# pachterlab/kallisto

Measured on AMD Instinct MI355X. Metric: M paired-end reads/sec quantified (human txome index), higher is better.
Workload: dtype u64+f64

## Files before the change

### include/kallisto_amd.h

```cpp
#ifndef KALLISTO_AMD_H
#define KALLISTO_AMD_H

#include <stddef.h>
#include <stdint.h>

#ifdef __cplusplus
extern "C" {
#endif

#define KAMD_MAX_FRAG_LEN 1000
#define KAMD_SLOTS_PER_BUCKET 3

typedef struct kamd_index kamd_index;
typedef struct kamd_ctx kamd_ctx;

typedef struct {
  int32_t k;
  uint64_t n_kmers, n_unitigs, n_blocks, n_uec, n_ecs, ec_nnz, n_targets, dlist_size;
  uint64_t n_buckets;
  uint64_t pad_buckets;
  const uint64_t* table;
  const uint32_t* slot_block;
  const uint32_t* slot_dist;
  const uint32_t* uec_ec;
  const uint64_t* ec_off;
  const uint32_t* ec_ids;
  const uint64_t* unitig_blk_off;
  const uint32_t* unitig_len;
  const uint32_t* blk_unitig;
  const uint32_t* blk_lb;
  const uint32_t* blk_ub;
  const uint32_t* blk_ec;
  const uint64_t* blk_pos_off;
  const uint32_t* blk_posw;
  const uint8_t* blk_sense;
  const int32_t* target_lens;
  const uint32_t* onlist_bits;
  uint64_t onlist_words;
  const uint64_t* dtable;
  uint64_t n_dbuckets, dpad_buckets;
  uint64_t dummy_slot;
  uint32_t dummy_uec;
  uint32_t dummy_strand;
  const uint32_t* utext;
  uint64_t utext_words;
  uint64_t text_bases;
  const uint64_t* unitig_gpos;
  uint32_t table_layout, slots_per_bucket, tag_q, tag_dsh, tag_w;
  uint64_t n_shades;
  const uint32_t* shade_colour;
  const uint64_t* core_off;
  const uint32_t* core_ids;
  uint64_t core_nnz;
  const uint64_t* shade_off;
  const uint32_t* shade_ids;
  uint64_t shade_nnz;
} kamd_index_view;

typedef struct {
  int32_t paired;
  double fld;
  double sd;
  int32_t single_overhang;
  int32_t strand;
  int32_t no_jump;
  int32_t do_union;
} kamd_quant_opts;

const char* kamd_last_error(void);
#define KAMD_ABI_VERSION 8
uint32_t kamd_abi_version(void);

int kamd_index_load(const char* path, int threads, kamd_index** out);
#define KAMD_TABLE_WIDE 0
#define KAMD_TABLE_COMPACT 1
#define KAMD_TABLE_AUTO 2
int kamd_index_load_layout(const char* path, int threads, int layout, double load, kamd_index** out);
int kamd_index_load_deferred(const char* path, int threads, int layout, double load, kamd_index** out);
int kamd_index_save(const kamd_index*, const char* path);
int kamd_flat_index_matches(const char* flat_path, const char* index_path);
void kamd_index_free(kamd_index*);
int kamd_index_get_view(const kamd_index*, kamd_index_view* out);
const char* kamd_index_target_name(const kamd_index*, uint64_t i);
int kamd_index_check_opts(const kamd_index*, const kamd_quant_opts*);

typedef struct {
  int32_t text_verify;
  int32_t items_per_wave;
  int32_t refill_min;
  int32_t lds_pad;
  int32_t em_form;
  int32_t em_entries_per_lane;
  int32_t em_windowed;
  int32_t em_graph;
  int32_t em_row_lanes;
  int32_t em_fin_blocks;
  int32_t em_local_block;
  int32_t em_group_div;
  int32_t em_split_len;
  int32_t dedup_form;
  int32_t align_chunks;
  int32_t em_small_nnz;
  int32_t em_reg_slices;
  int32_t em_hybrid;
  int32_t overflow_second_pass;
  int32_t em_giant_nnz;
  int32_t em_blocked;
} kamd_tuning;
int kamd_ctx_tune(kamd_ctx*, const kamd_tuning*);
int kamd_ctx_get_tuning(const kamd_ctx*, kamd_tuning* out);
int kamd_ctx_create(int device, void* hip_stream, kamd_ctx** out);
void kamd_ctx_destroy(kamd_ctx*);
int kamd_index_upload(kamd_ctx*, const kamd_index*);
int kamd_ec_reset(kamd_ctx*);
typedef struct {
  uint64_t n_buckets, pad_buckets;
  uint32_t table_layout, slots_per_bucket, tag_q, tag_dsh, tag_w;
  uint64_t n_dbuckets, dpad_buckets;
  uint64_t dummy_slot;
  uint32_t dummy_uec, dummy_strand;
  int32_t built_on_device;
  int32_t build_rounds;
  float build_ms;
  float build_count_ms, build_place_ms, build_order_ms, build_fill_ms, build_dlist_ms;
} kamd_table_info;
int kamd_ctx_table_info(kamd_ctx*, kamd_table_info* out);
int kamd_ctx_table_download(kamd_ctx*, uint64_t* table, uint32_t* slot_block, uint32_t* slot_dist, uint64_t* dtable);

uint64_t kamd_packed_record_words(int32_t max_len);
int kamd_pack_reads_host(const char* seqs, const uint64_t* off, const int32_t* len, uint64_t n_reads, int32_t max_len,
                         uint32_t* out_words, uint16_t* out_len);
int kamd_pack_reads_host_strided(const char* seqs, const uint64_t* off, const int32_t* len, uint64_t n_reads, int32_t max_len,
                                 uint32_t* out_words, uint16_t* out_len, uint64_t rec_stride, uint64_t rec_first);
int kamd_pack_reads_device(kamd_ctx*, const char* d_seqs, const uint64_t* d_off, const int32_t* d_len, uint64_t n_reads,
                           int32_t max_len, uint32_t* d_out_words, uint16_t* d_out_len);

typedef struct {
  const uint32_t* d_words;
  const uint16_t* d_len;
  uint64_t n_items;
  int32_t max_len;
  int32_t status;
  uint64_t first_bad_record;
} kamd_fastq_unit;
int kamd_fastq_unit_parse(kamd_ctx*, const char* const* d_text, const uint64_t* n_bytes, int32_t n_files, uint64_t n_records,
                          kamd_fastq_unit* out);
int kamd_fastq_batch_pack(kamd_ctx*, kamd_fastq_unit* out);
int kamd_fastq_unit_pack(kamd_ctx*, const char* const* d_text, const uint64_t* n_bytes, int32_t n_files, uint64_t n_records,
                         kamd_fastq_unit* out);

int kamd_pseudoalign(kamd_ctx*, const kamd_quant_opts*, const uint32_t* d_words, const uint16_t* d_len, uint64_t n_items,
                     int32_t max_len);
int kamd_fld_from_batch(kamd_ctx*, const kamd_quant_opts*, const uint32_t* d_words, const uint16_t* d_len, uint64_t n_items,
                        int32_t max_len, uint32_t* flens, uint64_t* n_used);
int kamd_fld_prefetch(kamd_ctx*, const kamd_quant_opts*, const uint32_t* d_words, const uint16_t* d_len, uint64_t n_items,
                      int32_t max_len);

typedef struct {
  uint64_t n_processed;
  uint64_t n_single;
  uint64_t n_multi;
  uint64_t n_probes;
  uint64_t n_bucket_reads;
  uint64_t n_distinct_tuples;
  uint64_t n_stream_words;
  uint64_t n_raw_words;
  uint64_t n_text_hits;
  uint64_t n_wave_iters;
  uint64_t n_lane_iters;
} kamd_align_stats;
int kamd_align_stats_get(kamd_ctx*, kamd_align_stats* out);

typedef struct {
  float last_align_kernel_ms;
  float last_em_ms;
  uint64_t last_em_iters;
  float last_classify_ms;
  int32_t kernel_a_version;
  uint64_t last_em_nnz;
  uint64_t last_em_nnz_multi;
  uint64_t last_em_nseg;
  uint64_t last_em_necs;
  int32_t last_em_k;
  uint32_t last_em_grid;
  uint32_t last_em_lds;
  int32_t last_em_plan_cached;
  float last_finalize_ms;
  uint64_t last_fin_records;
  uint64_t last_fin_stream_words;
  uint64_t last_fin_cand_words;
  float absorb_ms;
  uint64_t n_distinct_tuples;
  uint64_t tuple_store_words;
  uint64_t tuple_table_slots;
  uint64_t last_em_max_comp_nnz;
  uint64_t last_em_giant_nnz;
  uint64_t last_em_giant_rows;
  uint64_t last_em_giant_tr;
  uint32_t last_em_giant_chunks;
  int32_t last_em_graph_fallback;
  float last_em_plan_ms;
  uint64_t n_overflow_items;
  float overflow_ms;
  float last_merge_ms;
  float em_collective_ms;
  uint32_t em_collectives;
  uint64_t n_overflow_second_pass;
  uint64_t last_em_giant_pieces;
} kamd_profile;
int kamd_profile_get(kamd_ctx*, kamd_profile* out);

int kamd_debug_random_lines(kamd_ctx*, uint32_t n_blocks, uint32_t block_threads, uint32_t iters, double* gbytes_per_s,
                            double* mlines_per_s);
int kamd_debug_random_lines_span(kamd_ctx*, uint32_t n_blocks, uint32_t block_threads, uint32_t iters, uint32_t span_mb,
                                 uint32_t access_bytes, double* gbytes_per_s, double* mlines_per_s);

int kamd_ec_dense_counts(kamd_ctx*, uint32_t** d_counts, uint64_t* n);
int kamd_ec_tuples_export(kamd_ctx*, uint64_t* n_words, uint64_t* n_tuples);
int kamd_ec_tuples_copy(kamd_ctx*, uint32_t* d_out_words, uint64_t* d_out_rec_off);
int kamd_ec_tuples_replace(kamd_ctx*, const uint32_t* d_words, uint64_t n_words, const uint64_t* d_rec_off, uint64_t n_recs);

int kamd_ec_explicit_export(kamd_ctx*, uint64_t* n_words, uint64_t* n_recs);
int kamd_ec_explicit_copy(kamd_ctx*, uint32_t* d_out_words, uint64_t* d_out_rec_off);
int kamd_ec_explicit_replace(kamd_ctx*, const uint32_t* d_words, uint64_t n_words, const uint64_t* d_rec_off, uint64_t n_recs);

typedef struct kamd_comm kamd_comm;
#define KAMD_COMM_ID_BYTES 128
typedef struct {
  int (*allreduce_sum)(void* user, void* d_buf, uint64_t count, int32_t type);
  int (*allgather)(void* user, const void* d_send, void* d_recv, uint64_t bytes_per_rank);
  int (*broadcast)(void* user, void* d_buf, uint64_t bytes, int32_t root);
} kamd_comm_callbacks;
int kamd_comm_unique_id(void* id128);
int kamd_comm_create_rccl(kamd_ctx*, int32_t rank, int32_t world, const void* id128, kamd_comm** out);
int kamd_comm_create_callbacks(kamd_ctx*, int32_t rank, int32_t world, const kamd_comm_callbacks*, void* user, kamd_comm** out);
void kamd_comm_destroy(kamd_comm*);
int kamd_comm_info(const kamd_comm*, int32_t* rank, int32_t* world, int32_t* ranks_seen, int32_t* backend);
int kamd_ec_allreduce(kamd_ctx*, kamd_comm*);
int kamd_comm_broadcast_host(kamd_ctx*, kamd_comm*, void* buf, uint64_t bytes, int32_t root);
int kamd_comm_sum_u64_host(kamd_ctx*, kamd_comm*, uint64_t* values, uint64_t count);
int kamd_em_run_comm(kamd_ctx*, kamd_comm*, const double* eff_lens, uint64_t n_targets, uint32_t n_iter, uint32_t min_rounds,
                     double* alpha, double* alpha_before_zeroes, int32_t* rounds);

typedef struct {
  uint64_t n_ecs, nnz, n_pseudoaligned;
  const uint64_t* d_ec_off;
  const uint32_t* d_ec_ids;
  const uint32_t* d_counts;
} kamd_ec_result;
int kamd_ec_track_order(kamd_ctx*, int on);
int kamd_ec_finalize(kamd_ctx*, kamd_ec_result* out);
int kamd_ec_finalize_result(kamd_ctx*, kamd_ec_result* out);
int kamd_ec_download(kamd_ctx*, uint64_t* ec_off, uint32_t* ec_ids, uint32_t* counts);
int kamd_ec_upload(kamd_ctx*, const uint64_t* ec_off, const uint32_t* ec_ids, const uint32_t* counts, uint64_t n_ecs);
int kamd_ec_set_counts(kamd_ctx*, const uint32_t* counts);

int kamd_em_run(kamd_ctx*, const uint64_t* d_ec_off, const uint32_t* d_ec_ids, const uint32_t* d_counts,
                const uint32_t* d_weight_counts, uint64_t n_ecs, const double* eff_lens, uint64_t n_targets, uint32_t n_iter,
                uint32_t min_rounds, double* alpha, double* alpha_before_zeroes, int32_t* rounds);

typedef int (*kamd_em_sum_cb)(void* user, int32_t* d_counts, int32_t n);
// ... 58 lines not shown
```

### kallisto_amd/api.py

```python
from __future__ import annotations

import ctypes as C
import os
import sys
from dataclasses import dataclass, field

import numpy as np

HERE = os.path.dirname(os.path.abspath(__file__))
MAX_FRAG_LEN = 1000


class KallistoAmdError(RuntimeError):
    pass


def library_path() -> str:
    return os.path.join(HERE, "libkallisto_amd.so")


class _View(C.Structure):
    _fields_ = ([("k", C.c_int32)] +
                [(n, C.c_uint64) for n in ("n_kmers", "n_unitigs", "n_blocks", "n_uec", "n_ecs", "ec_nnz", "n_targets",
                                           "dlist_size", "n_buckets", "pad_buckets")] +
                [(n, C.c_void_p) for n in ("table", "slot_block", "slot_dist", "uec_ec", "ec_off", "ec_ids",
                                           "unitig_blk_off", "unitig_len", "blk_unitig", "blk_lb", "blk_ub", "blk_ec",
                                           "blk_pos_off", "blk_posw", "blk_sense", "target_lens", "onlist_bits")] +
                [("onlist_words", C.c_uint64), ("dtable", C.c_void_p), ("n_dbuckets", C.c_uint64), ("dpad_buckets", C.c_uint64),
                 ("dummy_slot", C.c_uint64), ("dummy_uec", C.c_uint32), ("dummy_strand", C.c_uint32),
                 ("utext", C.c_void_p), ("utext_words", C.c_uint64), ("text_bases", C.c_uint64), ("unitig_gpos", C.c_void_p)] +
                [(n, C.c_uint32) for n in ("table_layout", "slots_per_bucket", "tag_q", "tag_dsh", "tag_w")] +
                [("n_shades", C.c_uint64), ("shade_colour", C.c_size_t),
                 ("core_off", C.c_size_t), ("core_ids", C.c_size_t), ("core_nnz", C.c_uint64),
                 ("shade_off", C.c_size_t), ("shade_ids", C.c_size_t), ("shade_nnz", C.c_uint64)])


class QuantOpts(C.Structure):
    _fields_ = [("paired", C.c_int32), ("fld", C.c_double), ("sd", C.c_double), ("single_overhang", C.c_int32),
                ("strand", C.c_int32), ("no_jump", C.c_int32), ("do_union", C.c_int32)]


class _Stats(C.Structure):
    _fields_ = [(n, C.c_uint64) for n in ("n_processed", "n_single", "n_multi", "n_probes", "n_bucket_reads",
                                          "n_distinct_tuples", "n_stream_words", "n_raw_words", "n_text_hits", "n_wave_iters",
                                          "n_lane_iters")]


class Tuning(C.Structure):
    _fields_ = [(n, C.c_int32) for n in ("text_verify", "items_per_wave", "refill_min", "lds_pad", "em_form", "em_entries_per_lane", "em_windowed", "em_graph", "em_row_lanes",
                                         "em_fin_blocks", "em_local_block", "em_group_div", "em_split_len", "dedup_form", "align_chunks", "em_small_nnz", "em_reg_slices",
                                         "em_hybrid", "overflow_second_pass", "em_giant_nnz", "em_blocked")]


EM_FORMS = {"streamed": 1, "csr": 2, "local": 3}
ABI_VERSION = 8


class _Profile(C.Structure):
    _fields_ = [("last_align_kernel_ms", C.c_float), ("last_em_ms", C.c_float), ("last_em_iters", C.c_uint64),
                ("last_classify_ms", C.c_float), ("kernel_a_version", C.c_int32), ("last_em_nnz", C.c_uint64),
                ("last_em_nnz_multi", C.c_uint64), ("last_em_nseg", C.c_uint64), ("last_em_necs", C.c_uint64),
                ("last_em_k", C.c_int32), ("last_em_grid", C.c_uint32), ("last_em_lds", C.c_uint32),
                ("last_em_plan_cached", C.c_int32), ("last_finalize_ms", C.c_float), ("last_fin_records", C.c_uint64),
                ("last_fin_stream_words", C.c_uint64), ("last_fin_cand_words", C.c_uint64), ("absorb_ms", C.c_float),
                ("n_distinct_tuples", C.c_uint64), ("tuple_store_words", C.c_uint64), ("tuple_table_slots", C.c_uint64),
                ("last_em_max_comp_nnz", C.c_uint64), ("last_em_giant_nnz", C.c_uint64), ("last_em_giant_rows", C.c_uint64),
                ("last_em_giant_tr", C.c_uint64), ("last_em_giant_chunks", C.c_uint32), ("last_em_graph_fallback", C.c_int32),
                ("last_em_plan_ms", C.c_float), ("n_overflow_items", C.c_uint64), ("overflow_ms", C.c_float),
                ("last_merge_ms", C.c_float), ("em_collective_ms", C.c_float), ("em_collectives", C.c_uint32), ("n_overflow_second_pass", C.c_uint64), ("last_em_giant_pieces", C.c_uint64)]


class _AaStats(C.Structure):
    _fields_ = [("n_processed", C.c_uint64), ("n_rejected_offlist", C.c_uint64), ("n_all_empty", C.c_uint64), ("n_frame_clashes", C.c_uint64),
                ("n_winner", C.c_uint64 * 6), ("last_translate_ms", C.c_float), ("last_match_ms", C.c_float)]


class BgzfMember(C.Structure):
    _fields_ = [("src_off", C.c_uint64), ("src_len", C.c_uint32), ("isize", C.c_uint32), ("crc32", C.c_uint32), ("reserved", C.c_uint32),
                ("dst_off", C.c_uint64)]


class _InflateResult(C.Structure):
    _fields_ = [("status", C.c_int32), ("reason", C.c_int32), ("first_bad_member", C.c_uint64), ("n_bytes", C.c_uint64), ("n_newlines", C.c_uint64)]


class _TableInfo(C.Structure):
    _fields_ = [("n_buckets", C.c_uint64), ("pad_buckets", C.c_uint64), ("table_layout", C.c_uint32), ("slots_per_bucket", C.c_uint32),
                ("tag_q", C.c_uint32), ("tag_dsh", C.c_uint32), ("tag_w", C.c_uint32), ("n_dbuckets", C.c_uint64), ("dpad_buckets", C.c_uint64),
                ("dummy_slot", C.c_uint64), ("dummy_uec", C.c_uint32), ("dummy_strand", C.c_uint32), ("built_on_device", C.c_int32),
                ("build_rounds", C.c_int32), ("build_ms", C.c_float), ("build_count_ms", C.c_float), ("build_place_ms", C.c_float),
                ("build_order_ms", C.c_float), ("build_fill_ms", C.c_float), ("build_dlist_ms", C.c_float)]


class _FastqUnit(C.Structure):
    _fields_ = [("d_words", C.c_void_p), ("d_len", C.c_void_p), ("n_items", C.c_uint64), ("max_len", C.c_int32), ("status", C.c_int32),
                ("first_bad_record", C.c_uint64)]


class _Batch(C.Structure):
    _fields_ = [("d_words", C.c_void_p), ("d_len", C.c_void_p), ("n_items", C.c_uint64), ("max_len", C.c_int32)]


class _QuantOut(C.Structure):
    _fields_ = [("n_processed", C.c_uint64), ("em_rounds", C.c_int32), ("flens", C.c_void_p), ("eff_lens", C.c_void_p), ("est_counts", C.c_void_p),
                ("alpha_before_zeroes", C.c_void_p), ("tpm", C.c_void_p)]


class _EcResult(C.Structure):
    _fields_ = [("n_ecs", C.c_uint64), ("nnz", C.c_uint64), ("n_pseudoaligned", C.c_uint64), ("d_ec_off", C.c_void_p),
                ("d_ec_ids", C.c_void_p), ("d_counts", C.c_void_p)]


_LIB = None

_SYMBOLS = {
    "kamd_last_error": (C.c_char_p, []),
    "kamd_abi_version": (C.c_uint32, []),
    "kamd_index_load": (C.c_int, [C.c_char_p, C.c_int, C.POINTER(C.c_void_p)]),
    "kamd_index_load_layout": (C.c_int, [C.c_char_p, C.c_int, C.c_int, C.c_double, C.POINTER(C.c_void_p)]),
    "kamd_index_load_deferred": (C.c_int, [C.c_char_p, C.c_int, C.c_int, C.c_double, C.POINTER(C.c_void_p)]),
    "kamd_index_free": (None, [C.c_void_p]),
    "kamd_index_save": (C.c_int, [C.c_void_p, C.c_char_p]),
# ... 378 lines not shown
                                                          text.data_ptr(), int(text.numel() if text_cap is None else text_cap), 1 if debug_check_crc else 0,
                                                          C.byref(res), C.byref(ms)), "kamd_debug_bgzf_inflate")
            return {"status": int(res.status), "reason": int(res.reason), "first_bad_member": int(res.first_bad_member), "n_bytes": int(res.n_bytes),
                    "n_newlines": int(res.n_newlines), "kernel_ms": float(ms.value)}
        _check(load_library().kamd_bgzf_inflate(self._h, comp.data_ptr(), int(comp.numel() if comp_bytes is None else comp_bytes), arr, len(members),
                                                text.data_ptr(), int(text.numel() if text_cap is None else text_cap), C.byref(res)), "kamd_bgzf_inflate")
        return {"status": int(res.status), "reason": int(res.reason), "first_bad_member": int(res.first_bad_member), "n_bytes": int(res.n_bytes),
                "n_newlines": int(res.n_newlines)}

    def text_cut(self, texts, n_bytes, max_records: int):
        ptrs = (C.c_void_p * 2)(*[t.data_ptr() for t in texts], *([None] * (2 - len(texts))))
        nb = (C.c_uint64 * 2)(*[int(n) for n in n_bytes], *([0] * (2 - len(texts))))
        nrec, end = C.c_uint64(0), (C.c_uint64 * 2)(0, 0)
        _check(load_library().kamd_text_cut(self._h, ptrs, nb, len(texts), int(max_records), C.byref(nrec), end), "kamd_text_cut")
        return int(nrec.value), [int(end[i]) for i in range(len(texts))]

    def fld_prefetch(self, opts: QuantOpts, words, lens, n_items: int, max_len: int):
        _check(load_library().kamd_fld_prefetch(self._h, C.byref(opts), words.data_ptr(), lens.data_ptr(), n_items, max_len),
               "kamd_fld_prefetch")

    def fld_from_batch(self, opts: QuantOpts, words, lens, n_items: int, max_len: int, flens=None, used: int = 0):
        if flens is None:
            flens = np.zeros(MAX_FRAG_LEN, np.uint32)
        used = C.c_uint64(used)
        _check(load_library().kamd_fld_from_batch(self._h, C.byref(opts), words.data_ptr(), lens.data_ptr(), n_items, max_len,
                                                  flens.ctypes.data, C.byref(used)), "kamd_fld_from_batch")
        return flens, int(used.value)

    def stats(self) -> dict:
        s = _Stats()
        _check(load_library().kamd_align_stats_get(self._h, C.byref(s)), "kamd_align_stats_get")
        return {n: int(getattr(s, n)) for n, _ in _Stats._fields_}

    def random_lines(self, n_blocks: int, block_threads: int = 256, iters: int = 256, span_mb: int = 0, access_bytes: int = 64):
        g, m = C.c_double(0), C.c_double(0)
        _check(load_library().kamd_debug_random_lines_span(self._h, n_blocks, block_threads, iters, span_mb, access_bytes, C.byref(g), C.byref(m)),
               "kamd_debug_random_lines_span")
        return g.value, m.value

    def profile(self) -> dict:
        p = _Profile()
        _check(load_library().kamd_profile_get(self._h, C.byref(p)), "kamd_profile_get")
        return {"align_kernel_ms": float(p.last_align_kernel_ms), "em_ms": float(p.last_em_ms), "em_iters": int(p.last_em_iters),
                "classify_ms": float(p.last_classify_ms), "kernel_a_version": int(p.kernel_a_version),
                "em_nnz": int(p.last_em_nnz), "em_nnz_multi": int(p.last_em_nnz_multi), "em_nseg": int(p.last_em_nseg),
                "em_necs": int(p.last_em_necs), "em_k": int(p.last_em_k), "em_grid": int(p.last_em_grid), "em_lds": int(p.last_em_lds),
                "em_plan_cached": int(p.last_em_plan_cached), "finalize_ms": float(p.last_finalize_ms),
                "fin_records": int(p.last_fin_records), "fin_stream_words": int(p.last_fin_stream_words),
                "fin_cand_words": int(p.last_fin_cand_words), "absorb_ms": float(p.absorb_ms), "n_distinct_tuples": int(p.n_distinct_tuples),
                "tuple_store_words": int(p.tuple_store_words), "tuple_table_slots": int(p.tuple_table_slots),
                "em_max_comp_nnz": int(p.last_em_max_comp_nnz), "em_giant_nnz": int(p.last_em_giant_nnz), "em_giant_rows": int(p.last_em_giant_rows),
                "em_giant_tr": int(p.last_em_giant_tr), "em_giant_chunks": int(p.last_em_giant_chunks), "em_graph_fallback": int(p.last_em_graph_fallback), "em_giant_pieces": int(p.last_em_giant_pieces),
                "em_plan_ms": float(p.last_em_plan_ms), "n_overflow_items": int(p.n_overflow_items), "overflow_ms": float(p.overflow_ms),
                "merge_ms": float(p.last_merge_ms), "em_collective_ms": float(p.em_collective_ms), "em_collectives": int(p.em_collectives), "n_overflow_second_pass": int(p.n_overflow_second_pass)}

    def dense_counts(self):
        torch = self.torch
        p, n = C.c_void_p(), C.c_uint64(0)
        _check(load_library().kamd_ec_dense_counts(self._h, C.byref(p), C.byref(n)), "kamd_ec_dense_counts")
        return _alias_tensor(torch, p.value, int(n.value), torch.int32, self.device)

    def tuples_export(self):
        torch = self.torch
        nw, nt = C.c_uint64(0), C.c_uint64(0)
        _check(load_library().kamd_ec_tuples_export(self._h, C.byref(nw), C.byref(nt)), "kamd_ec_tuples_export")
        words = torch.zeros(max(int(nw.value), 1), dtype=torch.int32, device=f"cuda:{self.device}")
        offs = torch.zeros(max(int(nt.value), 1), dtype=torch.int64, device=f"cuda:{self.device}")
        _check(load_library().kamd_ec_tuples_copy(self._h, words.data_ptr(), offs.data_ptr()), "kamd_ec_tuples_copy")
        return words[:int(nw.value)], offs[:int(nt.value)]

    def tuples_replace(self, words, offs):
        _check(load_library().kamd_ec_tuples_replace(self._h, words.data_ptr() if words.numel() else None, words.numel(),
                                                     offs.data_ptr() if offs.numel() else None, offs.numel()),
               "kamd_ec_tuples_replace")

    def explicit_export(self):
        torch = self.torch
        nw, nr = C.c_uint64(0), C.c_uint64(0)
        _check(load_library().kamd_ec_explicit_export(self._h, C.byref(nw), C.byref(nr)), "kamd_ec_explicit_export")
        words = torch.zeros(max(int(nw.value), 1), dtype=torch.int32, device=f"cuda:{self.device}")
        offs = torch.zeros(max(int(nr.value), 1), dtype=torch.int64, device=f"cuda:{self.device}")
        _check(load_library().kamd_ec_explicit_copy(self._h, words.data_ptr(), offs.data_ptr()), "kamd_ec_explicit_copy")
        return words[:int(nw.value)], offs[:int(nr.value)]

    def explicit_replace(self, words, offs):
        _check(load_library().kamd_ec_explicit_replace(self._h, words.data_ptr() if words.numel() else None, words.numel(),
                                                       offs.data_ptr() if offs.numel() else None, offs.numel()),
               "kamd_ec_explicit_replace")

    def ec_allreduce(self, comm: "Comm"):
        _check(load_library().kamd_ec_allreduce(self._h, comm._h), "kamd_ec_allreduce")

    def em_run_comm(self, comm: "Comm", eff_lens: np.ndarray, n_iter: int = 10000, min_rounds: int = 50):
        eff = np.ascontiguousarray(eff_lens, np.float64)
        T = len(eff)
        alpha = np.zeros(T, np.float64)
        abz = np.zeros(T, np.float64)
        rounds = C.c_int32(0)
        _check(load_library().kamd_em_run_comm(self._h, comm._h, eff.ctypes.data, T, n_iter, min_rounds, alpha.ctypes.data,
                                               abz.ctypes.data, C.byref(rounds)), "kamd_em_run_comm")
        return alpha, abz, int(rounds.value)

    def finalize(self, download: bool = True):
        res = _EcResult()
        _check(load_library().kamd_ec_finalize(self._h, C.byref(res)), "kamd_ec_finalize")
        self.ec_result = res
        if not download:
# ... 404 lines not shown
```

### kallisto_amd/csrc/kamd_ctx.hip

```cpp
#include "kamd_dev.h"

namespace {
void tuning_defaults(kamd_tuning* t) {
  memset(t, 0, sizeof *t);
  t->text_verify = 1; t->items_per_wave = 1024; t->refill_min = 8; t->lds_pad = -1;
  t->em_form = 3; t->em_local_block = 1024; t->em_group_div = -1; t->em_split_len = 16; t->em_small_nnz = -1; t->em_entries_per_lane = -1; t->em_windowed = 2; t->em_graph = 1; t->em_row_lanes = 4;
  t->em_fin_blocks = 1024; t->dedup_form = 2; t->align_chunks = -1; t->em_reg_slices = 1;
  t->em_hybrid = 1; t->overflow_second_pass = 1; t->em_giant_nnz = -1; t->em_blocked = 1;
}
void tuning_merge(kamd_tuning* t, const kamd_tuning& n) {
  if (n.text_verify == 1 || n.text_verify == 2) t->text_verify = n.text_verify;
  if (n.dedup_form == 1 || n.dedup_form == 2) t->dedup_form = n.dedup_form;
  if (n.items_per_wave >= 64) t->items_per_wave = n.items_per_wave;
  if (n.refill_min >= 1 && n.refill_min <= 64) t->refill_min = n.refill_min;
  if (n.lds_pad != 0) t->lds_pad = n.lds_pad < 0 ? -1 : n.lds_pad;
  if (n.em_form >= 1 && n.em_form <= 3) t->em_form = n.em_form;
  if (n.em_local_block == 128 || n.em_local_block == 256 || n.em_local_block == 512 || n.em_local_block == 1024) t->em_local_block = n.em_local_block;
  if (n.em_split_len >= 1 && n.em_split_len <= 64) t->em_split_len = n.em_split_len;
  if (n.em_group_div >= 1 && n.em_group_div <= 1024) t->em_group_div = n.em_group_div;
  else if (n.em_group_div < 0) t->em_group_div = -1;
  if (n.em_small_nnz != 0) t->em_small_nnz = n.em_small_nnz < 0 ? -1 : std::min(n.em_small_nnz, 4096);
  if (n.em_entries_per_lane != 0) t->em_entries_per_lane = n.em_entries_per_lane < 0 ? -1 : n.em_entries_per_lane;
  if (n.em_windowed == 1 || n.em_windowed == 2) t->em_windowed = n.em_windowed;
  if (n.em_graph == 1 || n.em_graph == 2) t->em_graph = n.em_graph;
  if (n.em_row_lanes == 2 || n.em_row_lanes == 4 || n.em_row_lanes == 8) t->em_row_lanes = n.em_row_lanes;
  if (n.em_fin_blocks >= 64) t->em_fin_blocks = n.em_fin_blocks;
  if (n.align_chunks != 0) t->align_chunks = n.align_chunks < 0 ? -1 : std::min(n.align_chunks, 64);
  if (n.em_reg_slices == 1 || n.em_reg_slices == 2) t->em_reg_slices = n.em_reg_slices;
  if (n.em_hybrid == 1 || n.em_hybrid == 2) t->em_hybrid = n.em_hybrid;
  if (n.overflow_second_pass >= 1 && n.overflow_second_pass <= 3) t->overflow_second_pass = n.overflow_second_pass;
  if (n.em_blocked == 1 || n.em_blocked == 2) t->em_blocked = n.em_blocked;
  if (n.em_giant_nnz != 0) t->em_giant_nnz = n.em_giant_nnz < 0 ? -1 : std::max(n.em_giant_nnz, 8);
}
void tuning_from_env(kamd_tuning* t) {
  const char* e = getenv("KAMD_TUNE");
  if (!e || !*e) return;
  kamd_tuning n; memset(&n, 0, sizeof n);
  struct Field { const char* name; int32_t kamd_tuning::*p; bool onoff; };
  static const Field fields[] = {
    {"text_verify", &kamd_tuning::text_verify, true}, {"items_per_wave", &kamd_tuning::items_per_wave, false}, {"refill_min", &kamd_tuning::refill_min, false},
    {"lds_pad", &kamd_tuning::lds_pad, false}, {"em_form", &kamd_tuning::em_form, false}, {"em_entries_per_lane", &kamd_tuning::em_entries_per_lane, false},
    {"em_windowed", &kamd_tuning::em_windowed, true}, {"em_graph", &kamd_tuning::em_graph, true}, {"em_row_lanes", &kamd_tuning::em_row_lanes, false},
    {"em_fin_blocks", &kamd_tuning::em_fin_blocks, false}, {"em_local_block", &kamd_tuning::em_local_block, false}, {"em_group_div", &kamd_tuning::em_group_div, false},
    {"em_split_len", &kamd_tuning::em_split_len, false}, {"dedup_form", &kamd_tuning::dedup_form, false}, {"align_chunks", &kamd_tuning::align_chunks, false},
    {"em_small_nnz", &kamd_tuning::em_small_nnz, false}, {"em_reg_slices", &kamd_tuning::em_reg_slices, true}, {"em_hybrid", &kamd_tuning::em_hybrid, true},
    {"overflow_second_pass", &kamd_tuning::overflow_second_pass, false}, {"em_giant_nnz", &kamd_tuning::em_giant_nnz, false}, {"em_blocked", &kamd_tuning::em_blocked, true}};
  std::string all(e);
  for (size_t pos = 0; pos < all.size();) {
    size_t end = all.find(',', pos);
    if (end == std::string::npos) end = all.size();
    const std::string kv = all.substr(pos, end - pos);
    pos = end + 1;
    const size_t eq = kv.find('=');
    if (eq == std::string::npos) continue;
    const std::string key = kv.substr(0, eq), val = kv.substr(eq + 1);
    bool known = false;
    for (const Field& f : fields) {
      if (key != f.name) continue;
      known = true;
      int32_t v = atoi(val.c_str());
      if (key == "em_form") v = val == "streamed" ? 1 : val == "csr" ? 2 : val == "local" ? 3 : v;
      if (key == "overflow_second_pass" && v == 0) v = 2;
      n.*(f.p) = f.onoff ? (v != 0 ? 1 : 2) : v;
    }
    if (!known) fprintf(stderr, "[kallisto_amd] KAMD_TUNE: unknown field '%s' ignored\n", key.c_str());
  }
  tuning_merge(t, n);
}
}
namespace kamdi {
void apply_quant_opts(kamd_ctx* c, const kamd_quant_opts* o) {
  c->ix.no_jump = o->no_jump ? 1 : 0;
  c->ix.union_mode = o->do_union ? 1 : 0;
  c->ix.comprehensive = (o->strand != 0 && (o->no_jump || o->do_union || c->ix.n_shades)) ? 1 : 0;
}
void apply_tuning(kamd_ctx* c) {
  c->items_per_wave = c->tune.items_per_wave; c->refill_min = c->tune.refill_min;
}
int sync_state(kamd_ctx* c) {
  if (!c->state_pin) HIPC(hipHostMalloc((void**)&c->state_pin, sizeof(DevState), hipHostMallocDefault));
  HIPC(hipMemcpyAsync(c->state_pin, c->state.p, sizeof(DevState), hipMemcpyDeviceToHost, c->stream));
  HIPC(hipStreamSynchronize(c->stream));
  memcpy(&c->host_state, c->state_pin, sizeof(DevState));
  return 0;
}
int push_state(kamd_ctx* c) {
  HIPC(hipMemcpyAsync(c->state.p, &c->host_state, sizeof(DevState), hipMemcpyHostToDevice, c->stream));
  return 0;
}
}

extern "C" uint32_t kamd_abi_version(void) { return KAMD_ABI_VERSION; }
extern "C" int kamd_ctx_create(int device, void* hip_stream, kamd_ctx** out) {
  if (!out) return kamd::fail(-1, "kamd_ctx_create: null output pointer");
  *out = nullptr;
  int ndev = 0;
  if (hipGetDeviceCount(&ndev) != hipSuccess || ndev == 0)
    return kamd::fail(-102, "kamd_ctx_create: no HIP device available (this library has no CPU path)");
  if (device < 0 || device >= ndev) return kamd::fail(-1, "kamd_ctx_create: bad device ordinal");
// ... 219 lines not shown
    const u64 b = __umul64hi(x, n_buckets);
    u64 v;
    if (WORDS == 8) {
      const ulonglong2* bp = (const ulonglong2*)(table + b * 8);
      const ulonglong2 s0 = bp[0], s1 = bp[1], s2 = bp[2], s3 = bp[3];
      v = s0.x ^ s0.y ^ s1.x ^ s1.y ^ s2.x ^ s2.y ^ s3.x ^ s3.y;
    } else v = table[b * 8 + (x & 7)];
    acc ^= v;
    x = kamd::mix64(x ^ v);
  }
  if (acc == 0x1234567ULL) sink[0] = acc;
}
}
extern "C" int kamd_debug_random_lines_span(kamd_ctx* c, uint32_t n_blocks, uint32_t block_threads, uint32_t iters, uint32_t span_mb,
                                            uint32_t access_bytes, double* gbytes_per_s, double* mlines_per_s) {
  if (!c || !c->has_index) return kamd::fail(-1, "kamd_debug_random_lines: no context / index");
  HIPC(hipSetDevice(c->device));
  if (int rc = c->sizes.ensure(64, 0, c->stream)) return rc;
  u64 nb = c->ix.n_buckets;
  if (span_mb) nb = std::min<u64>(nb, (u64)span_mb * 1024 * 1024 / 64);
  auto launch = [&](int it) {
    if (access_bytes == 8) hipLaunchKernelGGL(k_random_lines<1>, dim3(n_blocks), dim3(block_threads), 0, c->stream, c->ix.table, nb, it, c->sizes.as<u64>());
    else hipLaunchKernelGGL(k_random_lines<8>, dim3(n_blocks), dim3(block_threads), 0, c->stream, c->ix.table, nb, it, c->sizes.as<u64>());
  };
  launch(8);
  HIPC(hipEventRecord(c->ev0, c->stream));
  launch((int)iters);
  HIPC(hipEventRecord(c->ev1, c->stream));
  HIPC(hipEventSynchronize(c->ev1));
  float ms = 0.f;
  HIPC(hipEventElapsedTime(&ms, c->ev0, c->ev1));
  const double lines = (double)n_blocks * block_threads * iters;
  if (mlines_per_s) *mlines_per_s = lines / (ms * 1e-3) / 1e6;
  if (gbytes_per_s) *gbytes_per_s = lines * 64.0 / (ms * 1e-3) / 1e9;
  return 0;
}
extern "C" int kamd_debug_random_lines(kamd_ctx* c, uint32_t n_blocks, uint32_t block_threads, uint32_t iters, double* gbytes_per_s,
                                       double* mlines_per_s) {
  return kamd_debug_random_lines_span(c, n_blocks, block_threads, iters, 0, 64, gbytes_per_s, mlines_per_s);
}

extern "C" int kamd_profile_get(kamd_ctx* c, kamd_profile* p) {
  if (!c || !p) return kamd::fail(-1, "kamd_profile_get: null argument");
  p->last_align_kernel_ms = c->last_align_ms; p->last_em_ms = c->last_em_ms; p->last_em_iters = c->last_em_iters;
  p->last_classify_ms = c->last_classify_ms; p->kernel_a_version = 3;
  p->last_em_nnz = c->last_em_nnz; p->last_em_nnz_multi = c->last_em_nnz_multi; p->last_em_nseg = c->last_em_nseg; p->last_em_necs = c->last_em_necs;
  p->last_em_k = c->last_em_k; p->last_em_grid = c->last_em_grid; p->last_em_lds = c->last_em_lds; p->last_em_plan_cached = c->last_em_plan_cached;
  p->last_finalize_ms = c->last_finalize_ms; p->last_fin_records = c->last_fin_records; p->last_fin_stream_words = c->last_fin_stream_words;
  p->last_fin_cand_words = c->last_fin_cand_words;
  p->absorb_ms = c->last_absorb_ms; p->n_distinct_tuples = c->n_distinct_tuples; p->tuple_store_words = c->host_state.ts_words; p->tuple_table_slots = c->tcap;
  p->last_em_max_comp_nnz = c->last_em_max_comp_nnz; p->last_em_giant_nnz = c->last_em_giant_nnz; p->last_em_giant_rows = c->last_em_giant_rows;
  p->last_em_giant_tr = c->last_em_giant_tr; p->last_em_giant_chunks = c->last_em_giant_chunks; p->last_em_graph_fallback = c->last_em_graph_fallback; p->last_em_giant_pieces = c->last_em_giant_pieces;
  p->last_em_plan_ms = c->last_em_plan_ms;
  p->n_overflow_items = c->overflow_total; p->overflow_ms = c->overflow_ms;
  p->n_overflow_second_pass = c->overflow_second_total;
  p->last_merge_ms = c->last_merge_ms; p->em_collective_ms = c->em_coll_ms; p->em_collectives = c->em_coll_n;
  return 0;
}

namespace {
typedef struct ncclComm* ncclComm_t;
typedef struct { char internal[KAMD_COMM_ID_BYTES]; } ncclUniqueId;
typedef int ncclResult_t;
enum { kNcclSum = 0, kNcclUint8 = 1, kNcclInt32 = 2, kNcclUint32 = 3, kNcclUint64 = 5, kNcclFloat64 = 8 };
struct RcclApi {
  void* lib = nullptr;
  ncclResult_t (*GetUniqueId)(ncclUniqueId*) = nullptr;
  ncclResult_t (*CommInitRank)(ncclComm_t*, int, ncclUniqueId, int) = nullptr;
  ncclResult_t (*CommDestroy)(ncclComm_t) = nullptr;
  ncclResult_t (*CommCount)(const ncclComm_t, int*) = nullptr;
  ncclResult_t (*AllReduce)(const void*, void*, size_t, int, int, ncclComm_t, hipStream_t) = nullptr;
  ncclResult_t (*AllGather)(const void*, void*, size_t, int, ncclComm_t, hipStream_t) = nullptr;
  ncclResult_t (*Broadcast)(const void*, void*, size_t, int, int, ncclComm_t, hipStream_t) = nullptr;
  const char* (*GetErrorString)(ncclResult_t) = nullptr;
};
RcclApi g_rccl;
int rccl_load() {
  if (g_rccl.lib) return 0;
  void* h = nullptr;
  for (const char* n : {"librccl.so", "librccl.so.1"}) { h = dlopen(n, RTLD_NOW | RTLD_NOLOAD); if (h) break; }
  if (!h) if (const char* e = getenv("KAMD_RCCL_LIB")) h = dlopen(e, RTLD_NOW | RTLD_GLOBAL);
  if (!h) for (const char* n : {"librccl.so.1", "librccl.so", "/opt/rocm/lib/librccl.so.1", "/opt/rocm/lib/librccl.so"}) { h = dlopen(n, RTLD_NOW | RTLD_GLOBAL); if (h) break; }
  if (!h) return kamd::fail(-106, std::string("kamd_comm: librccl.so could not be loaded (") + (dlerror() ? dlerror() : "not found") + "); set KAMD_RCCL_LIB");
  RcclApi a; a.lib = h;
  a.GetUniqueId = (decltype(a.GetUniqueId))dlsym(h, "ncclGetUniqueId");
  a.CommInitRank = (decltype(a.CommInitRank))dlsym(h, "ncclCommInitRank");
  a.CommDestroy = (decltype(a.CommDestroy))dlsym(h, "ncclCommDestroy");
  a.CommCount = (decltype(a.CommCount))dlsym(h, "ncclCommCount");
  a.AllReduce = (decltype(a.AllReduce))dlsym(h, "ncclAllReduce");
  a.AllGather = (decltype(a.AllGather))dlsym(h, "ncclAllGather");
  a.Broadcast = (decltype(a.Broadcast))dlsym(h, "ncclBroadcast");
  a.GetErrorString = (decltype(a.GetErrorString))dlsym(h, "ncclGetErrorString");
  if (!a.GetUniqueId || !a.CommInitRank || !a.CommDestroy || !a.AllReduce || !a.AllGather || !a.Broadcast)
    return kamd::fail(-106, "kamd_comm: librccl.so lacks an expected entry point");
  g_rccl = a;
  return 0;
}
int rccl_fail(ncclResult_t r, const char* what) {
  return kamd::fail(-107, std::string(what) + ": " + (g_rccl.GetErrorString ? g_rccl.GetErrorString(r) : "RCCL error") + " (" + std::to_string(r) + ")");
}
}

struct kamd_comm {
  kamd_ctx* ctx = nullptr;
  int device = 0;
  int rank = 0, world = 1;
// ... 307 lines not shown
```

### kallisto_amd/csrc/kamd_dev.h

```cpp
#pragma once

#include <hip/hip_runtime.h>

#include <dlfcn.h>

#include <algorithm>
#include <cstring>
#include <string>
#include <chrono>
#include <thread>
#include <vector>

#include "../../include/kallisto_amd.h"
#include "kamd_core.h"
#include "kamd_fq_core.h"
#include "kamd_host.h"
#include "kamd_em_local.h"
#include "kamd_em_sell.h"

#define HIPC(x)                                                                                   \
  do {                                                                                            \
    hipError_t e_ = (x);                                                                          \
    if (e_ != hipSuccess) return kamd::fail(-100, std::string(#x) + ": " + hipGetErrorString(e_)); \
  } while (0)
// ... 199 lines not shown
  u32 n_set_bitmaps = 0;
  kamd_table_info tinfo{};
  DBuf dense, stream_buf, rec_off, overflow_items, overflow_scratch, state, rec_slot, retry, ttable, list;
  DBuf cand, cand_off, cand_slot, ctable, clist, sizes, block_sums, tup_bound, tup_off, tup_big;
  DBuf raw2, overflow_left, stats_b;
  u64 overflow_second_total = 0;
  DBuf ov_state; DevState* ov_pin = nullptr; hipStream_t ov_stream = nullptr; hipEvent_t ov_ev_in = nullptr, ov_ev_done = nullptr, ov_ev_t0 = nullptr, ov_ev_t1 = nullptr;
  bool ov_side_pending = false;
  u64 last_fin_big = 0;
  DBuf explicit_items, explicit_items_big, exp_stream, exp_off, exp_scratch, bs_cp, bs_samp, raw, dense_first, exp_key, cand_key, ec_first;
  DBuf ec_off, ec_ids, ec_counts;
  DBuf em_alpha, em_next, em_eff, em_state, em_cn, em_colcnt, em_coloff, em_colrow, em_segoff, em_segt, em_partial, em_a0, em_a1, em_single, em_actflag, em_actpos, em_active;
  DBuf pm_a, pm_b, pm_rank;
  DBuf eml_tmp, ems_tmp, ems_plan, ems_maps;
  SellCache* sell_cache = nullptr;
  u64 ec_generation = 0;
  int last_em_plan_cached = 0;
  DBuf fq_tiles, fq_nlpos[2], fq_recs, fq_res, fq_words, fq_len;
  void* fq_host = nullptr;
  u64 fq_batch_reads = 0; int32_t fq_batch_max_len = 0, fq_batch_files = 0;
  DBuf fld_tl, fld_card, fld_scratch, fld_items, fld_cand;
  void* fld_host = nullptr; u64 fld_host_cap = 0;
  hipStream_t fld_stream = nullptr; hipEvent_t fld_ev = nullptr, fld_ev_in = nullptr;
  struct { const uint32_t* w = nullptr; const uint16_t* l = nullptr; u64 n = 0; int32_t max_len = 0, strand = 0, so = 0; bool valid = false; } fld_pending;
  struct { const uint32_t* w = nullptr; const uint16_t* l = nullptr; u64 n = 0; int32_t max_len = 0, strand = 0, so = 0, comp = 0; bool valid = false; } fld_deferred;
  DBuf pt_label, pt_flag, pt_len, pt_rowpos, pt_nnzpos, pt_off, pt_ids, pt_counts, pt_wcounts, pt_hist, pt_ck_alpha, pt_ck_a;
  DevState host_state{};
  DevState* state_pin = nullptr;
  u64 tcap = 0, ccap = 0;
  DBuf tstore;
  bool ttable_clean = false;
  u64 recs_total = 0;
  u64 multi_before = 0;
  u64 n_distinct_tuples = 0;
  float last_absorb_ms = 0.f; hipEvent_t ev_ab0 = nullptr, ev_ab1 = nullptr;
  kamd_ec_result result{};
  bool finalized = false;
  u64 exp_words_done = 0;
  hipEvent_t ev0 = nullptr, ev1 = nullptr;
  float last_align_ms = 0.f, last_em_ms = 0.f, last_classify_ms = 0.f;
  hipEvent_t ev2 = nullptr, ev3 = nullptr, ev_fin0 = nullptr, ev_fin1 = nullptr;
  DBuf stats_a;
  hipStream_t al_stream = nullptr; hipEvent_t al_ev_in = nullptr, al_ev_out = nullptr; std::vector<hipEvent_t> al_ev_chunk;
  float last_finalize_ms = 0.f; u64 last_fin_records = 0, last_fin_stream_words = 0, last_fin_cand_words = 0;
  hipStream_t em_stream = nullptr;
  hipStream_t em_side_stream = nullptr; hipEvent_t em_ev_fork = nullptr, em_ev_join = nullptr;
  void* em_pin = nullptr; size_t em_pin_bytes = 0;
  DBuf em_clk;
  DBuf hy_sub, hy_a, hy_b, hy_x, hy_maps;
  DBuf hy_gb[6];
  hipStream_t hy_giant_stream = nullptr;
  hipEvent_t hy_ev_sell = nullptr, hy_ev_giant = nullptr;
  uint64_t last_em_max_comp_nnz = 0, last_em_giant_nnz = 0, last_em_giant_rows = 0, last_em_giant_tr = 0;
  uint32_t last_em_giant_chunks = 0; uint64_t last_em_giant_pieces = 0; int last_em_graph_fallback = 0; float last_em_plan_ms = 0.f;
  float last_merge_ms = 0.f, em_coll_ms = 0.f; uint32_t em_coll_n = 0; hipEvent_t ev_mg0 = nullptr, ev_mg1 = nullptr;
  const uint32_t* labels_override = nullptr;
  bool em_prefer_hybrid = false;
  uint64_t overflow_total = 0; float overflow_ms = 0.f; hipEvent_t ev_ov0 = nullptr, ev_ov1 = nullptr;
  int items_per_wave = 1024, refill_min = 8;
  kamd_tuning tune{};
  bool track_order = false;
  bool had_overflow_items = false;
  int n_cus = 0, last_em_k = 0; unsigned last_em_grid = 0, last_em_lds = 0;
  uint64_t last_em_iters = 0, last_em_nnz = 0, last_em_nnz_multi = 0, last_em_nseg = 0, last_em_necs = 0;
  DBuf aa_frames, aa_flen, aa_scratch, aa_offlist, aa_ctr;
  bool aa_ready = false;
  kamd_aa_stats aa_stats{};
  hipEvent_t aa_ev[3] = {nullptr, nullptr, nullptr};
  DBuf inf_members, inf_res, txt_counts, txt_res;
  std::vector<struct kamd_comm*> comms;
};

namespace kamdi {
int sync_state(kamd_ctx* c);
int push_state(kamd_ctx* c);
void apply_quant_opts(kamd_ctx* c, const kamd_quant_opts* o);
void apply_tuning(kamd_ctx* c);
void comm_detach_all(kamd_ctx* c);
int index_build_device(kamd_ctx* c, const kamd_index* hix, const kamd_index_view& v, DevIndex* d, kamd_table_info* info);
int exclusive_scan(kamd_ctx* c, const u32* sizes, u64 n, u64* out, u64* d_total);
int tuples_clear(kamd_ctx* c);
int absorb_tuples(kamd_ctx* c, const u32* batch, const u64* rec_off, u64 n, u64 batch_words, u64 key_base, u64 n_tuple_bound,
                  const u64* first_idx = nullptr, u32 fixed_stride = 0, u64 item0 = 0);
template <class T>
int upload(kamd_ctx* c, const T* host, size_t n, const T** dev) {
  void* p = nullptr;
  size_t bytes = std::max<size_t>(n, 1) * sizeof(T);
  HIPC(hipMalloc(&p, bytes));
  c->index_allocs.push_back(p);
  if (n) HIPC(hipMemcpyAsync(p, host, n * sizeof(T), hipMemcpyHostToDevice, c->stream));
  *dev = reinterpret_cast<const T*>(p);
  return 0;
}
}
```

### kallisto_amd/csrc/kamd_em.hip

```cpp
#include "kamd_dev.h"

namespace {

struct EmState {
  int iter;
  int chcount;
  int final_round;
  int done;
  int rounds;
  int force_final;
  int pad[2];
};
struct EmNow { int it, fin, done, rounds; };
__host__ __device__ inline EmNow em_next_round(const EmState& prev, int n_iter, int min_rounds, bool spec) {
  EmNow n; n.it = prev.iter; n.fin = prev.final_round; n.done = prev.done; n.rounds = prev.rounds;
  if (n.done) return n;
  if (prev.final_round) { n.done = 1; n.rounds = prev.iter; return n; }
  const bool stopEM = !spec && prev.chcount == 0 && prev.iter > min_rounds;
  n.it = prev.iter + 1;
  n.fin = (stopEM || prev.force_final) ? 1 : 0;
  if (n.it >= n_iter) { n.done = 1; n.rounds = n_iter; }
  return n;
}
__device__ __forceinline__ double em_clamped(const double* alpha, const double* a, u32 t, int clamp) {
// ... 1078 lines not shown
    ems_reg_gather<NB>(w, lds0, v);
#pragma unroll
    for (int i = 0; i < 4 * NB; i++) S += v[i];
    if constexpr (NQ > 2) return ems_reg_sum<NQ - 2, false>(w + 2, lds0, S);
    else return S;
  } else {
    constexpr int NB = NQ < 4 ? NQ : 4;
    double v[4 * NB];
    ems_reg_gather<NB>(w, lds0, v);
#pragma unroll
    for (int st = 1; st < 4 * NB; st *= 2)
#pragma unroll
      for (int i = 0; i + st < 4 * NB; i += 2 * st) v[i] += v[i + st];
    if constexpr (NQ > 4) return ems_reg_sum<NQ - 4, true>(w + 4, lds0, S + v[0]);
    else return S + v[0];
  }
}
template <int W, bool TREE, int NQ = 1>
__device__ __forceinline__ double ems_reg_slice_sum(const u64* w, u32 nq, const unsigned char* lds0) {
  if constexpr (NQ >= W) return ems_reg_sum<W, TREE>(w, lds0);
  else { if (nq <= (u32)NQ) return ems_reg_sum<NQ, TREE>(w, lds0); return ems_reg_slice_sum<W, TREE, NQ + 1>(w, nq, lds0); }
}
__device__ __forceinline__ u32 pm_scan_seg_steps(int reach, int lane) {
  const int r = lane & 15;
  u32 m = 0;
  if (__ballot(reach >= 1 && r >= 1)) m |= 1u;
  if (__ballot(reach >= 2 && r >= 2)) m |= 2u;
  if (__ballot(reach >= 4 && r >= 4)) m |= 4u;
  if (__ballot(reach >= 8 && r >= 8)) m |= 8u;
  if (__ballot((lane & 16) && reach > r)) m |= 16u;
  if (__ballot(lane >= 32 && reach > lane - 32)) m |= 32u;
  return m;
}
__device__ __forceinline__ double pm_scan_seg_masked(double y, int reach, int lane, u32 steps) {
  const int r = lane & 15;
  if (steps & 1u) { const double t = pm_dpp<0x111, 0xF>(y); if (reach >= 1 && r >= 1) y += t; }
  if (steps & 2u) { const double t = pm_dpp<0x112, 0xF>(y); if (reach >= 2 && r >= 2) y += t; }
  if (steps & 4u) { const double t = pm_dpp<0x114, 0xF>(y); if (reach >= 4 && r >= 4) y += t; }
  if (steps & 8u) { const double t = pm_dpp<0x118, 0xF>(y); if (reach >= 8 && r >= 8) y += t; }
  if (steps & 16u) { const double t = pm_dpp<0x142, 0xA>(y); if ((lane & 16) && reach > r) y += t; }
  if (steps & 32u) { const double t = pm_dpp<0x143, 0xC>(y); if (lane >= 32 && reach > lane - 32) y += t; }
  return y;
}
__device__ __forceinline__ double ems_slice_sum_narrow(const u64* e, u32 width, const double* src) {
  double S = 0.0;
  for (u32 j = 0; j < width; j += 4) {
    const u64 w = e[(size_t)(j >> 2) * 64];
    const u32 lo = (u32)w, hi = (u32)(w >> 32);
    const double v0 = src[lo & 0xFFFFu], v1 = src[lo >> 16], v2 = src[hi & 0xFFFFu], v3 = src[hi >> 16];
    S += v0; S += v1; S += v2; S += v3;
  }
  return S;
}
template <int W, int NS>
__device__ __forceinline__ void ems_group_rounds_reg(const EmSellDev& P, u32 g, unsigned char* smem, u32 tid, u32 nthr, const double* alpha, const double* a,
                                                     double* alpha_out, double* a_out, int n_rounds, int clamp, int* s_hist, long long* clk = nullptr) {
  namespace L = kamd_em_sell;
  constexpr bool TREE = W >= 8 || (W == 4 && NS == 2);
  const int lane = lane_id();
  const u32 wv = (u32)__builtin_amdgcn_readfirstlane((int)(tid >> 6)), NW = nthr >> 6;
  const u32 r0 = P.row_base[g], nR = P.row_base[g + 1] - r0, t0 = P.tr_base[g], nT = P.tr_base[g + 1] - t0;
  const u32 rs0 = P.rslice_base[g], nrs = P.rslice_base[g + 1] - rs0, cs0 = P.cslice_base[g], ncs = P.cslice_base[g + 1] - cs0;
  const u64 re0 = P.rell_base[g], ce0 = P.cell_base[g];
  const u32 nru = (u32)(P.rell_base[g + 1] - re0), ncu = (u32)(P.cell_base[g + 1] - ce0);
  double* s_a0 = reinterpret_cast<double*>(smem);
  double* s_g = s_a0 + (nT + 1);
  double* s_al0 = s_g + (nR + 1);
  double* s_single = s_al0 + (nT + 1); double* s_eff = s_single + nT;
  u64* s_cw = reinterpret_cast<u64*>(s_eff + nT);
  u32* s_rdesc = reinterpret_cast<u32*>(s_cw + nR); u32* s_cdesc = s_rdesc + 2 * nrs;
  uint16_t* s_rell = reinterpret_cast<uint16_t*>(s_cdesc + 2 * ncs); uint16_t* s_cell = s_rell + ((nru + 1) & ~1u);
  const u32 a_off = 0u, g_off = (nT + 1) * 8u;
  const bool near = g_off + (nR + 1) * 8u <= 0x10000u;
  for (u32 i = tid; i < nT; i += nthr) {
    double al = alpha[t0 + i], av = a[t0 + i];
    if (clamp && al < 1e-7 / 10.0) { al = 0.0; av = 0.0; }
    s_al0[i] = al; s_a0[i] = av; s_single[i] = P.single[t0 + i]; s_eff[i] = P.eff[t0 + i];
  }
  for (u32 i = tid; i < nR; i += nthr) s_cw[i] = P.cw[r0 + i];
  for (u32 i = tid; i < 2 * nrs; i += nthr) s_rdesc[i] = P.rdesc[2 * (u64)rs0 + i];
  for (u32 i = tid; i < 2 * ncs; i += nthr) s_cdesc[i] = P.cdesc[2 * (u64)cs0 + i];
  for (u32 i = tid; i < nru; i += nthr) { const uint16_t v = P.rell[re0 + i]; s_rell[i] = v == (uint16_t)L::SELL_PAD ? (uint16_t)nT : v; }
  for (u32 i = tid; i < ncu; i += nthr) { const uint16_t v = P.cell[ce0 + i]; s_cell[i] = v == (uint16_t)L::SELL_PAD ? (uint16_t)nR : v; }
  if (tid == 0) { s_al0[nT] = s_a0[nT] = 0.0; s_g[nR] = 0.0; }
  __syncthreads();
  struct Own { u64 w[W]; u32 nq, seg, steps; int reach; bool has, meta, fin; };
  auto take = [&](const u32* desc, const uint16_t* ell, u32 s, u32 n_slices, u32 n_segs, u32 zero, u32 base_off) {
    Own o;
    o.has = near && s < n_slices; o.nq = 1; o.seg = 0; o.reach = 0; o.meta = false; o.fin = false; o.steps = 0;
    if (o.has && (((desc[2 * s + 1] & 0xFFFFu) + 3u) >> 2) > (u32)W) o.has = false;
    const u64 padw = (u64)(base_off + zero * 8u) * 0x0001000100010001ULL;
#pragma unroll
    for (int q = 0; q < W; q++) o.w[q] = padw;
    if (o.has) {
      const u32 d0 = desc[2 * s], d1 = desc[2 * s + 1];
      o.meta = (d0 & L::DESC_META) != 0;
      const u32 off = d0 & ~L::DESC_META, width = d1 & 0xFFFFu;
      o.nq = (u32)__builtin_amdgcn_readfirstlane((int)((width + 3u) >> 2));
      const u64* e = reinterpret_cast<const u64*>(ell + off + (o.meta ? 2 * L::SELL_META_WORDS : 0u)) + lane;
#pragma unroll
      for (int q = 0; q < W; q++) if ((u32)q < o.nq) {
        const u64 ix4 = e[(size_t)q * 64];
        o.w[q] = ((ix4 & 0x1FFF1FFF1FFF1FFFULL) << 3) + (u64)base_off * 0x0001000100010001ULL;
      }
      o.seg = (d1 >> 16) + (u32)lane; o.fin = o.seg < n_segs;
      if (o.meta) {
        const u32 w = reinterpret_cast<const u32*>(ell + off)[lane];
        o.reach = (int)((w >> 16) & 0x7Fu); o.seg = w & 0xFFFFu; o.fin = (w & L::META_ACTIVE) && (w & L::META_LAST);
        o.steps = pm_scan_seg_steps(o.reach, lane);
      }
      if (!o.fin) o.seg = 0;
    }
    return o;
  };
  Own ro[NS], co[NS];
  u32 r_cnt[NS], r_wc[NS];
  double c_single[NS], c_eff[NS], c_at[NS], c_cur[NS];
  u32 r_next = wv, c_next = wv;
#pragma unroll
  for (int k = 0; k < NS; k++) {
    ro[k] = take(s_rdesc, s_rell, wv + (u32)k * NW, nrs, nR, nT, a_off);
    co[k] = take(s_cdesc, s_cell, wv + (u32)k * NW, ncs, nT, nR, g_off);
    if (ro[k].has && r_next == wv + (u32)k * NW) r_next += NW; else ro[k].has = false;
    if (co[k].has && c_next == wv + (u32)k * NW) c_next += NW; else co[k].has = false;
    r_cnt[k] = 0; r_wc[k] = 0; c_single[k] = 0.0; c_eff[k] = 1.0; c_at[k] = 0.0; c_cur[k] = 0.0;
    if (ro[k].has && ro[k].fin) { const u64 cwv = s_cw[ro[k].seg]; r_cnt[k] = (u32)cwv; r_wc[k] = (u32)(cwv >> 32); }
    if (co[k].has && co[k].fin) { c_single[k] = s_single[co[k].seg]; c_eff[k] = s_eff[co[k].seg]; c_at[k] = s_a0[co[k].seg]; c_cur[k] = s_al0[co[k].seg]; }
  }
  double* const al = s_al0; double* const av = s_a0;
  const unsigned char* const lds0 = smem;
  for (int r = 0; r < n_rounds; r++) {
    const bool tick = clk && r == EMS_CLK_ROUND && lane == 0;
    long long w0 = 0;
    if (tick) { clk[0] = clock64(); w0 = wall_clock64(); }
#pragma unroll
    for (int k = 0; k < NS; k++) {
      if (ro[k].has) {
        const bool tk = tick && k == 0;
        if (tk) clk[12] = clock64();
        double S = ems_reg_slice_sum<W, TREE>(ro[k].w, ro[k].nq, lds0);
        if (tk) { clk[13] = clock64(); clk[14] = (long long)((ro[k].nq * 4u) | (ro[k].meta ? 0x10000u : 0u)); }
        if (ro[k].meta) S = pm_scan_seg_masked(S, ro[k].reach, lane, ro[k].steps);
        if (ro[k].fin) s_g[ro[k].seg] = (r_cnt[k] == 0 || (double)r_wc[k] * S < 4.9406564584124654e-324) ? 0.0 : (double)r_cnt[k] / S;
        if (tk) clk[15] = clock64();
      }
    }
    for (u32 s = r_next; s < nrs; s += NW) {
      const u32 d0 = s_rdesc[2 * s], d1 = s_rdesc[2 * s + 1];
      const bool meta = (d0 & L::DESC_META) != 0;
      const u32 off = d0 & ~L::DESC_META, width = d1 & 0xFFFFu;
      double S = ems_slice_sum_narrow(reinterpret_cast<const u64*>(s_rell + off + (meta ? 2 * L::SELL_META_WORDS : 0u)) + lane, width, av);
      u32 seg = (d1 >> 16) + (u32)lane; bool fin = seg < nR;
      if (meta) {
        const u32 w = reinterpret_cast<const u32*>(s_rell + off)[lane];
        S = pm_scan_seg(S, (int)((w >> 16) & 0x7Fu), lane);
        seg = w & 0xFFFFu; fin = (w & L::META_ACTIVE) && (w & L::META_LAST);
      }
      if (fin) {
        const u64 cwv = s_cw[seg];
        const u32 cnt = (u32)cwv, wc = (u32)(cwv >> 32);
        s_g[seg] = (cnt == 0 || (double)wc * S < 4.9406564584124654e-324) ? 0.0 : (double)cnt / S;
      }
    }
    if (tick) clk[1] = clock64();
    __syncthreads();
    if (tick) clk[2] = clock64();
    int ch = 0;
    auto finish_col = [&](u32 seg, double at, double cur, double single, double eff, double acc, double& nx_out, double& a_out_v) {
      const double nx = single + at * acc;
      const double dd = fabs(nx - cur);
      bool moved = dd > 1.0000001e-2 * nx;
      if (dd > 0.9999999e-2 * nx && !moved) moved = dd / nx > 1e-2;
      nx_out = nx; a_out_v = nx / eff;
      al[seg] = nx; av[seg] = a_out_v;
      return nx > 1e-2 && moved;
    };
#pragma unroll
    for (int k = 0; k < NS; k++) {
      if (co[k].has) {
        const bool tk = tick && k == 0;
        if (tk) clk[8] = clock64();
        double acc = ems_reg_slice_sum<W, TREE>(co[k].w, co[k].nq, lds0);
        if (tk) { clk[9] = clock64(); clk[10] = (long long)((co[k].nq * 4u) | (co[k].meta ? 0x10000u : 0u)); }
        if (co[k].meta) acc = pm_scan_seg_masked(acc, co[k].reach, lane, co[k].steps);
        bool chg = false;
        if (co[k].fin) chg = finish_col(co[k].seg, c_at[k], c_cur[k], c_single[k], c_eff[k], acc, c_cur[k], c_at[k]);
        ch += __popcll(__ballot(chg));
        if (tk) clk[11] = clock64();
      }
    }
    for (u32 s = c_next; s < ncs; s += NW) {
      const u32 d0 = s_cdesc[2 * s], d1 = s_cdesc[2 * s + 1];
      const bool meta = (d0 & L::DESC_META) != 0;
      const u32 off = d0 & ~L::DESC_META, width = d1 & 0xFFFFu;
      double acc = ems_slice_sum_narrow(reinterpret_cast<const u64*>(s_cell + off + (meta ? 2 * L::SELL_META_WORDS : 0u)) + lane, width, s_g);
      u32 seg = (d1 >> 16) + (u32)lane; bool fin = seg < nT;
      if (meta) {
        const u32 w = reinterpret_cast<const u32*>(s_cell + off)[lane];
        acc = pm_scan_seg(acc, (int)((w >> 16) & 0x7Fu), lane);
        seg = w & 0xFFFFu; fin = (w & L::META_ACTIVE) && (w & L::META_LAST);
      }
      bool chg = false;
      if (fin) { double nx, an; chg = finish_col(seg, av[seg], al[seg], s_single[seg], s_eff[seg], acc, nx, an); }
      ch += __popcll(__ballot(chg));
    }
    if (ch && lane == 0) atomicAdd(&s_hist[r], ch);
    if (tick) clk[3] = clock64();
    __syncthreads();
    if (tick) { clk[4] = clock64(); clk[5] = (long long)(nrs | (ncs << 16)); clk[6] = (long long)(nru | ((u64)ncu << 32)); clk[7] = wall_clock64() - w0; }
  }
  for (u32 i = tid; i < nT; i += nthr) { alpha_out[t0 + i] = al[i]; a_out[t0 + i] = av[i]; }
}
struct EmsPrev { const int* hist; int n; int base; int min_rounds; int* host_hist; int* host_seq; int seq; };
__device__ __forceinline__ bool ems_prev_stopped(const EmsPrev& v, int* s_flag) {
  if (!v.hist) return false;
  if (threadIdx.x < 64) {
    const int i = (int)threadIdx.x;
    const int h = i < v.n ? v.hist[i] : 1;
    const bool stop = i < v.n && h == 0 && v.base + i > v.min_rounds;
    const u64 m = __ballot(stop);
    if (blockIdx.x == 0 && v.host_hist) {
      if (i < v.n) v.host_hist[i] = h;
      __threadfence_system();
      if (i == 0) __hip_atomic_store(v.host_seq, v.seq, __ATOMIC_RELEASE, __HIP_MEMORY_SCOPE_SYSTEM);
    }
    if (i == 0) *s_flag = m != 0;
  }
  __syncthreads();
  return *s_flag != 0;
}
template <bool CLK, int EXP = 0, int W = 0, int NS = 1>
__global__ __launch_bounds__(EMS_MAX_BLOCK) __attribute__((amdgpu_waves_per_eu((W >= 8 || (W == 4 && NS == 2)) ? 4 : 8))) void k_em_sell(EmSellDev P, u32 g_first, const double* alpha, const double* a, double* alpha_out, double* a_out,
                                                           int n_rounds, int clamp, int* hist, EmsPrev prev, long long* clk) {
  extern __shared__ __attribute__((aligned(16))) unsigned char ems_smem[];
  __shared__ int s_hist[EML_MAX_ROUNDS];
  __shared__ int s_stop;
  if (ems_prev_stopped(prev, &s_stop)) return;
  if (threadIdx.x < EML_MAX_ROUNDS) s_hist[threadIdx.x] = 0;
  __syncthreads();
  long long* my_clk = CLK ? clk + ((size_t)blockIdx.x * (EMS_MAX_BLOCK / 64) + (threadIdx.x >> 6)) * EMS_CLK_WORDS : nullptr;
  if constexpr (W > 0) ems_group_rounds_reg<W, NS>(P, g_first + blockIdx.x, ems_smem, threadIdx.x, blockDim.x, alpha, a, alpha_out, a_out, n_rounds, clamp, s_hist, my_clk);
  else ems_group_rounds<false, EXP>(P, g_first + blockIdx.x, ems_smem, threadIdx.x, blockDim.x, alpha, a, alpha_out, a_out, n_rounds, clamp, s_hist, my_clk);
  __syncthreads();
  if (hist && (int)threadIdx.x < n_rounds && s_hist[threadIdx.x]) atomicAdd(&hist[threadIdx.x], s_hist[threadIdx.x]);
}
constexpr int EMS_WAVE_TEAMS = 4;
__global__ __launch_bounds__(64 * EMS_WAVE_TEAMS) void k_em_sell_wave(EmSellDev P, u32 n_small, u32 team_bytes, const double* alpha, const double* a,
                                                                        double* alpha_out, double* a_out, int n_rounds, int clamp, int* hist, EmsPrev prev) {
  extern __shared__ __attribute__((aligned(16))) unsigned char ems_smem[];
  __shared__ int s_hist[EML_MAX_ROUNDS];
  __shared__ int s_stop;
  if (ems_prev_stopped(prev, &s_stop)) return;
  if (threadIdx.x < EML_MAX_ROUNDS) s_hist[threadIdx.x] = 0;
  __syncthreads();
  const u32 team = (u32)__builtin_amdgcn_readfirstlane((int)(threadIdx.x >> 6));
  const u32 g = blockIdx.x * EMS_WAVE_TEAMS + team;
  if (g < n_small) ems_group_rounds<true>(P, g, ems_smem + (size_t)team * team_bytes, (u32)lane_id(), 64u, alpha, a, alpha_out, a_out, n_rounds, clamp, s_hist);
  __syncthreads();
  if (hist && (int)threadIdx.x < n_rounds && s_hist[threadIdx.x]) atomicAdd(&hist[threadIdx.x], s_hist[threadIdx.x]);
}
struct SellBuild {
  const u32* row_base; const u32* tr_base; const u32* row_ptr; const u32* col_ptr; const uint16_t* row_tr; const uint16_t* col_row; const u64* nz_base;
  const u64* cw; const double* single; const double* eff; const u32* tr_id; u32 n_groups; u32 R; u32 M; u32 cap;
  u32* rlen; u32* clen; u32* rnew; u32* cnew; u32* rlane; u32* clane; u32* rvl; u32* cvl; u32* gsz;
  const u32* rslice_base; const u32* cslice_base; const u64* rell_base; const u64* cell_base;
  u32* rdesc; u32* cdesc; uint16_t* rell; uint16_t* cell; u64* cw_new; double* single_new; double* eff_new; u32* tr_id_new;
};
__device__ __forceinline__ u32 sell_group_of(const u32* base, u32 n_groups, u32 i) {
  u32 lo = 0, hi = n_groups;
  while (hi - lo > 1) { const u32 mid = (lo + hi) / 2; if (base[mid] <= i) lo = mid; else hi = mid; }
  return lo;
}
__global__ void k_sell_lens(SellBuild B) {
  const u32 i = blockIdx.x * blockDim.x + threadIdx.x;
  if (i < B.R) { const u32 g = sell_group_of(B.row_base, B.n_groups, i); B.rlen[i] = B.row_ptr[(u64)i + g + 1] - B.row_ptr[(u64)i + g]; }
  if (i < B.M) { const u32 g = sell_group_of(B.tr_base, B.n_groups, i); B.clen[i] = B.col_ptr[(u64)i + g + 1] - B.col_ptr[(u64)i + g]; }
}
constexpr int SELL_BUILD_WAVES = 4;
struct SellWaveScratch { u32 hist[kamd_em_sell::SELL_LANES + 1], start[kamd_em_sell::SELL_LANES + 1], cur[kamd_em_sell::SELL_LANES + 1]; };
template <class Sink>
__device__ kamd_em_sell::LayoutSize sell_layout_wave(const u32* __restrict__ len, u32 n, u32 cap, Sink& sink, SellWaveScratch& S) {
  namespace L = kamd_em_sell;
  const int lane = lane_id();
  for (u32 b = lane; b <= L::SELL_LANES; b += 64) { S.hist[b] = 0; S.cur[b] = 0; }
  __builtin_amdgcn_wave_barrier();
  u32 n_split = 0, pos = 0;
  u32 off = 0;
  u32 width = 0;
  u32 mw = 0;
  u32 closed = 0;
  for (u32 c0 = 0; c0 < n; c0 += 64) {
    const u32 i = c0 + lane;
    const u32 l = i < n ? len[i] : 0;
    if (i < n && l <= cap) atomicAdd(&S.hist[l], 1u);
    u64 m = __ballot(i < n && l > cap);
    while (m) {
      const int b = __ffsll((unsigned long long)m) - 1;
      m &= m - 1;
      const u32 lb = (u32)__shfl((int)l, b, 64);
      const u32 nv = L::seg_lanes(lb, cap), vl = L::seg_vlen(lb, cap);
      if ((pos % L::SELL_LANES) + nv > L::SELL_LANES) {
        sink.meta(off, lane, mw);
        if (lane == 0) sink.slice(closed, off | L::DESC_META, width);
        off += 2 * L::SELL_META_WORDS + L::quad_width(width) * L::SELL_LANES; ++closed; width = 0; mw = 0;
        pos = (pos / L::SELL_LANES + 1) * L::SELL_LANES;
      }
      if (Sink::wants_segments && lane == b) sink.seg(c0 + b, n_split, pos, nv, vl);
      const u32 rel = pos % L::SELL_LANES;
      if ((u32)lane >= rel && (u32)lane < rel + nv) {
        const u32 v = (u32)lane - rel;
        mw = n_split | (v << 16) | (v + 1 == nv ? L::META_LAST : 0u) | L::META_ACTIVE;
      }
      width = vl > width ? vl : width;
      pos += nv; ++n_split;
      if (pos % L::SELL_LANES == 0) {
        sink.meta(off, lane, mw);
        if (lane == 0) sink.slice(closed, off | L::DESC_META, width);
        off += 2 * L::SELL_META_WORDS + L::quad_width(width) * L::SELL_LANES; ++closed; width = 0; mw = 0;
      }
    }
  }
  __builtin_amdgcn_wave_barrier();
  const u32 split_lanes = pos;
  if (lane == 0) { u32 c = split_lanes; for (u32 b = L::SELL_LANES; b >= 1; b--) { S.start[b] = c; c += S.hist[b]; } S.start[0] = c; }
  __builtin_amdgcn_wave_barrier();
  const u32 total_lanes = S.start[0];
  if (Sink::wants_segments) {
    for (u32 c0 = 0; c0 < n; c0 += 64) {
      const u32 i = c0 + lane;
      const u32 l = i < n ? len[i] : 0u;
      const bool act = i < n && l <= cap;
      u64 same = __ballot(act);
#pragma unroll
      for (int b = 0; b < 7; b++) { const u64 bal = __ballot((l >> b) & 1u); same &= ((l >> b) & 1u) ? bal : ~bal; }
      const u32 below = (u32)__popcll(same & ((1ULL << lane) - 1ULL)), cls = (u32)__popcll(same);
      u32 base = 0;
      if (act) base = S.cur[l];
      __builtin_amdgcn_wave_barrier();
      if (act) {
        const u32 p = S.start[l] + base + below;
        sink.seg(i, n_split + (p - split_lanes), p, 1u, l);
        if (below + 1 == cls) S.cur[l] = base + cls;
      }
      __builtin_amdgcn_wave_barrier();
    }
  }
  auto len_at = [&](u32 p) -> u32 {
    u32 b = L::SELL_LANES;
    while (b > 1 && !(p >= S.start[b] && p < S.start[b] + S.hist[b])) --b;
    return b;
  };
  const u32 n_slices = (total_lanes + L::SELL_LANES - 1) / L::SELL_LANES;
  if (split_lanes % L::SELL_LANES) {
    const u32 lo = closed * L::SELL_LANES, p = lo + (u32)lane;
    if (split_lanes < total_lanes) { const u32 b = len_at(split_lanes); width = b > width ? b : width; }
    if (p >= split_lanes && p < total_lanes) mw = (n_split + (p - split_lanes)) | L::META_LAST | L::META_ACTIVE;
    sink.meta(off, lane, mw);
    if (lane == 0) sink.slice(closed, off | L::DESC_META, width);
    off += 2 * L::SELL_META_WORDS + L::quad_width(width) * L::SELL_LANES; ++closed;
  }
  for (u32 s0 = closed; s0 < n_slices; s0 += 64) {
    const u32 si = s0 + (u32)lane;
    u32 w = 0;
    if (si < n_slices) w = len_at(si * L::SELL_LANES);
    const u32 mine = L::quad_width(w) * L::SELL_LANES;
    const u32 incl = wave_incl_scan(mine);
    if (si < n_slices) sink.slice(si, off + (incl - mine), w | ((n_split + (si * L::SELL_LANES - split_lanes)) << 16));
    off += (u32)__shfl((int)incl, 63, 64);
  }
  return L::LayoutSize{n_slices, off};
}
__global__ __launch_bounds__(64 * SELL_BUILD_WAVES) void k_sell_sizes(SellBuild B) {
  __shared__ SellWaveScratch scr[SELL_BUILD_WAVES];
  const u32 w = (blockIdx.x * blockDim.x + threadIdx.x) / 64, g = w >> 1;
  if (g >= B.n_groups) return;
  kamd_em_sell::NullSink ns;
  const kamd_em_sell::LayoutSize z = (w & 1) ? sell_layout_wave(B.clen + B.tr_base[g], B.tr_base[g + 1] - B.tr_base[g], B.cap, ns, scr[threadIdx.x / 64])
                                             : sell_layout_wave(B.rlen + B.row_base[g], B.row_base[g + 1] - B.row_base[g], B.cap, ns, scr[threadIdx.x / 64]);
  if (lane_id() == 0) { B.gsz[4 * g + 2 * (w & 1)] = z.n_slices; B.gsz[4 * g + 2 * (w & 1) + 1] = z.n_u16; }
}
struct SellDevSink {
  static const bool wants_segments = true;
  u32* new_id; u32* lane; u32* vlen; u32* desc; uint16_t* ell; u32 seg0; u32 desc0; u64 ell0;
  __device__ void seg(u32 old, u32 id, u32 ln, u32, u32 vl) const { new_id[seg0 + old] = id; lane[seg0 + old] = ln; vlen[seg0 + old] = vl; }
  __device__ void slice(u32 i, u32 d0, u32 d1) const { desc[2 * (u64)(desc0 + i)] = d0; desc[2 * (u64)(desc0 + i) + 1] = d1; }
  __device__ void meta(u32 off, u32 l, u32 w) const { ell[ell0 + off + 2 * l] = (uint16_t)w; ell[ell0 + off + 2 * l + 1] = (uint16_t)(w >> 16); }
};
__global__ __launch_bounds__(64 * SELL_BUILD_WAVES) void k_sell_layout(SellBuild B) {
  __shared__ SellWaveScratch scr[SELL_BUILD_WAVES];
  const u32 w = (blockIdx.x * blockDim.x + threadIdx.x) / 64, g = w >> 1;
  if (g >= B.n_groups) return;
  if (w & 1) {
    SellDevSink sc{B.cnew, B.clane, B.cvl, B.cdesc, B.cell, B.tr_base[g], B.cslice_base[g], B.cell_base[g]};
    sell_layout_wave(B.clen + B.tr_base[g], B.tr_base[g + 1] - B.tr_base[g], B.cap, sc, scr[threadIdx.x / 64]);
  } else {
    SellDevSink sr{B.rnew, B.rlane, B.rvl, B.rdesc, B.rell, B.row_base[g], B.rslice_base[g], B.rell_base[g]};
    sell_layout_wave(B.rlen + B.row_base[g], B.row_base[g + 1] - B.row_base[g], B.cap, sr, scr[threadIdx.x / 64]);
  }
}
__global__ void k_sell_entries(SellBuild B) {
  const u32 i = blockIdx.x * blockDim.x + threadIdx.x;
  if (i < B.R) {
    const u32 g = sell_group_of(B.row_base, B.n_groups, i), r0 = B.row_base[g], t0 = B.tr_base[g];
    B.cw_new[r0 + B.rnew[i]] = B.cw[i];
    const u32* rd = B.rdesc + 2 * (u64)B.rslice_base[g];
    const uint16_t* src = B.row_tr + B.nz_base[g];
    const u32 b = B.row_ptr[(u64)i + g], e = B.row_ptr[(u64)i + g + 1];
    const u32 ln = B.rlane[i], vl = B.rvl[i];
    for (u32 j = b, q = 0; j < e; j++, q++)
      B.rell[B.rell_base[g] + kamd_em_sell::entry_pos(rd, ln, vl, q)] = (uint16_t)B.cnew[t0 + src[j]];
  }
  if (i < B.M) {
    const u32 g = sell_group_of(B.tr_base, B.n_groups, i), r0 = B.row_base[g], t0 = B.tr_base[g];
    const u32 m = t0 + B.cnew[i];
    B.single_new[m] = B.single[i]; B.eff_new[m] = B.eff[i]; B.tr_id_new[m] = B.tr_id[i];
    const u32* cd = B.cdesc + 2 * (u64)B.cslice_base[g];
    const uint16_t* src = B.col_row + B.nz_base[g];
    const u32 b = B.col_ptr[(u64)i + g], e = B.col_ptr[(u64)i + g + 1];
    const u32 ln = B.clane[i], vl = B.cvl[i];
    for (u32 j = b, q = 0; j < e; j++, q++)
      B.cell[B.cell_base[g] + kamd_em_sell::entry_pos(cd, ln, vl, q)] = (uint16_t)B.rnew[r0 + src[j]];
  }
}
__global__ void k_eml_init(double* alpha, double* a, const double* __restrict__ eff_m, u64 M, double a0) {
  const u64 m = (u64)blockIdx.x * blockDim.x + threadIdx.x;
  if (m < M) { alpha[m] = a0; a[m] = a0 / eff_m[m]; }
}
__device__ __forceinline__ void eml_step_tr_f_wave(u64 t, const kamd_em_local::BuildArgs& A) {
  const bool act = t < A.T && A.in_multi[t];
  const u32 g = act ? kamd_em_local::eml_group_of(A, A.label[t]) : 0xFFFFFFFFu;
  u64 m = __ballot(act);
  const u64 lt = (1ULL << lane_id()) - 1ULL;
  while (m) {
    const int leader = __ffsll((long long)m) - 1;
    const u32 lg = (u32)__shfl((int)g, leader, 64);
    const u64 same = __ballot(act && g == lg);
    u32 base = 0;
    if (lane_id() == leader) base = atomicAdd(&A.tr_fill[lg], (u32)__popcll(same));
    base = (u32)__shfl((int)base, leader, 64);
    if (act && g == lg) A.tmp_tr_id[(u64)A.tr_base[lg] + base + (u32)__popcll(same & lt)] = (u32)t;
    m &= ~same;
  }
}
__device__ __forceinline__ void eml_step_tr_b_wave(u64 t, const kamd_em_local::BuildArgs& A) {
  const bool act = t < A.T && A.in_multi[t];
  const u32 r = act ? A.label[t] : 0xFFFFFFFFu;
  u64 m = __ballot(act);
  while (m) {
    const int leader = __ffsll((long long)m) - 1;
    const u32 lr = (u32)__shfl((int)r, leader, 64);
// ... 977 lines not shown
  if (P.n_fix[0]) hipLaunchKernelGGL(k_gi_rows_fix, dim3(grid_for(P.n_chunks, PM_BLOCK)), dim3(PM_BLOCK), 0, s, P.args, G.desc);
  if (P.windowed) hipLaunchKernelGGL((k_gi_cols<K, PRE_C, true>), dim3(grid), dim3(PM_BLOCK), 0, s, P.args, al_src, a_src, al_dst, a_dst, round, clamp, G.desc);
  else hipLaunchKernelGGL((k_gi_cols<K, PRE_C, false>), dim3(grid), dim3(PM_BLOCK), 0, s, P.args, al_src, a_src, al_dst, a_dst, round, clamp, G.desc);
  if (P.n_fix[1]) hipLaunchKernelGGL(k_gi_cols_fix, dim3(grid_for(P.n_chunks, PM_BLOCK)), dim3(PM_BLOCK), 0, s, P.args, al_src, a_src, al_dst, a_dst, round, clamp, G.desc);
}
void gi_enqueue_rounds(const GiantPart& G, hipStream_t s, int n, int clamp, int pin, int pout) {
  const u32 M = G.plan.args.M;
  for (int i = 0; i < n; i++) {
    const double* al_src = i == 0 ? G.G_al[pin] : G.S_al[(i - 1) & 1];
    const double* a_src = i == 0 ? G.G_a[pin] : G.S_a[(i - 1) & 1];
    double* al_dst = i == n - 1 ? G.G_al[pout] : G.S_al[i & 1];
    double* a_dst = i == n - 1 ? G.G_a[pout] : G.S_a[i & 1];
    if (clamp) {
      hipLaunchKernelGGL(k_gi_clamp, dim3(grid_for((u64)M + 1, BLOCK)), dim3(BLOCK), 0, s, al_src, a_src, G.ac, M, G.desc);
      a_src = G.ac;
    }
    if (G.gb.valid) { gb_round(G, s, i, clamp, al_src, a_src, al_dst, a_dst); continue; }
    switch (G.plan.k) {
      case 8: gi_round<8>(G, s, i, clamp, al_src, a_src, al_dst, a_dst); break;
      case 12: gi_round<12>(G, s, i, clamp, al_src, a_src, al_dst, a_dst); break;
      case 16: gi_round<16>(G, s, i, clamp, al_src, a_src, al_dst, a_dst); break;
      case 20: gi_round<20>(G, s, i, clamp, al_src, a_src, al_dst, a_dst); break;
      case 24: gi_round<24>(G, s, i, clamp, al_src, a_src, al_dst, a_dst); break;
      case 28: gi_round<28>(G, s, i, clamp, al_src, a_src, al_dst, a_dst); break;
      default: gi_round<32>(G, s, i, clamp, al_src, a_src, al_dst, a_dst); break;
    }
  }
}
int gi_launch_chunk(GiantPart& G, int n, int clamp, int pin, int pout, int* d_h, const EmsPrev& prev) {
  hipLaunchKernelGGL(k_gi_set_desc, dim3(1), dim3(64), 0, G.stream, G.desc, prev, d_h);
  if (G.use_graph && n == EML_MAX_ROUNDS && !clamp && pin != pout) {
    if (!G.gexec[pin]) {
      const bool inject = getenv("KAMD_DEBUG_GRAPH_FAIL") != nullptr;
      hipError_t e = hipStreamBeginCapture(G.stream, hipStreamCaptureModeThreadLocal);
      if (e == hipSuccess) {
        gi_enqueue_rounds(G, G.stream, n, 0, pin, pout);
        e = hipStreamEndCapture(G.stream, &G.graph[pin]);
      }
      if (e == hipSuccess && inject && G.gexec[pin ^ 1]) e = hipErrorOutOfMemory;
      if (e == hipSuccess) e = hipGraphInstantiate(&G.gexec[pin], G.graph[pin], nullptr, nullptr, 0);
      if (e != hipSuccess) {
        (void)hipGetLastError();
        G.drop_graphs();
        G.use_graph = false;
      }
    }
    if (G.use_graph) { HIPC(hipGraphLaunch(G.gexec[pin], G.stream)); }
    else gi_enqueue_rounds(G, G.stream, n, clamp, pin, pout);
  } else gi_enqueue_rounds(G, G.stream, n, clamp, pin, pout);
  HIPC(hipGetLastError());
  return 0;
}
}
namespace kamdi {
struct SellCache {
  bool valid = false;
  const u64* d_ec_off = nullptr; const u32* d_ec_ids = nullptr; u64 n_ecs = 0, nnz = 0, T = 0, generation = 0;
  int split_len = 0, group_div = 0, small_nnz = 0;
  bool host_maps = false;
  kamd_em_sell::Plan P;
  EmSellDev dev{};
  u32* row_final = nullptr; u32* mslot = nullptr; double* single_all = nullptr; double* d_eff = nullptr;
  bool hybrid = false;
  GiantPart G;
  struct HyKeep {
    const u32* flag_s = nullptr; const u32* flag_g = nullptr; const u64* rpos_s = nullptr; const u64* rpos_g = nullptr;
    const u64* off_s = nullptr; const u64* off_g = nullptr; const u32* ids_s = nullptr; const u32* ids_g = nullptr;
    u32* cnt_s = nullptr; u32* cnt_g = nullptr; u32* wc_s = nullptr; u32* wc_g = nullptr;
    u64 n_s = 0, n_g = 0; bool no_groups = false;
  } hy;
  int giant_nnz_t = 0, blocked_t = 0, hybrid_t = 0;
  ~SellCache() { G.drop_graphs(); }
};
}
namespace {

__global__ void k_em_publish(EmsPrev prev);
struct EmSellGpu {
  kamd_ctx* c; const kamd_em_sell::Plan& P; EmSellDev dev{}; u64 M = 0; size_t lds = 0, team_bytes = 0; int block = 256;
  hipStream_t side = nullptr; hipEvent_t ev_fork = nullptr, ev_join = nullptr;
  int reg_words = 0;
  double* d_alpha = nullptr; double* d_a = nullptr; double* d_ck_alpha = nullptr; double* d_ck_a = nullptr; int* d_hist = nullptr; double* d_out = nullptr;
  std::vector<double> h_alpha; int err = 0;
  const EmPartition* part = nullptr;
  GiantPart* gi = nullptr;
  hipEvent_t ev_sell = nullptr;
  int gi_par(const double* al) const { return al == d_alpha ? 0 : 1; }
  EmSellGpu(kamd_ctx* ctx, const kamd_em_sell::Plan& p) : c(ctx), P(p) {}
  int setup(int hist_ints, const double* d_eff_new, u64 T_out);
  void checkpoint() {
    if (err) return;
    if (hipMemcpyAsync(d_ck_alpha, d_alpha, M * 8, hipMemcpyDeviceToDevice, c->stream) != hipSuccess ||
        hipMemcpyAsync(d_ck_a, d_a, M * 8, hipMemcpyDeviceToDevice, c->stream) != hipSuccess) err = -104;
    if (gi && !err) {
      const size_t gb = ((size_t)gi->plan.args.M + 1) * 8;
      if (hipMemcpyAsync(gi->G_al[1], gi->G_al[0], gb, hipMemcpyDeviceToDevice, c->stream) != hipSuccess ||
          hipMemcpyAsync(gi->G_a[1], gi->G_a[0], gb, hipMemcpyDeviceToDevice, c->stream) != hipSuccess) err = -104;
    }
  }
  void restore() {
    if (err) return;
    if (hipMemcpyAsync(d_alpha, d_ck_alpha, M * 8, hipMemcpyDeviceToDevice, c->stream) != hipSuccess ||
        hipMemcpyAsync(d_a, d_ck_a, M * 8, hipMemcpyDeviceToDevice, c->stream) != hipSuccess) err = -104;
    if (gi && !err) {
      const size_t gb = ((size_t)gi->plan.args.M + 1) * 8;
      if (hipMemcpyAsync(gi->G_al[0], gi->G_al[1], gb, hipMemcpyDeviceToDevice, c->stream) != hipSuccess ||
          hipMemcpyAsync(gi->G_a[0], gi->G_a[1], gb, hipMemcpyDeviceToDevice, c->stream) != hipSuccess) err = -104;
    }
  }
  std::vector<double> h_gi_cur, h_gi_prev; int host_reads = 0;
  int launch(int n, int clamp, const double* al_in, const double* a_in, double* al_out, double* a_out, int* d_h, const EmsPrev& prev, long long* clk = nullptr) {
    if (n <= 0 || n > EML_MAX_ROUNDS) return -104;
    const u32 n_big = P.n_groups - P.n_small;
    const bool fork = P.n_small && n_big;
    hipStream_t ss = c->stream;
    if ((fork || gi) && hipEventRecord(ev_fork, c->stream) != hipSuccess) return -104;
    if (fork && hipStreamWaitEvent(side, ev_fork, 0) != hipSuccess) return -104;
    if (gi) {
      if (!n_big && !P.n_small && prev.hist && prev.host_hist) hipLaunchKernelGGL(k_em_publish, dim3(1), dim3(64), 0, c->stream, prev);
      if (hipStreamWaitEvent(gi->stream, ev_fork, 0) != hipSuccess) return -104;
      if (ss != c->stream && hipStreamWaitEvent(ss, ev_fork, 0) != hipSuccess) return -104;
      if (int rc = gi_launch_chunk(*gi, n, clamp, gi_par(al_in), gi_par(al_out), d_h, prev)) return rc;
      if (hipEventRecord(gi->ev, gi->stream) != hipSuccess) return -104;
    }
    if (n_big) {
#define KAMD_EMS_LAUNCH(C, E) hipLaunchKernelGGL((k_em_sell<C, E>), dim3(n_big), dim3(block), lds, ss, dev, P.n_small, al_in, a_in, al_out, a_out, n, clamp, d_h, prev, clk)
#define KAMD_EMS_LAUNCH_REG(C, W, NS) hipLaunchKernelGGL((k_em_sell<C, 0, W, NS>), dim3(n_big), dim3(block), lds, ss, dev, P.n_small, al_in, a_in, al_out, a_out, n, clamp, d_h, prev, clk)
      if (reg_words == 2) { if (clk) KAMD_EMS_LAUNCH_REG(true, 2, 1); else KAMD_EMS_LAUNCH_REG(false, 2, 1); }
      else if (reg_words == 4) { if (clk) KAMD_EMS_LAUNCH_REG(true, 4, 2); else KAMD_EMS_LAUNCH_REG(false, 4, 2); }
      else if (reg_words == 8) { if (clk) KAMD_EMS_LAUNCH_REG(true, 8, 1); else KAMD_EMS_LAUNCH_REG(false, 8, 1); }
      else if (clk) KAMD_EMS_LAUNCH(true, 0);
      else KAMD_EMS_LAUNCH(false, 0);
#undef KAMD_EMS_LAUNCH
#undef KAMD_EMS_LAUNCH_REG
    }
    EmsPrev prev_w = prev;
    if (n_big) prev_w.host_hist = nullptr;
    if (P.n_small) hipLaunchKernelGGL(k_em_sell_wave, dim3((P.n_small + EMS_WAVE_TEAMS - 1) / EMS_WAVE_TEAMS), dim3(64 * EMS_WAVE_TEAMS), (size_t)EMS_WAVE_TEAMS * team_bytes,
                                      fork ? side : c->stream, dev, P.n_small, (u32)team_bytes, al_in, a_in, al_out, a_out, n, clamp, d_h, prev_w);
    if (hipGetLastError() != hipSuccess) return -104;
    if (fork && (hipEventRecord(ev_join, side) != hipSuccess || hipStreamWaitEvent(c->stream, ev_join, 0) != hipSuccess)) return -104;
    if (gi) {
      if (ss != c->stream && (hipEventRecord(ev_sell, ss) != hipSuccess || hipStreamWaitEvent(c->stream, ev_sell, 0) != hipSuccess)) return -104;
      if (hipStreamWaitEvent(c->stream, gi->ev, 0) != hipSuccess) return -104;
    }
    return 0;
  }
  void run(int n, int clamp, int* hist) {
    if (err || n <= 0) return;
    if (n > EML_MAX_ROUNDS) { err = -104; return; }
    if (hist && hipMemsetAsync(d_hist, 0, (size_t)n * sizeof(int), c->stream) != hipSuccess) { err = -104; return; }
    if (int rc = launch(n, clamp, d_alpha, d_a, d_alpha, d_a, hist ? d_hist : nullptr, EmsPrev{})) { err = rc; return; }
    if (hist && part) {
      if (hipStreamSynchronize(c->stream) != hipSuccess) { err = -104; return; }
      if (part->cb(part->user, (int32_t*)d_hist, n)) { err = -103; return; }
    }
    if (hist && (hipMemcpyAsync(hist, d_hist, (size_t)n * sizeof(int), hipMemcpyDeviceToHost, c->stream) != hipSuccess ||
                 hipStreamSynchronize(c->stream) != hipSuccess)) err = -104;
  }
  const std::vector<double>& host_alpha() {
    h_alpha.resize(M);
    if (gi && !err) {
      h_gi_prev.swap(h_gi_cur);
      h_gi_cur.resize(gi->plan.args.M);
      if (hipMemcpyAsync(h_gi_cur.data(), gi->G_al[0], (size_t)gi->plan.args.M * 8, hipMemcpyDeviceToHost, c->stream) != hipSuccess) err = -104;
    }
    ++host_reads;
    if (!err && ((M && hipMemcpyAsync(h_alpha.data(), d_alpha, M * 8, hipMemcpyDeviceToHost, c->stream) != hipSuccess) ||
                 hipStreamSynchronize(c->stream) != hipSuccess)) err = -104;
    return h_alpha;
  }
};
int EmSellGpu::setup(int hist_ints, const double* d_eff_new, u64 T_out) {
  Carver sv;
  const u64 Mp = M ? M : 1;
  const size_t o_al = sv.take(2 * Mp * 8 + 8), o_a = sv.take(2 * Mp * 8 + 8), o_h = sv.take((size_t)hist_ints * 4 + 8), o_out = sv.take(2 * T_out * 8 + 8);
  if (int rc = c->pm_b.ensure(sv.off, 0, c->stream)) return rc;
  char* sb = (char*)c->pm_b.p;
  d_alpha = (double*)(sb + o_al); d_a = (double*)(sb + o_a); d_ck_alpha = d_alpha + Mp; d_ck_a = d_a + Mp; d_hist = (int*)(sb + o_h); d_out = (double*)(sb + o_out);
  if (M) hipLaunchKernelGGL(k_eml_init, dim3(grid_for(M, BLOCK)), dim3(BLOCK), 0, c->stream, d_alpha, d_a, d_eff_new, M, 1.0 / (double)P.T);
  HIPC(hipGetLastError());
  lds = (size_t)P.max_group_bytes;
  reg_words = 0;
  {
    const int cap = std::min(64, std::max(1, c->tune.em_split_len));
    if (c->tune.em_reg_slices == 1) reg_words = cap <= 8 ? 2 : cap <= 16 ? 4 : cap <= 32 ? 8 : 0;
  }
  if (P.n_groups > P.n_small) {
    HIPC(hipFuncSetAttribute((const void*)k_em_sell<false, 0>, hipFuncAttributeMaxDynamicSharedMemorySize, (int)lds));
    HIPC(hipFuncSetAttribute((const void*)k_em_sell<true, 0>, hipFuncAttributeMaxDynamicSharedMemorySize, (int)lds));
    HIPC(hipFuncSetAttribute((const void*)k_em_sell<false, 0, 2>, hipFuncAttributeMaxDynamicSharedMemorySize, (int)lds));
    HIPC(hipFuncSetAttribute((const void*)k_em_sell<true, 0, 2>, hipFuncAttributeMaxDynamicSharedMemorySize, (int)lds));
    HIPC(hipFuncSetAttribute((const void*)k_em_sell<false, 0, 4, 2>, hipFuncAttributeMaxDynamicSharedMemorySize, (int)lds));
    HIPC(hipFuncSetAttribute((const void*)k_em_sell<true, 0, 4, 2>, hipFuncAttributeMaxDynamicSharedMemorySize, (int)lds));
    HIPC(hipFuncSetAttribute((const void*)k_em_sell<false, 0, 8>, hipFuncAttributeMaxDynamicSharedMemorySize, (int)lds));
    HIPC(hipFuncSetAttribute((const void*)k_em_sell<true, 0, 8>, hipFuncAttributeMaxDynamicSharedMemorySize, (int)lds));
  }
  if (gi && !c->em_ev_fork) {
    HIPC(hipEventCreateWithFlags(&c->em_ev_fork, hipEventDisableTiming));
    HIPC(hipEventCreateWithFlags(&c->em_ev_join, hipEventDisableTiming));
  }
  if (gi) ev_fork = c->em_ev_fork;
  if (P.n_small) {
    team_bytes = ((size_t)P.max_small_bytes + 15) & ~(size_t)15;
    HIPC(hipFuncSetAttribute((const void*)k_em_sell_wave, hipFuncAttributeMaxDynamicSharedMemorySize, (int)(EMS_WAVE_TEAMS * team_bytes)));
    if (!c->em_side_stream) {
      HIPC(hipStreamCreateWithFlags(&c->em_side_stream, hipStreamNonBlocking));
      if (!c->em_ev_fork) {
        HIPC(hipEventCreateWithFlags(&c->em_ev_fork, hipEventDisableTiming));
        HIPC(hipEventCreateWithFlags(&c->em_ev_join, hipEventDisableTiming));
      }
    }
    side = c->em_side_stream; ev_fork = c->em_ev_fork; ev_join = c->em_ev_join;
  }
  return 0;
}
__global__ void k_em_scatter(const u32* __restrict__ mslot, const double* __restrict__ single_all, const double* __restrict__ fin,
                             const double* __restrict__ before, u64 T, int have_final, double* out_alpha, double* out_abz) {
  const u64 t = (u64)blockIdx.x * blockDim.x + threadIdx.x;
  if (t >= T) return;
  const u32 ms = mslot[t];
  const double sa = single_all[t];
  out_alpha[t] = ms != 0xFFFFFFFFu ? fin[ms] : sa;
  out_abz[t] = have_final ? (ms != 0xFFFFFFFFu ? before[ms] : sa) : 0.0;
}
__global__ void k_em_publish(EmsPrev prev) {
  __shared__ int s_stop;
  (void)ems_prev_stopped(prev, &s_stop);
}
int em_sell_drive_async(kamd_ctx* c, EmSellGpu& B, const SellCache& K, u64 T, int n_iter, int min_rounds, double* alpha_out, double* abz_out, int* rounds_out) {
  const int CH = EML_MAX_ROUNDS;
  if (n_iter <= 0) {
    hipLaunchKernelGGL(k_em_scatter, dim3(grid_for(T, BLOCK)), dim3(BLOCK), 0, c->stream, K.mslot, K.single_all, B.d_alpha, B.d_alpha, T, 0, B.d_out, B.d_out + T);
    if (B.gi) hipLaunchKernelGGL(k_gi_scatter, dim3(grid_for(T, BLOCK)), dim3(BLOCK), 0, c->stream, T, B.gi->plan.mflag, B.gi->plan.mpos, B.gi->G_al[0], B.gi->G_al[0], 0,
                                 B.d_out, B.d_out + T);
    HIPC(hipGetLastError());
    std::vector<double> tmp(2 * T);
    HIPC(hipMemcpyAsync(tmp.data(), B.d_out, 2 * T * 8, hipMemcpyDeviceToHost, c->stream));
    HIPC(hipStreamSynchronize(c->stream));
    memcpy(alpha_out, tmp.data(), T * 8);
    if (abz_out) memcpy(abz_out, tmp.data() + T, T * 8);
    *rounds_out = 0;
    return 0;
  }
  const int n_chunks = std::max(1, (n_iter + CH - 1) / CH);
  const size_t hist_ints = (size_t)(n_chunks + 1) * CH;
  const size_t need = hist_ints * 4 + 256 + 2 * T * 8 + 256;
  if (c->em_pin_bytes < need) {
    if (c->em_pin) { HIPC(hipStreamSynchronize(c->stream)); HIPC(hipHostFree(c->em_pin)); c->em_pin = nullptr; c->em_pin_bytes = 0; }
// ... 56 lines not shown
    const int base = decided * CH, n = std::min(CH, n_iter - base);
    const int* hh = h_hist + (size_t)decided * CH;
    for (int i = 0; i < n; i++) if (hh[i] == 0 && base + i > min_rounds) { stop = base + i; break; }
    if (stop >= 0) break;
    if (++decided == n_chunks) break;
  }
  const double* fin; const double* before;
  int rounds;
  const bool have_final = stop >= 0;
  if (have_final) {
    const int s = decided, base = s * CH;
    if (int rc = B.launch(stop - base + 1, 0, al[s & 1], av[s & 1], al[(s + 1) & 1], av[(s + 1) & 1], nullptr, EmsPrev{})) return kamd::fail(rc, "kamd_em_run: replay failed to launch");
    if (int rc = B.launch(1, 1, al[(s + 1) & 1], av[(s + 1) & 1], al[s & 1], av[s & 1], nullptr, EmsPrev{})) return kamd::fail(rc, "kamd_em_run: final round failed to launch");
    before = al[(s + 1) & 1]; fin = al[s & 1];
    rounds = stop + 1;
  } else {
    fin = al[n_chunks & 1]; before = fin;
    rounds = n_iter;
  }
  hipLaunchKernelGGL(k_em_scatter, dim3(grid_for(T, BLOCK)), dim3(BLOCK), 0, c->stream, K.mslot, K.single_all, fin, before, T, have_final ? 1 : 0, B.d_out, B.d_out + T);
  if (B.gi) hipLaunchKernelGGL(k_gi_scatter, dim3(grid_for(T, BLOCK)), dim3(BLOCK), 0, c->stream, T, B.gi->plan.mflag, B.gi->plan.mpos, B.gi->G_al[B.gi_par(fin)],
                               B.gi->G_al[B.gi_par(before)], have_final ? 1 : 0, B.d_out, B.d_out + T);
  HIPC(hipGetLastError());
  HIPC(hipMemcpyAsync(h_out, B.d_out, 2 * T * 8, hipMemcpyDeviceToHost, c->stream));
  HIPC(hipStreamSynchronize(c->stream));
  memcpy(alpha_out, h_out, T * 8);
  if (abz_out) memcpy(abz_out, h_out + T, T * 8);
  if (d_clk) {
    std::vector<long long> hc(clk_words);
    HIPC(hipMemcpy(hc.data(), d_clk, clk_words * 8, hipMemcpyDeviceToHost));
    if (FILE* f = fopen(clk_path, "wb")) {
      const long long hdr[4] = {(long long)(B.P.n_groups - B.P.n_small), EMS_MAX_BLOCK / 64, EMS_CLK_WORDS, B.block};
      fwrite(hdr, 8, 4, f); fwrite(hc.data(), 8, clk_words, f); fclose(f);
    }
  }
  *rounds_out = rounds;
  return 0;
}
int em_sell_setup_device(kamd_ctx* c, const u64* d_ec_off, const u32* d_ec_ids, const u32* d_counts, const u32* d_wcounts, u64 n_ecs, u64 nnz,
                         const double* eff_lens, u64 T, u64 lds_budget, u64 target, kamd_em_sell::Plan* P, EmSellDev* dev, SellCache* cache,
                         u32 small_limit = 0, u64 target_small = 0, u64 small_budget = 0, bool host_maps = true, CompStats* comp_out = nullptr) {
  namespace S = kamd_em_sell;
  kamd_em_local::Plan C;
  EmLocalDev cd{};
  kamd_em_local::BuildArgs A{};
  if (int rc = em_local_setup_device(c, d_ec_off, d_ec_ids, d_counts, d_wcounts, n_ecs, nnz, eff_lens, T, ~0ULL, target, &C, &cd, &A, small_limit, target_small, host_maps, comp_out)) return rc;
  const u32 ng = C.n_groups;
  const u64 R = C.row_base[ng], M = C.tr_base[ng];
  if (R >= 0xFFFFFFF0ULL || M >= 0xFFFFFFF0ULL) return 1;
  for (u32 g = 0; g < ng; g++)
    if (C.row_base[g + 1] - C.row_base[g] >= S::SELL_PAD || C.tr_base[g + 1] - C.tr_base[g] >= S::SELL_PAD) return 1;
  Carver tv;
  const size_t o_rlen = tv.take(R * 4 + 8), o_clen = tv.take(M * 4 + 8), o_rnew = tv.take(R * 4 + 8), o_cnew = tv.take(M * 4 + 8);
  const size_t o_rlane = tv.take(R * 4 + 8), o_clane = tv.take(M * 4 + 8), o_rvl = tv.take(R * 4 + 8), o_cvl = tv.take(M * 4 + 8), o_gsz = tv.take((size_t)ng * 16 + 16);
  if (int rc = c->ems_tmp.ensure(tv.off, 0, c->stream)) return rc;
  char* tb = (char*)c->ems_tmp.p;
  SellBuild B{};
  B.row_base = cd.row_base; B.tr_base = cd.tr_base; B.row_ptr = cd.row_ptr; B.col_ptr = cd.col_ptr; B.row_tr = cd.row_tr; B.col_row = cd.col_row;
  B.nz_base = cd.nz_base; B.cw = cd.cw; B.single = cd.single; B.eff = cd.eff; B.tr_id = cd.tr_id; B.n_groups = ng; B.R = (u32)R; B.M = (u32)M;
  B.cap = (u32)std::min(64, std::max(1, c->tune.em_split_len));
  B.rlen = (u32*)(tb + o_rlen); B.clen = (u32*)(tb + o_clen); B.rnew = (u32*)(tb + o_rnew); B.cnew = (u32*)(tb + o_cnew);
  B.rlane = (u32*)(tb + o_rlane); B.clane = (u32*)(tb + o_clane); B.rvl = (u32*)(tb + o_rvl); B.cvl = (u32*)(tb + o_cvl); B.gsz = (u32*)(tb + o_gsz);
  const u64 nseg = std::max(R, M);
  hipLaunchKernelGGL(k_sell_lens, dim3(grid_for(nseg, BLOCK)), dim3(BLOCK), 0, c->stream, B);
  hipLaunchKernelGGL(k_sell_sizes, dim3(grid_for(2 * (u64)ng, SELL_BUILD_WAVES)), dim3(64 * SELL_BUILD_WAVES), 0, c->stream, B);
  std::vector<u32> gsz((size_t)ng * 4);
  HIPC(hipMemcpyAsync(gsz.data(), B.gsz, (size_t)ng * 16, hipMemcpyDeviceToHost, c->stream));
  HIPC(hipStreamSynchronize(c->stream));
  P->n_groups = ng; P->n_small = C.n_small; P->T = T; P->row_base = C.row_base; P->tr_base = C.tr_base; P->single_all = C.single_all;
  P->rslice_base.assign(ng + 1, 0); P->cslice_base.assign(ng + 1, 0); P->rell_base.assign(ng + 1, 0); P->cell_base.assign(ng + 1, 0);
  P->max_group_bytes = 0; P->max_small_bytes = 0;
  for (u32 g = 0; g < ng; g++) {
    const u64 gb = S::group_bytes(C.row_base[g + 1] - C.row_base[g], C.tr_base[g + 1] - C.tr_base[g], gsz[4 * g], gsz[4 * g + 2], gsz[4 * g + 1], gsz[4 * g + 3]);
    if (g < P->n_small) {
      if (gb > small_budget) return 2;
      P->max_small_bytes = std::max<uint64_t>(P->max_small_bytes, gb);
    } else {
      if (gb > lds_budget) return 1;
      P->max_group_bytes = std::max<uint64_t>(P->max_group_bytes, gb);
    }
    P->rslice_base[g + 1] = P->rslice_base[g] + gsz[4 * g]; P->rell_base[g + 1] = P->rell_base[g] + gsz[4 * g + 1];
    P->cslice_base[g + 1] = P->cslice_base[g] + gsz[4 * g + 2]; P->cell_base[g + 1] = P->cell_base[g] + gsz[4 * g + 3];
  }
  const u64 nrs = P->rslice_base[ng], ncs = P->cslice_base[ng], nru = P->rell_base[ng], ncu = P->cell_base[ng];
  Carver pv;
  const size_t p_rsb = pv.take((ng + 1) * 4), p_csb = pv.take((ng + 1) * 4), p_reb = pv.take((ng + 1) * 8), p_ceb = pv.take((ng + 1) * 8);
  const size_t p_rd = pv.take(nrs * 8 + 8), p_cdesc = pv.take(ncs * 8 + 8), p_re = pv.take(nru * 2 + 8), p_ce = pv.take(ncu * 2 + 8);
  const size_t p_cw = pv.take(R * 8 + 8), p_sg = pv.take(M * 8 + 8), p_ef = pv.take(M * 8 + 8), p_id = pv.take(M * 4 + 8);
  if (int rc = c->ems_plan.ensure(pv.off, 0, c->stream)) return rc;
  char* pb = (char*)c->ems_plan.p;
  HIPC(hipMemcpyAsync(pb + p_rsb, P->rslice_base.data(), (ng + 1) * 4, hipMemcpyHostToDevice, c->stream));
  HIPC(hipMemcpyAsync(pb + p_csb, P->cslice_base.data(), (ng + 1) * 4, hipMemcpyHostToDevice, c->stream));
  HIPC(hipMemcpyAsync(pb + p_reb, P->rell_base.data(), (ng + 1) * 8, hipMemcpyHostToDevice, c->stream));
  HIPC(hipMemcpyAsync(pb + p_ceb, P->cell_base.data(), (ng + 1) * 8, hipMemcpyHostToDevice, c->stream));
  HIPC(hipMemsetAsync(pb + p_re, 0xFF, nru * 2, c->stream));
  HIPC(hipMemsetAsync(pb + p_ce, 0xFF, ncu * 2, c->stream));
  B.rslice_base = (const u32*)(pb + p_rsb); B.cslice_base = (const u32*)(pb + p_csb); B.rell_base = (const u64*)(pb + p_reb); B.cell_base = (const u64*)(pb + p_ceb);
  B.rdesc = (u32*)(pb + p_rd); B.cdesc = (u32*)(pb + p_cdesc); B.rell = (uint16_t*)(pb + p_re); B.cell = (uint16_t*)(pb + p_ce);
  B.cw_new = (u64*)(pb + p_cw); B.single_new = (double*)(pb + p_sg); B.eff_new = (double*)(pb + p_ef); B.tr_id_new = (u32*)(pb + p_id);
  hipLaunchKernelGGL(k_sell_layout, dim3(grid_for(2 * (u64)ng, SELL_BUILD_WAVES)), dim3(64 * SELL_BUILD_WAVES), 0, c->stream, B);
  hipLaunchKernelGGL(k_sell_entries, dim3(grid_for(nseg, BLOCK)), dim3(BLOCK), 0, c->stream, B);
  HIPC(hipGetLastError());
  if (host_maps) {
    P->tr_id.resize(M);
    if (M) HIPC(hipMemcpyAsync(P->tr_id.data(), B.tr_id_new, M * 4, hipMemcpyDeviceToHost, c->stream));
  }
  Carver bv;
  const size_t b_rb = bv.take((ng + 1) * 4), b_tb = bv.take((ng + 1) * 4), b_rf = bv.take(n_ecs * 4 + 8), b_ms = bv.take(T * 4 + 8), b_sa = bv.take(T * 8 + 8),
               b_ef = bv.take(T * 8 + 8);
  if (int rc = c->ems_maps.ensure(bv.off, 0, c->stream)) return rc;
  char* mb = (char*)c->ems_maps.p;
  HIPC(hipMemcpyAsync(mb + b_rb, cd.row_base, (ng + 1) * 4, hipMemcpyDeviceToDevice, c->stream));
  HIPC(hipMemcpyAsync(mb + b_tb, cd.tr_base, (ng + 1) * 4, hipMemcpyDeviceToDevice, c->stream));
  hipLaunchKernelGGL(k_sell_maps, dim3(grid_for(std::max<u64>(n_ecs, T), BLOCK)), dim3(BLOCK), 0, c->stream, A, B, (u32*)(mb + b_rf), (u32*)(mb + b_ms));
  HIPC(hipMemcpyAsync(mb + b_sa, A.single_all, T * 8, hipMemcpyDeviceToDevice, c->stream));
  HIPC(hipGetLastError());
  HIPC(hipStreamSynchronize(c->stream));
  *dev = EmSellDev{(const u32*)(mb + b_rb), (const u32*)(mb + b_tb), B.rslice_base, B.cslice_base, B.rell_base, B.cell_base, B.rdesc, B.cdesc, B.rell, B.cell,
                   B.cw_new, B.single_new, B.eff_new};
  if (cache) { cache->row_final = (u32*)(mb + b_rf); cache->mslot = (u32*)(mb + b_ms); cache->single_all = (double*)(mb + b_sa); cache->d_eff = (double*)(mb + b_ef); }
  return 0;
}
}
namespace kamdi { void sell_cache_free(SellCache* k) { delete k; } }
namespace {
__global__ void k_hy_comp_nnz(const u64* __restrict__ ec_off, const u32* __restrict__ ec_ids, u64 n_ecs, const u32* __restrict__ label, u32* c_nnz) {
  const u64 e = (u64)blockIdx.x * blockDim.x + threadIdx.x;
  u32 root = 0xFFFFFFFFu, len = 0;
  if (e < n_ecs) {
    const u64 a = ec_off[e], b = ec_off[e + 1];
    if (b - a >= 2) { root = label[ec_ids[a]]; len = (u32)(b - a); }
  }
  const bool act = len != 0;
  const u64 am = __ballot(act);
  if (!am) return;
// ... 172 lines not shown
    K.hy.cnt_s = cnt_s; K.hy.cnt_g = cnt_g; K.hy.wc_s = wc_s; K.hy.wc_g = wc_g; K.hy.n_s = n_s; K.hy.n_g = n_g; K.hy.no_groups = K.row_final == nullptr;
    c->last_em_giant_nnz = c->last_em_nnz_multi; c->last_em_giant_rows = A.R; c->last_em_giant_tr = A.M; c->last_em_giant_chunks = G.plan.n_chunks;
    return 0;
  }
  return 1;
}
__global__ void k_hy_counts(const u32* __restrict__ counts, const u32* __restrict__ wcounts, u64 n_ecs, const u32* __restrict__ row_flag, const u64* __restrict__ row_pos,
                            u32* out_counts, u32* out_wcounts) {
  const u64 e = (u64)blockIdx.x * blockDim.x + threadIdx.x;
  if (e >= n_ecs || !row_flag[e]) return;
  out_counts[row_pos[e]] = counts[e]; out_wcounts[row_pos[e]] = wcounts[e];
}
__global__ void k_gi_refresh(const u64* __restrict__ off, const u32* __restrict__ ids, const u32* __restrict__ counts, const u32* __restrict__ wcounts, u64 n,
                             const u64* __restrict__ rpos, u64* cw, double* single_t) {
  const u64 e = (u64)blockIdx.x * blockDim.x + threadIdx.x;
  if (e >= n) return;
  const u64 a = off[e], len = off[e + 1] - a;
  if (len == 1) single_t[ids[a]] = (double)counts[e];
  else if (len >= 2) cw[rpos[e]] = (u64)counts[e] | ((u64)wcounts[e] << 32);
}
int em_hybrid_refresh(kamd_ctx* c, SellCache& K, const u32* d_counts, const u32* d_wcounts, u64 n_ecs, const double* eff_lens, u64 T) {
  const SellCache::HyKeep& H = K.hy;
  GiantPart& G = K.G;
  const PmArgs& A = G.plan.args;
  hipLaunchKernelGGL(k_hy_counts, dim3(grid_for(n_ecs, BLOCK)), dim3(BLOCK), 0, c->stream, d_counts, d_wcounts, n_ecs, H.flag_s, H.rpos_s, H.cnt_s, H.wc_s);
  hipLaunchKernelGGL(k_hy_counts, dim3(grid_for(n_ecs, BLOCK)), dim3(BLOCK), 0, c->stream, d_counts, d_wcounts, n_ecs, H.flag_g, H.rpos_g, H.cnt_g, H.wc_g);
  HIPC(hipMemsetAsync(K.single_all, 0, T * 8, c->stream));
  if (H.no_groups) { if (H.n_s) hipLaunchKernelGGL(k_hy_single, dim3(grid_for(H.n_s, BLOCK)), dim3(BLOCK), 0, c->stream, H.off_s, H.ids_s, (const u32*)H.cnt_s, H.n_s, K.single_all); }
  else {
    HIPC(hipMemcpyAsync(K.d_eff, eff_lens, T * 8, hipMemcpyHostToDevice, c->stream));
    hipLaunchKernelGGL(k_sell_refresh, dim3(grid_for(std::max<u64>(H.n_s, T), BLOCK)), dim3(BLOCK), 0, c->stream, H.off_s, H.ids_s, (const u32*)H.cnt_s, (const u32*)H.wc_s,
                       H.n_s, K.d_eff, T, K.row_final, K.mslot, const_cast<u64*>(K.dev.cw), const_cast<double*>(K.dev.single), const_cast<double*>(K.dev.eff), K.single_all);
  }
  for (DBuf* b : {&c->em_eff, &c->em_single}) if (int rc = b->ensure(T * sizeof(double), 0, c->stream)) return rc;
  HIPC(hipMemcpyAsync(c->em_eff.p, eff_lens, T * sizeof(double), hipMemcpyHostToDevice, c->stream));
  HIPC(hipMemsetAsync(c->em_single.p, 0, T * sizeof(double), c->stream));
  hipLaunchKernelGGL(k_gi_refresh, dim3(grid_for(H.n_g, BLOCK)), dim3(BLOCK), 0, c->stream, H.off_g, H.ids_g, (const u32*)H.cnt_g, (const u32*)H.wc_g, H.n_g, G.plan.rpos,
                     const_cast<u64*>(A.cw), c->em_single.as<double>());
  hipLaunchKernelGGL(k_pm_minit, dim3(grid_for(T, BLOCK)), dim3(BLOCK), 0, c->stream, T, G.plan.mflag, G.plan.mpos, (const u64*)nullptr, (const double*)c->em_single.as<double>(),
                     (const double*)c->em_eff.as<double>(), (u64)A.M, (u64*)nullptr, const_cast<double*>(A.single), const_cast<double*>(A.eff), A.alpha0, A.alpha1, A.a0, A.a1, A.ac0, A.ac1);
  HIPC(hipGetLastError());
  return 0;
}
int em_sell_run_device(kamd_ctx* c, const u64* d_ec_off, const u32* d_ec_ids, const u32* d_counts, const u32* d_wcounts, u64 n_ecs, u64 nnz,
                       const double* eff_lens, u64 T, int n_iter, int min_rounds, double* alpha, double* abz, int32_t* rounds,
                       const EmPartition* part = nullptr) {
  const bool multi = part && part->world > 1 && part->cb;
  if (c->n_cus == 0) { int v = 0; HIPC(hipDeviceGetAttribute(&v, hipDeviceAttributeMultiprocessorCount, c->device)); c->n_cus = v > 0 ? v : 256; }
  if (!c->sell_cache) c->sell_cache = new SellCache;
  SellCache& K = *c->sell_cache;
  HIPC(hipEventRecord(c->ev0, c->stream));
  const bool own = c->finalized && d_ec_off == (const u64*)c->result.d_ec_off && d_ec_ids == c->result.d_ec_ids;
  const bool hit = own && K.valid && K.d_ec_off == d_ec_off && K.d_ec_ids == d_ec_ids && K.n_ecs == n_ecs && K.nnz == nnz && K.T == T &&
                   K.generation == c->ec_generation && K.split_len == c->tune.em_split_len && K.group_div == c->tune.em_group_div &&
                   K.small_nnz == c->tune.em_small_nnz && (K.host_maps || !multi) &&
                   (!K.hybrid || (!multi && K.giant_nnz_t == c->tune.em_giant_nnz && K.blocked_t == c->tune.em_blocked && K.hybrid_t == c->tune.em_hybrid));
  if (hit && K.hybrid) {
    c->last_em_plan_ms = 0.f;
    if (int rc = em_hybrid_refresh(c, K, d_counts, d_wcounts, n_ecs, eff_lens, T)) return rc;
  } else if (hit) {
    c->last_em_plan_ms = 0.f;
    HIPC(hipMemcpyAsync(K.d_eff, eff_lens, T * 8, hipMemcpyHostToDevice, c->stream));
    HIPC(hipMemsetAsync(K.single_all, 0, T * 8, c->stream));
    hipLaunchKernelGGL(k_sell_refresh, dim3(grid_for(std::max<u64>(n_ecs, T), BLOCK)), dim3(BLOCK), 0, c->stream, d_ec_off, d_ec_ids, d_counts, d_wcounts,
                       n_ecs, K.d_eff, T, K.row_final, K.mslot, const_cast<u64*>(K.dev.cw), const_cast<double*>(K.dev.single), const_cast<double*>(K.dev.eff),
                       K.single_all);
    HIPC(hipGetLastError());
    if (multi) {
      K.P.single_all.resize(T);
      HIPC(hipMemcpyAsync(K.P.single_all.data(), K.single_all, T * 8, hipMemcpyDeviceToHost, c->stream));
      HIPC(hipStreamSynchronize(c->stream));
    }
  } else {
    const auto plan_t0 = std::chrono::steady_clock::now();
    K.valid = false; K.hybrid = false;
    c->last_em_giant_nnz = 0; c->last_em_giant_rows = 0; c->last_em_giant_tr = 0; c->last_em_giant_chunks = 0; c->last_em_giant_pieces = 0;
    const u64 lds_budget = 160 * 1024 - 2048;
    int prc = 1;
    if (multi && n_ecs == 0) {
      K.P = kamd_em_sell::Plan{};
      K.P.T = T; K.P.row_base.assign(1, 0); K.P.tr_base.assign(1, 0); K.P.single_all.assign(T, 0.0);
      K.dev = EmSellDev{};
      prc = 0;
    } else {
      const bool may_hybrid = c->tune.em_hybrid != 2 && n_ecs > 0;
      if (may_hybrid && c->em_prefer_hybrid) {
        prc = em_hybrid_setup(c, d_ec_off, d_ec_ids, d_counts, d_wcounts, n_ecs, nnz, eff_lens, T, lds_budget, K, true, multi);
        if (prc < 0) return prc;
        if (prc == 1) { K.hybrid = false; c->em_prefer_hybrid = false; }
      }
      if (prc == 1) {
        CompStats cst{};
        prc = em_sell_plan_search(c, d_ec_off, d_ec_ids, d_counts, d_wcounts, n_ecs, nnz, eff_lens, T, lds_budget, c->n_cus, multi, K, &cst);
        c->last_em_max_comp_nnz = cst.max_nnz;
        if (prc == 1 && may_hybrid && cst.max_nnz > 0) {
          prc = em_hybrid_setup(c, d_ec_off, d_ec_ids, d_counts, d_wcounts, n_ecs, nnz, eff_lens, T, lds_budget, K, false, multi);
          if (prc == 1) K.hybrid = false;
          else if (prc == 0) c->em_prefer_hybrid = true;
        }
      }
    }
    if (prc < 0) return prc;
    bool not_applicable = prc == 1 || (!multi && K.P.n_groups == 0 && !K.hybrid);
    if (multi) {
      int flag = not_applicable ? 1 : 0;
      if (int rc = c->pt_hist.ensure(64, 0, c->stream)) return rc;
      HIPC(hipMemcpyAsync(c->pt_hist.p, &flag, sizeof(int), hipMemcpyHostToDevice, c->stream));
      HIPC(hipStreamSynchronize(c->stream));
      if (int rc = part->cb(part->user, (int32_t*)c->pt_hist.p, 1)) return kamd::fail(-103, "kamd_em_run_partitioned: the sum callback failed (" + std::to_string(rc) + ")");
      HIPC(hipMemcpyAsync(&flag, c->pt_hist.p, sizeof(int), hipMemcpyDeviceToHost, c->stream));
      HIPC(hipStreamSynchronize(c->stream));
      not_applicable = flag != 0;
    }
    if (not_applicable) return 1;
    c->last_em_plan_ms = std::chrono::duration<float, std::milli>(std::chrono::steady_clock::now() - plan_t0).count();
    if (own) {
      K.giant_nnz_t = c->tune.em_giant_nnz; K.blocked_t = c->tune.em_blocked; K.hybrid_t = c->tune.em_hybrid;
      K.valid = true; K.d_ec_off = d_ec_off; K.d_ec_ids = d_ec_ids; K.n_ecs = n_ecs; K.nnz = nnz; K.T = T; K.generation = c->ec_generation;
      K.split_len = c->tune.em_split_len; K.group_div = c->tune.em_group_div; K.small_nnz = c->tune.em_small_nnz; K.host_maps = multi;
    }
  }
  const kamd_em_sell::Plan& P = K.P;
  const int chunk = EML_MAX_ROUNDS;
  EmSellGpu B(c, P);
  B.dev = K.dev; B.M = P.tr_base[P.n_groups]; B.block = c->tune.em_local_block; B.part = multi ? part : nullptr;
  if (K.hybrid) { B.gi = &K.G; B.ev_sell = c->hy_ev_sell; }
  const int n_chunks = std::max(1, (n_iter + chunk - 1) / chunk);
  if (int rc = B.setup(multi ? chunk : n_chunks * chunk, K.dev.eff, multi ? 0 : T)) return rc;
  int r = 0;
  if (multi) {
    r = kamd_em_local::run(B, P, n_iter, min_rounds, chunk, alpha, abz);
    if (K.hybrid && !B.err) {
      const PmPlan& GP = K.G.plan;
      std::vector<u32> mflag(T); std::vector<u64> mpos(T);
      HIPC(hipMemcpyAsync(mflag.data(), GP.mflag, T * 4, hipMemcpyDeviceToHost, c->stream));
      HIPC(hipMemcpyAsync(mpos.data(), GP.mpos, T * 8, hipMemcpyDeviceToHost, c->stream));
      HIPC(hipStreamSynchronize(c->stream));
      const bool have_final = B.host_reads >= 2;
      for (u64 t = 0; t < T; t++) if (mflag[t]) {
        alpha[t] = B.h_gi_cur[mpos[t]];
        if (abz) abz[t] = have_final ? B.h_gi_prev[mpos[t]] : 0.0;
      }
    }
  }
  else if (int rc = em_sell_drive_async(c, B, K, T, n_iter, min_rounds, alpha, abz, &r)) return rc;
  if (B.err) return kamd::fail(B.err, "kamd_em_run: the component-local EM failed on the device");
  HIPC(hipEventRecord(c->ev1, c->stream));
  HIPC(hipEventSynchronize(c->ev1));
  HIPC(hipEventElapsedTime(&c->last_em_ms, c->ev0, c->ev1));
  c->last_em_iters = (uint64_t)r + (r < n_iter ? 1 : 0);
  c->last_em_nnz = nnz; c->last_em_k = -2; c->last_em_grid = P.n_groups; c->last_em_necs = n_ecs;
  c->last_em_lds = (uint32_t)P.max_group_bytes;
  c->last_em_plan_cached = hit ? 1 : 0;
  c->last_em_graph_fallback = (K.hybrid && c->tune.em_graph != 2 && !K.G.use_graph) ? 1 : 0;
  if (rounds) *rounds = r;
  return 0;
}
int em_run_impl(kamd_ctx* c, const uint64_t* d_ec_off, const uint32_t* d_ec_ids, const uint32_t* d_counts,
                const uint32_t* d_weight_counts, uint64_t n_ecs, const double* eff_lens, uint64_t n_targets, uint32_t n_iter,
                uint32_t min_rounds, double* alpha, double* alpha_before_zeroes, int32_t* rounds, const EmPartition& part) {
  if (!c || !eff_lens || !alpha) return kamd::fail(-1, "kamd_em_run: null argument");
  HIPC(hipSetDevice(c->device));
  if (!d_ec_off) {
    if (!c->finalized) return kamd::fail(-1, "kamd_em_run: no EC result (call kamd_ec_finalize or pass a CSR)");
    d_ec_off = c->result.d_ec_off; d_ec_ids = c->result.d_ec_ids; n_ecs = c->result.n_ecs;
    if (!d_counts) d_counts = c->result.d_counts;
    if (!d_weight_counts) d_weight_counts = c->result.d_counts;
  }
  const u32* d_wcounts = d_weight_counts ? d_weight_counts : d_counts;
  const u64 T = n_targets;
  if (T == 0) return kamd::fail(-1, "kamd_em_run: no targets");
  const bool spec = part.world > 1;
  if (spec && n_ecs) {
    u64 nnz_all = 0;
    HIPC(hipMemcpyAsync(&nnz_all, (const u64*)d_ec_off + n_ecs, sizeof(u64), hipMemcpyDeviceToHost, c->stream));
    HIPC(hipStreamSynchronize(c->stream));
    if (int rc = c->pt_label.ensure((T + 1) * sizeof(u32), 0, c->stream)) return rc;
    if (int rc = c->pt_hist.ensure(64, 0, c->stream)) return rc;
    if (int rc = cc_labels(c, (const u64*)d_ec_off, d_ec_ids, (u64)n_ecs, T)) return rc;
    for (DBuf* b : {&c->pt_flag, &c->pt_len}) if (int rc = b->ensure((n_ecs + 1) * sizeof(u32), 0, c->stream)) return rc;
    for (DBuf* b : {&c->pt_rowpos, &c->pt_nnzpos}) if (int rc = b->ensure((n_ecs + 2) * sizeof(u64), 0, c->stream)) return rc;
    hipLaunchKernelGGL(k_part_sizes, dim3(grid_for(n_ecs, BLOCK)), dim3(BLOCK), 0, c->stream, (const u64*)d_ec_off, d_ec_ids, (u64)n_ecs,
                       c->pt_label.as<u32>(), part.rank, part.world, c->pt_flag.as<u32>(), c->pt_len.as<u32>());
    if (int rc = exclusive_scan(c, c->pt_flag.as<u32>(), n_ecs, c->pt_rowpos.as<u64>(), c->pt_rowpos.as<u64>() + n_ecs)) return rc;
    if (int rc = exclusive_scan(c, c->pt_len.as<u32>(), n_ecs, c->pt_nnzpos.as<u64>(), c->pt_nnzpos.as<u64>() + n_ecs)) return rc;
    u64 n_local = 0, nnz_local = 0;
    HIPC(hipMemcpyAsync(&n_local, c->pt_rowpos.as<u64>() + n_ecs, sizeof(u64), hipMemcpyDeviceToHost, c->stream));
    HIPC(hipMemcpyAsync(&nnz_local, c->pt_nnzpos.as<u64>() + n_ecs, sizeof(u64), hipMemcpyDeviceToHost, c->stream));
    HIPC(hipStreamSynchronize(c->stream));
    if (int rc = c->pt_off.ensure((n_local + 2) * sizeof(u64), 0, c->stream)) return rc;
    if (int rc = c->pt_ids.ensure((nnz_local + 1) * sizeof(u32), 0, c->stream)) return rc;
    if (int rc = c->pt_counts.ensure((n_local + 1) * sizeof(u32), 0, c->stream)) return rc;
    if (int rc = c->pt_wcounts.ensure((n_local + 1) * sizeof(u32), 0, c->stream)) return rc;
    hipLaunchKernelGGL(k_part_copy, dim3(grid_for(n_ecs, BLOCK)), dim3(BLOCK), 0, c->stream, (const u64*)d_ec_off, d_ec_ids, d_counts,
                       d_wcounts, (u64)n_ecs, c->pt_flag.as<u32>(), c->pt_rowpos.as<u64>(), c->pt_nnzpos.as<u64>(), c->pt_off.as<u64>(),
                       c->pt_ids.as<u32>(), c->pt_counts.as<u32>(), c->pt_wcounts.as<u32>());
    HIPC(hipMemcpyAsync(c->pt_off.as<u64>() + n_local, &nnz_local, sizeof(u64), hipMemcpyHostToDevice, c->stream));
    HIPC(hipStreamSynchronize(c->stream));
    HIPC(hipGetLastError());
    d_ec_off = c->pt_off.as<uint64_t>(); d_ec_ids = c->pt_ids.as<u32>(); d_counts = c->pt_counts.as<u32>(); d_wcounts = c->pt_wcounts.as<u32>();
    n_ecs = n_local;
    (void)nnz_all;
  }
  u64 nnz = 0;
  if (n_ecs) {
// ... 320 lines not shown
```

### kallisto_amd/csrc/kamd_em_sell.h

```cpp
#pragma once
#include <cstdint>
#include <vector>

#include "kamd_em_local.h"

namespace kamd_em_sell {

static const uint32_t SELL_LANES = 64;
static const uint32_t SELL_PAD = 0xFFFFu;
static const uint32_t SELL_META_WORDS = 64;
KAMD_HD uint32_t quad_width(uint32_t width) { return (width + 3u) & ~3u; }
static const uint32_t META_LAST = 1u << 23, META_ACTIVE = 1u << 24;

KAMD_HD uint32_t seg_lanes(uint32_t len, uint32_t cap) { const uint32_t nv = (len + cap - 1) / cap; return len <= cap ? 1u : (nv > SELL_LANES ? SELL_LANES : nv); }
KAMD_HD uint32_t seg_vlen(uint32_t len, uint32_t cap) { const uint32_t nv = seg_lanes(len, cap); return (len + nv - 1) / nv; }

static const uint32_t DESC_META = 1u << 31;

struct LayoutSize { uint32_t n_slices; uint32_t n_u16; };

struct NullSink {
  static const bool wants_segments = false;
  KAMD_HD void seg(uint32_t, uint32_t, uint32_t, uint32_t, uint32_t) const {}
  KAMD_HD void slice(uint32_t, uint32_t, uint32_t) const {}
  KAMD_HD void meta(uint32_t, uint32_t, uint32_t) const {}
};

static const uint32_t LAYOUT_SCRATCH_WORDS = 3 * (SELL_LANES + 1);
template <class Sink>
KAMD_HD LayoutSize layout_group(const uint32_t* len, uint32_t n, uint32_t cap, Sink& sink, uint32_t* scratch, uint32_t ss) {
#define hist(b) scratch[(size_t)(b) * ss]
#define start(b) scratch[(size_t)(SELL_LANES + 1 + (b)) * ss]
#define cur(b) scratch[(size_t)(2 * (SELL_LANES + 1) + (b)) * ss]
  for (uint32_t b = 0; b <= SELL_LANES; b++) hist(b) = 0;
  uint32_t n_split = 0;
  for (uint32_t i = 0; i < n; i++) { const uint32_t l = len[i]; if (l > cap) ++n_split; else ++hist(l); }
  uint32_t lane = 0;
  uint32_t next_id = 0;
  for (uint32_t i = 0; i < n && n_split; i++) {
    const uint32_t l = len[i];
    if (l <= cap) continue;
    const uint32_t nv = seg_lanes(l, cap), vl = seg_vlen(l, cap);
    if ((lane % SELL_LANES) + nv > SELL_LANES) lane = (lane / SELL_LANES + 1) * SELL_LANES;
    sink.seg(i, next_id++, lane, nv, vl);
    lane += nv;
  }
  const uint32_t split_lanes = lane;
  { uint32_t c = split_lanes; for (uint32_t b = SELL_LANES; b >= 1; b--) { start(b) = c; c += hist(b); } start(0) = c; }
  const uint32_t total_lanes = start(0);
  if (Sink::wants_segments) {
    for (uint32_t b = 0; b <= SELL_LANES; b++) cur(b) = 0;
    for (uint32_t i = 0; i < n; i++) {
      const uint32_t l = len[i];
      if (l > cap) continue;
      const uint32_t p = start(l) + cur(l);
      cur(l) = cur(l) + 1;
      sink.seg(i, n_split + (p - split_lanes), p, 1u, l);
    }
  }
  const uint32_t n_slices = (total_lanes + SELL_LANES - 1) / SELL_LANES;
  const uint32_t meta_slices = (split_lanes + SELL_LANES - 1) / SELL_LANES;
  uint32_t off = 0;
  uint32_t si = 0;
  uint32_t i_split = 0, lane2 = 0;
  for (si = 0; si < n_slices; si++) {
    const uint32_t lo = si * SELL_LANES, hi = lo + SELL_LANES;
    uint32_t width = 0;
    const bool has_meta = si < meta_slices;
    if (has_meta) {
      for (uint32_t l = 0; l < SELL_LANES; l++) sink.meta(off, l, 0u);
      uint32_t id = 0, ln = 0;
      ln = 0; id = 0;
      for (uint32_t i = 0; i < n; i++) {
        const uint32_t l = len[i];
        if (l <= cap) continue;
        const uint32_t nv = seg_lanes(l, cap), vl = seg_vlen(l, cap);
        if ((ln % SELL_LANES) + nv > SELL_LANES) ln = (ln / SELL_LANES + 1) * SELL_LANES;
        if (ln >= lo && ln < hi) {
          if (vl > width) width = vl;
          for (uint32_t v = 0; v < nv; v++)
            sink.meta(off, ln - lo + v, id | (v << 16) | (v + 1 == nv ? META_LAST : 0u) | META_ACTIVE);
        }
        ln += nv; ++id;
      }
      (void)i_split; (void)lane2;
    }
    const uint32_t plo = lo > split_lanes ? lo : split_lanes;
    if (plo < hi && plo < total_lanes) {
      uint32_t b = SELL_LANES;
      while (b > 1 && !(plo >= start(b) && plo < start(b) + hist(b))) --b;
      if (b > width) width = b;
      if (has_meta) {
        const uint32_t phi = hi < total_lanes ? hi : total_lanes;
        for (uint32_t p = plo; p < phi; p++) sink.meta(off, p - lo, (n_split + (p - split_lanes)) | META_LAST | META_ACTIVE);
      }
    }
    const uint32_t first_seg = has_meta ? 0u : n_split + (lo - split_lanes);
    sink.slice(si, off | (has_meta ? DESC_META : 0u), width | (first_seg << 16));
    off += (has_meta ? 2 * SELL_META_WORDS : 0u) + quad_width(width) * SELL_LANES;
  }
#undef hist
#undef start
#undef cur
  return LayoutSize{n_slices, off};
}

KAMD_HD uint64_t group_bytes(uint64_t rows, uint64_t tr, uint64_t row_slices, uint64_t col_slices, uint64_t row_u16, uint64_t col_u16) {
  return (tr + 1) * 8 * 4 + tr * 8 * 2 + (rows + 1) * 8 + rows * 8 + (row_slices + col_slices) * 8 + ((row_u16 + col_u16 + 3) & ~3ULL) * 2 + 64;
}

struct Plan {
  uint32_t n_groups = 0;
  uint32_t n_small = 0;
  uint64_t T = 0;
  uint32_t cap = SELL_LANES;
  std::vector<uint32_t> row_base, tr_base;
  std::vector<uint32_t> rslice_base, cslice_base;
  std::vector<uint64_t> rell_base, cell_base;
  std::vector<uint32_t> rdesc, cdesc;
  std::vector<uint16_t> rell, cell;
  std::vector<uint64_t> cw;
  std::vector<double> single, eff;
  std::vector<uint32_t> tr_id;
  std::vector<double> single_all;
  uint64_t max_group_bytes = 0;
  uint64_t max_small_bytes = 0;
};

struct VecSink {
  static const bool wants_segments = true;
  std::vector<uint32_t>* new_id; std::vector<uint32_t>* lane; std::vector<uint32_t>* nv; std::vector<uint32_t>* vlen;
  std::vector<uint32_t>* desc; std::vector<uint16_t>* ell; uint64_t ell0; uint32_t desc0; uint32_t seg0;
  void seg(uint32_t old, uint32_t id, uint32_t ln, uint32_t n, uint32_t vl) const { (*new_id)[seg0 + old] = id; (*lane)[seg0 + old] = ln; (*nv)[seg0 + old] = n; (*vlen)[seg0 + old] = vl; }
  void slice(uint32_t i, uint32_t d0, uint32_t d1) const { if (desc) { (*desc)[2 * (desc0 + i)] = d0; (*desc)[2 * (desc0 + i) + 1] = d1; } }
  void meta(uint32_t off, uint32_t l, uint32_t w) const { if (ell) { (*ell)[ell0 + off + 2 * l] = (uint16_t)w; (*ell)[ell0 + off + 2 * l + 1] = (uint16_t)(w >> 16); } }
};
KAMD_HD uint64_t entry_pos(const uint32_t* desc, uint32_t lane, uint32_t vlen, uint32_t q) {
  const uint32_t v = q / vlen, j = q % vlen;
  const uint32_t ln = lane + v, s = ln / SELL_LANES;
  const uint32_t d0 = desc[2 * s];
  const uint64_t base = (uint64_t)(d0 & ~DESC_META) + ((d0 & DESC_META) ? 2 * SELL_META_WORDS : 0u);
  return base + (uint64_t)(j / 4) * (4 * SELL_LANES) + (uint64_t)(ln % SELL_LANES) * 4 + (j % 4);
}

inline int from_csr_plan(const kamd_em_local::Plan& C, uint64_t budget_bytes, Plan* P, uint32_t cap = SELL_LANES) {
  const uint32_t ng = C.n_groups;
  P->cap = cap;
  P->n_groups = ng; P->n_small = C.n_small; P->T = C.T; P->row_base = C.row_base; P->tr_base = C.tr_base; P->single_all = C.single_all;
  const uint64_t R = C.row_base[ng], M = C.tr_base[ng];
  std::vector<uint32_t> rlen(R), clen(M), rnew(R), cnew(M), rlane(R), clane(M), rnv(R), cnv(M), rvl(R), cvl(M);
  P->rslice_base.assign(ng + 1, 0); P->cslice_base.assign(ng + 1, 0); P->rell_base.assign(ng + 1, 0); P->cell_base.assign(ng + 1, 0);
  P->max_group_bytes = 0;
  for (uint32_t g = 0; g < ng; g++) {
    const kamd_em_local::Group G = C.group(g);
    for (uint32_t r = 0; r < G.n_rows; r++) rlen[C.row_base[g] + r] = G.row_ptr[r + 1] - G.row_ptr[r];
    for (uint32_t t = 0; t < G.n_tr; t++) clen[C.tr_base[g] + t] = G.col_ptr[t + 1] - G.col_ptr[t];
    if (G.n_rows >= SELL_PAD || G.n_tr >= SELL_PAD) return 1;
    NullSink ns;
    uint32_t scratch[LAYOUT_SCRATCH_WORDS];
    const LayoutSize lr = layout_group(rlen.data() + C.row_base[g], G.n_rows, cap, ns, scratch, 1);
    const LayoutSize lc = layout_group(clen.data() + C.tr_base[g], G.n_tr, cap, ns, scratch, 1);
    const uint64_t gb = group_bytes(G.n_rows, G.n_tr, lr.n_slices, lc.n_slices, lr.n_u16, lc.n_u16);
    if (gb > budget_bytes) return 1;
    if (g < P->n_small) { if (gb > P->max_small_bytes) P->max_small_bytes = gb; }
    else if (gb > P->max_group_bytes) P->max_group_bytes = gb;
    P->rslice_base[g + 1] = P->rslice_base[g] + lr.n_slices; P->cslice_base[g + 1] = P->cslice_base[g] + lc.n_slices;
    P->rell_base[g + 1] = P->rell_base[g] + lr.n_u16; P->cell_base[g + 1] = P->cell_base[g] + lc.n_u16;
  }
  P->rdesc.assign(2 * (size_t)P->rslice_base[ng], 0); P->cdesc.assign(2 * (size_t)P->cslice_base[ng], 0);
  P->rell.assign(P->rell_base[ng], (uint16_t)SELL_PAD); P->cell.assign(P->cell_base[ng], (uint16_t)SELL_PAD);
  for (uint32_t g = 0; g < ng; g++) {
    const kamd_em_local::Group G = C.group(g);
    VecSink sr{&rnew, &rlane, &rnv, &rvl, &P->rdesc, &P->rell, P->rell_base[g], P->rslice_base[g], C.row_base[g]};
    VecSink sc{&cnew, &clane, &cnv, &cvl, &P->cdesc, &P->cell, P->cell_base[g], P->cslice_base[g], C.tr_base[g]};
    uint32_t scratch[LAYOUT_SCRATCH_WORDS];
    layout_group(rlen.data() + C.row_base[g], G.n_rows, cap, sr, scratch, 1);
    layout_group(clen.data() + C.tr_base[g], G.n_tr, cap, sc, scratch, 1);
  }
  P->cw.assign(R, 0); P->single.assign(M, 0.0); P->eff.assign(M, 0.0); P->tr_id.assign(M, 0);
  for (uint32_t g = 0; g < ng; g++) {
    const kamd_em_local::Group G = C.group(g);
    const uint32_t r0 = C.row_base[g], t0 = C.tr_base[g];
    const uint32_t* rd = P->rdesc.data() + 2 * (size_t)P->rslice_base[g];
    const uint32_t* cd = P->cdesc.data() + 2 * (size_t)P->cslice_base[g];
    for (uint32_t r = 0; r < G.n_rows; r++) {
      P->cw[r0 + rnew[r0 + r]] = G.cw[r];
      for (uint32_t q = 0, j = G.row_ptr[r]; j < G.row_ptr[r + 1]; j++, q++)
        P->rell[P->rell_base[g] + entry_pos(rd, rlane[r0 + r], rvl[r0 + r], q)] = (uint16_t)cnew[t0 + G.row_tr[j]];
    }
    for (uint32_t t = 0; t < G.n_tr; t++) {
      const uint32_t m = t0 + cnew[t0 + t];
      P->single[m] = G.single[t]; P->eff[m] = G.eff[t]; P->tr_id[m] = C.tr_id[t0 + t];
      for (uint32_t q = 0, j = G.col_ptr[t]; j < G.col_ptr[t + 1]; j++, q++)
        P->cell[P->cell_base[g] + entry_pos(cd, clane[t0 + t], cvl[t0 + t], q)] = (uint16_t)rnew[r0 + G.col_row[j]];
    }
  }
  return 0;
}

inline void host_pass(const uint32_t* desc, uint32_t n_slices, const uint16_t* ell, uint32_t n_segs, const double* src, uint32_t zero,
                      double* out) {
  for (uint32_t s = 0; s < n_slices; s++) {
    const uint32_t d0 = desc[2 * s], d1 = desc[2 * s + 1];
    const bool has_meta = (d0 & DESC_META) != 0;
    const uint32_t off = d0 & ~DESC_META, width = d1 & 0xFFFFu, first_seg = d1 >> 16;
    const uint16_t* e = ell + off + (has_meta ? 2 * SELL_META_WORDS : 0);
    double lane_sum[SELL_LANES];
    for (uint32_t l = 0; l < SELL_LANES; l++) {
      double S = 0.0;
      for (uint32_t j = 0; j < width; j++) { const uint32_t ix = e[(j / 4) * (4 * SELL_LANES) + l * 4 + (j % 4)]; S += src[ix == SELL_PAD ? zero : ix]; }
      lane_sum[l] = S;
    }
    if (!has_meta) {
      for (uint32_t l = 0; l < SELL_LANES; l++) if (first_seg + l < n_segs) out[first_seg + l] = lane_sum[l];
    } else {
      for (uint32_t l = 0; l < SELL_LANES; l++) {
        const uint32_t w = (uint32_t)ell[off + 2 * l] | ((uint32_t)ell[off + 2 * l + 1] << 16);
        if (!(w & META_ACTIVE) || !(w & META_LAST)) continue;
        const uint32_t reach = (w >> 16) & 0x7Fu;
        double S = 0.0;
        for (uint32_t v = 0; v <= reach; v++) S += lane_sum[l - reach + v];
        out[w & 0xFFFFu] = S;
      }
    }
  }
}

struct CpuBackend {
  const Plan& P;
  std::vector<double> alpha, a, ck_alpha, ck_a;
  explicit CpuBackend(const Plan& p) : P(p) {
    const uint64_t M = P.tr_base[P.n_groups];
    alpha.assign(M, 1.0 / (double)P.T);
    a.resize(M);
    for (uint64_t m = 0; m < M; m++) a[m] = alpha[m] / P.eff[m];
  }
  void checkpoint() { ck_alpha = alpha; ck_a = a; }
  void restore() { alpha = ck_alpha; a = ck_a; }
  const std::vector<double>& host_alpha() { return alpha; }
  void run(int n, int clamp, int* hist) {
    std::vector<double> av, g, S, acc;
    for (uint32_t gi = 0; gi < P.n_groups; gi++) {
      const uint32_t r0 = P.row_base[gi], nR = P.row_base[gi + 1] - r0, t0 = P.tr_base[gi], nT = P.tr_base[gi + 1] - t0;
      double* al = alpha.data() + t0; double* aa = a.data() + t0;
      if (clamp) for (uint32_t t = 0; t < nT; t++) if (al[t] < 1e-7 / 10.0) { al[t] = 0.0; aa[t] = 0.0; }
      av.assign(nT + 1, 0.0); g.assign(nR + 1, 0.0); S.assign(nR, 0.0); acc.assign(nT, 0.0);
      for (int i = 0; i < n; i++) {
        for (uint32_t t = 0; t < nT; t++) av[t] = aa[t];
        host_pass(P.rdesc.data() + 2 * (size_t)P.rslice_base[gi], P.rslice_base[gi + 1] - P.rslice_base[gi], P.rell.data() + P.rell_base[gi], nR,
                  av.data(), nT, S.data());
        for (uint32_t r = 0; r < nR; r++) {
          const uint64_t w = P.cw[r0 + r];
          const uint32_t cnt = (uint32_t)w, wc = (uint32_t)(w >> 32);
          g[r] = (cnt == 0 || (double)wc * S[r] < 4.9406564584124654e-324) ? 0.0 : (double)cnt / S[r];
        }
        host_pass(P.cdesc.data() + 2 * (size_t)P.cslice_base[gi], P.cslice_base[gi + 1] - P.cslice_base[gi], P.cell.data() + P.cell_base[gi], nT,
                  g.data(), nR, acc.data());
        int ch = 0;
        for (uint32_t t = 0; t < nT; t++) {
// ... 12 lines not shown
```

### scratch/em_clk_report.py

```python
import sys
import numpy as np

raw = np.fromfile(sys.argv[1], dtype=np.int64)
ng, nw, words, block = (int(x) for x in raw[:4])
c = raw[4:].reshape(ng, nw, words)
waves = block // 64
c = c[:, :waves]
ok = c[:, 0, 0] != 0
c = c[ok]
print(f"groups {ng} (with clocks {ok.sum()}), wavefronts per group {waves}")
rows = c[:, :, 1] - c[:, :, 0]; b1 = c[:, :, 2] - c[:, :, 1]; cols = c[:, :, 3] - c[:, :, 2]; b2 = c[:, :, 4] - c[:, :, 3]
tot = c[:, :, 4].max(1) - c[:, :, 0].min(1)
nrs = c[:, 0, 5] & 0xFFFF; ncs = (c[:, 0, 5] >> 16) & 0xFFFF
nru = c[:, 0, 6] & 0xFFFFFFFF; ncu = (c[:, 0, 6] >> 32) & 0xFFFFFFFF
wall = c[:, 0, 7]
def q(x): return f"mean {x.mean():9.1f}  p10 {np.percentile(x,10):8.0f}  p50 {np.percentile(x,50):8.0f}  p90 {np.percentile(x,90):8.0f}  max {x.max():8.0f}"
print("round, shader clocks      ", q(tot))
print("round, wall ticks (10 ns) ", q(wall))
print("rows pass, slowest wave   ", q(rows.max(1)))
print("rows pass, mean wave      ", q(rows.mean(1)))
print("barrier 1, shortest wait  ", q(b1.min(1)))
print("cols pass, slowest wave   ", q(cols.max(1)))
print("cols pass, mean wave      ", q(cols.mean(1)))
print("barrier 2, shortest wait  ", q(b2.min(1)))
print("row slices / group        ", q(nrs)); print("col slices / group        ", q(ncs))
print("row stream u16 / group    ", q(nru)); print("col stream u16 / group    ", q(ncu))
print("waves with a row slice    ", q(np.minimum(nrs, waves))); print("waves with a col slice    ", q(np.minimum(ncs, waves)))
if words >= 16:
    for name, a in (("cols", 8), ("rows", 12)):
        if name == "rows":
            st, sm, wd, fn = c[:, :, 12], c[:, :, 13], c[:, :, 14], c[:, :, 15]
        else:
            st, sm, wd, fn = c[:, :, 8], c[:, :, 9], c[:, :, 10], c[:, :, 11]
        has = st != 0
        width = (wd & 0xFFFF)[has]; meta = ((wd >> 16) & 1)[has]
        t_sum = (sm - st)[has]; t_fin = (fn - sm)[has]
        print(f"{name}: first slices {has.sum()}, with split lanes {meta.mean():.2f}")
        for lo, hi in ((1, 4), (5, 8), (9, 16), (17, 24), (25, 32), (33, 64)):
            sel = (width >= lo) & (width <= hi)
            if sel.any():
                print(f"  width {lo:2d}-{hi:2d}: n {sel.sum():6d}  sums {t_sum[sel].mean():8.1f} clk ({(t_sum[sel] / np.maximum(width[sel], 1)).mean():6.1f} / trip)  scan+finish {t_fin[sel].mean():8.1f}"
                      f"  (split {t_fin[sel & (meta == 1)].mean() if (sel & (meta == 1)).any() else 0:8.1f}, plain {t_fin[sel & (meta == 0)].mean() if (sel & (meta == 0)).any() else 0:8.1f})")
```

Baseline: 1136.

## Pack short EM row slices in pairs so one wave sums two lane groups

```diff
diff --git a/include/kallisto_amd.h b/include/kallisto_amd.h
--- a/include/kallisto_amd.h
+++ b/include/kallisto_amd.h
@@ -68,7 +68,7 @@
 } kamd_quant_opts;
 
 const char* kamd_last_error(void);
-#define KAMD_ABI_VERSION 8
+#define KAMD_ABI_VERSION 9
 uint32_t kamd_abi_version(void);
 
 int kamd_index_load(const char* path, int threads, kamd_index** out);
@@ -106,6 +106,7 @@
   int32_t overflow_second_pass;
   int32_t em_giant_nnz;
   int32_t em_blocked;
+  int32_t em_pair_rows;
 } kamd_tuning;
 int kamd_ctx_tune(kamd_ctx*, const kamd_tuning*);
 int kamd_ctx_get_tuning(const kamd_ctx*, kamd_tuning* out);
@@ -207,6 +208,8 @@
   uint32_t em_collectives;
   uint64_t n_overflow_second_pass;
   uint64_t last_em_giant_pieces;
+  uint64_t last_em_row_slices;
+  uint64_t last_em_pair_slices;
 } kamd_profile;
 int kamd_profile_get(kamd_ctx*, kamd_profile* out);
 
diff --git a/kallisto_amd/api.py b/kallisto_amd/api.py
--- a/kallisto_amd/api.py
+++ b/kallisto_amd/api.py
@@ -49,11 +49,11 @@
 class Tuning(C.Structure):
     _fields_ = [(n, C.c_int32) for n in ("text_verify", "items_per_wave", "refill_min", "lds_pad", "em_form", "em_entries_per_lane", "em_windowed", "em_graph", "em_row_lanes",
                                          "em_fin_blocks", "em_local_block", "em_group_div", "em_split_len", "dedup_form", "align_chunks", "em_small_nnz", "em_reg_slices",
-                                         "em_hybrid", "overflow_second_pass", "em_giant_nnz", "em_blocked")]
+                                         "em_hybrid", "overflow_second_pass", "em_giant_nnz", "em_blocked", "em_pair_rows")]
 
 
 EM_FORMS = {"streamed": 1, "csr": 2, "local": 3}
-ABI_VERSION = 8
+ABI_VERSION = 9
 
 
 class _Profile(C.Structure):
@@ -67,7 +67,8 @@
                 ("last_em_max_comp_nnz", C.c_uint64), ("last_em_giant_nnz", C.c_uint64), ("last_em_giant_rows", C.c_uint64),
                 ("last_em_giant_tr", C.c_uint64), ("last_em_giant_chunks", C.c_uint32), ("last_em_graph_fallback", C.c_int32),
                 ("last_em_plan_ms", C.c_float), ("n_overflow_items", C.c_uint64), ("overflow_ms", C.c_float),
-                ("last_merge_ms", C.c_float), ("em_collective_ms", C.c_float), ("em_collectives", C.c_uint32), ("n_overflow_second_pass", C.c_uint64), ("last_em_giant_pieces", C.c_uint64)]
+                ("last_merge_ms", C.c_float), ("em_collective_ms", C.c_float), ("em_collectives", C.c_uint32), ("n_overflow_second_pass", C.c_uint64), ("last_em_giant_pieces", C.c_uint64),
+                ("last_em_row_slices", C.c_uint64), ("last_em_pair_slices", C.c_uint64)]
 
 
 class _AaStats(C.Structure):
@@ -552,7 +553,8 @@
                 "em_max_comp_nnz": int(p.last_em_max_comp_nnz), "em_giant_nnz": int(p.last_em_giant_nnz), "em_giant_rows": int(p.last_em_giant_rows),
                 "em_giant_tr": int(p.last_em_giant_tr), "em_giant_chunks": int(p.last_em_giant_chunks), "em_graph_fallback": int(p.last_em_graph_fallback), "em_giant_pieces": int(p.last_em_giant_pieces),
                 "em_plan_ms": float(p.last_em_plan_ms), "n_overflow_items": int(p.n_overflow_items), "overflow_ms": float(p.overflow_ms),
-                "merge_ms": float(p.last_merge_ms), "em_collective_ms": float(p.em_collective_ms), "em_collectives": int(p.em_collectives), "n_overflow_second_pass": int(p.n_overflow_second_pass)}
+                "merge_ms": float(p.last_merge_ms), "em_collective_ms": float(p.em_collective_ms), "em_collectives": int(p.em_collectives), "n_overflow_second_pass": int(p.n_overflow_second_pass),
+                "em_row_slices": int(p.last_em_row_slices), "em_pair_slices": int(p.last_em_pair_slices)}
 
     def dense_counts(self):
         torch = self.torch
diff --git a/kallisto_amd/csrc/kamd_ctx.hip b/kallisto_amd/csrc/kamd_ctx.hip
--- a/kallisto_amd/csrc/kamd_ctx.hip
+++ b/kallisto_amd/csrc/kamd_ctx.hip
@@ -6,7 +6,7 @@
   t->text_verify = 1; t->items_per_wave = 1024; t->refill_min = 8; t->lds_pad = -1;
   t->em_form = 3; t->em_local_block = 1024; t->em_group_div = -1; t->em_split_len = 16; t->em_small_nnz = -1; t->em_entries_per_lane = -1; t->em_windowed = 2; t->em_graph = 1; t->em_row_lanes = 4;
   t->em_fin_blocks = 1024; t->dedup_form = 2; t->align_chunks = -1; t->em_reg_slices = 1;
-  t->em_hybrid = 1; t->overflow_second_pass = 1; t->em_giant_nnz = -1; t->em_blocked = 1;
+  t->em_hybrid = 1; t->overflow_second_pass = 1; t->em_giant_nnz = -1; t->em_blocked = 1; t->em_pair_rows = 2;
 }
 void tuning_merge(kamd_tuning* t, const kamd_tuning& n) {
   if (n.text_verify == 1 || n.text_verify == 2) t->text_verify = n.text_verify;
@@ -30,6 +30,7 @@
   if (n.em_hybrid == 1 || n.em_hybrid == 2) t->em_hybrid = n.em_hybrid;
   if (n.overflow_second_pass >= 1 && n.overflow_second_pass <= 3) t->overflow_second_pass = n.overflow_second_pass;
   if (n.em_blocked == 1 || n.em_blocked == 2) t->em_blocked = n.em_blocked;
+  if (n.em_pair_rows == 1 || n.em_pair_rows == 2) t->em_pair_rows = n.em_pair_rows;
   if (n.em_giant_nnz != 0) t->em_giant_nnz = n.em_giant_nnz < 0 ? -1 : std::max(n.em_giant_nnz, 8);
 }
 void tuning_from_env(kamd_tuning* t) {
@@ -44,7 +45,8 @@
     {"em_fin_blocks", &kamd_tuning::em_fin_blocks, false}, {"em_local_block", &kamd_tuning::em_local_block, false}, {"em_group_div", &kamd_tuning::em_group_div, false},
     {"em_split_len", &kamd_tuning::em_split_len, false}, {"dedup_form", &kamd_tuning::dedup_form, false}, {"align_chunks", &kamd_tuning::align_chunks, false},
     {"em_small_nnz", &kamd_tuning::em_small_nnz, false}, {"em_reg_slices", &kamd_tuning::em_reg_slices, true}, {"em_hybrid", &kamd_tuning::em_hybrid, true},
-    {"overflow_second_pass", &kamd_tuning::overflow_second_pass, false}, {"em_giant_nnz", &kamd_tuning::em_giant_nnz, false}, {"em_blocked", &kamd_tuning::em_blocked, true}};
+    {"overflow_second_pass", &kamd_tuning::overflow_second_pass, false}, {"em_giant_nnz", &kamd_tuning::em_giant_nnz, false}, {"em_blocked", &kamd_tuning::em_blocked, true},
+    {"em_pair_rows", &kamd_tuning::em_pair_rows, true}};
   std::string all(e);
   for (size_t pos = 0; pos < all.size();) {
     size_t end = all.find(',', pos);
@@ -370,6 +372,7 @@
   p->last_em_max_comp_nnz = c->last_em_max_comp_nnz; p->last_em_giant_nnz = c->last_em_giant_nnz; p->last_em_giant_rows = c->last_em_giant_rows;
   p->last_em_giant_tr = c->last_em_giant_tr; p->last_em_giant_chunks = c->last_em_giant_chunks; p->last_em_graph_fallback = c->last_em_graph_fallback; p->last_em_giant_pieces = c->last_em_giant_pieces;
   p->last_em_plan_ms = c->last_em_plan_ms;
+  p->last_em_row_slices = c->last_em_row_slices; p->last_em_pair_slices = c->last_em_pair_slices;
   p->n_overflow_items = c->overflow_total; p->overflow_ms = c->overflow_ms;
   p->n_overflow_second_pass = c->overflow_second_total;
   p->last_merge_ms = c->last_merge_ms; p->em_collective_ms = c->em_coll_ms; p->em_collectives = c->em_coll_n;
diff --git a/kallisto_amd/csrc/kamd_dev.h b/kallisto_amd/csrc/kamd_dev.h
--- a/kallisto_amd/csrc/kamd_dev.h
+++ b/kallisto_amd/csrc/kamd_dev.h
@@ -275,7 +275,7 @@
   hipStream_t hy_giant_stream = nullptr;
   hipEvent_t hy_ev_sell = nullptr, hy_ev_giant = nullptr;
   uint64_t last_em_max_comp_nnz = 0, last_em_giant_nnz = 0, last_em_giant_rows = 0, last_em_giant_tr = 0;
-  uint32_t last_em_giant_chunks = 0; uint64_t last_em_giant_pieces = 0; int last_em_graph_fallback = 0; float last_em_plan_ms = 0.f;
+  uint32_t last_em_giant_chunks = 0; uint64_t last_em_giant_pieces = 0, last_em_row_slices = 0, last_em_pair_slices = 0; int last_em_graph_fallback = 0; float last_em_plan_ms = 0.f;
   float last_merge_ms = 0.f, em_coll_ms = 0.f; uint32_t em_coll_n = 0; hipEvent_t ev_mg0 = nullptr, ev_mg1 = nullptr;
   const uint32_t* labels_override = nullptr;
   bool em_prefer_hybrid = false;
diff --git a/kallisto_amd/csrc/kamd_em.hip b/kallisto_amd/csrc/kamd_em.hip
--- a/kallisto_amd/csrc/kamd_em.hip
+++ b/kallisto_amd/csrc/kamd_em.hip
@@ -1154,7 +1154,7 @@
   }
   return S;
 }
-template <int W, int NS>
+template <int W, int NS, bool PAIRS>
 __device__ __forceinline__ void ems_group_rounds_reg(const EmSellDev& P, u32 g, unsigned char* smem, u32 tid, u32 nthr, const double* alpha, const double* a,
                                                      double* alpha_out, double* a_out, int n_rounds, int clamp, int* s_hist, long long* clk = nullptr) {
   namespace L = kamd_em_sell;
@@ -1186,19 +1186,28 @@
   for (u32 i = tid; i < ncu; i += nthr) { const uint16_t v = P.cell[ce0 + i]; s_cell[i] = v == (uint16_t)L::SELL_PAD ? (uint16_t)nR : v; }
   if (tid == 0) { s_al0[nT] = s_a0[nT] = 0.0; s_g[nR] = 0.0; }
   __syncthreads();
-  struct Own { u64 w[W]; u32 nq, seg, steps; int reach; bool has, meta, fin; };
-  auto take = [&](const u32* desc, const uint16_t* ell, u32 s, u32 n_slices, u32 n_segs, u32 zero, u32 base_off) {
+  struct Own { u64 w[W]; u32 nq, nq0, seg, steps; int reach; bool has, meta, fin, pair, fin2; };
+  auto take = [&](auto pairable, const u32* desc, const uint16_t* ell, u32 s, u32 n_slices, u32 n_segs, u32 zero, u32 base_off) {
+    constexpr bool CAN_PAIR = decltype(pairable)::value;
     Own o;
-    o.has = near && s < n_slices; o.nq = 1; o.seg = 0; o.reach = 0; o.meta = false; o.fin = false; o.steps = 0;
-    if (o.has && (((desc[2 * s + 1] & 0xFFFFu) + 3u) >> 2) > (u32)W) o.has = false;
+    o.has = near && s < n_slices; o.nq = 1; o.nq0 = 0; o.seg = 0; o.reach = 0; o.meta = false; o.fin = false; o.steps = 0; o.pair = false; o.fin2 = false;
+    auto words_of = [&](u32 d0, u32 d1) -> u32 {
+      if constexpr (CAN_PAIR) { if (d0 & L::DESC_PAIR) return ((L::pair_w0(d1) + 3u) >> 2) + ((L::pair_w1(d1) + 3u) >> 2); }
+      return ((d1 & 0xFFFFu) + 3u) >> 2;
+    };
+    if (o.has && words_of(desc[2 * s], desc[2 * s + 1]) > (u32)W) o.has = false;
     const u64 padw = (u64)(base_off + zero * 8u) * 0x0001000100010001ULL;
 #pragma unroll
     for (int q = 0; q < W; q++) o.w[q] = padw;
     if (o.has) {
       const u32 d0 = desc[2 * s], d1 = desc[2 * s + 1];
       o.meta = (d0 & L::DESC_META) != 0;
-      const u32 off = d0 & ~L::DESC_META, width = d1 & 0xFFFFu;
-      o.nq = (u32)__builtin_amdgcn_readfirstlane((int)((width + 3u) >> 2));
+      const u32 off = d0 & L::DESC_OFF_MASK;
+      o.nq = (u32)__builtin_amdgcn_readfirstlane((int)words_of(d0, d1));
+      if constexpr (CAN_PAIR) {
+        o.pair = __builtin_amdgcn_readfirstlane((int)(d0 & L::DESC_PAIR)) != 0;
+        o.nq0 = (u32)__builtin_amdgcn_readfirstlane((int)((L::pair_w0(d1) + 3u) >> 2));
+      }
       const u64* e = reinterpret_cast<const u64*>(ell + off + (o.meta ? 2 * L::SELL_META_WORDS : 0u)) + lane;
 #pragma unroll
       for (int q = 0; q < W; q++) if ((u32)q < o.nq) {
@@ -1206,6 +1215,7 @@
         o.w[q] = ((ix4 & 0x1FFF1FFF1FFF1FFFULL) << 3) + (u64)base_off * 0x0001000100010001ULL;
       }
       o.seg = (d1 >> 16) + (u32)lane; o.fin = o.seg < n_segs;
+      if constexpr (CAN_PAIR) o.fin2 = o.pair && o.seg + L::SELL_LANES < n_segs;
       if (o.meta) {
         const u32 w = reinterpret_cast<const u32*>(ell + off)[lane];
         o.reach = (int)((w >> 16) & 0x7Fu); o.seg = w & 0xFFFFu; o.fin = (w & L::META_ACTIVE) && (w & L::META_LAST);
@@ -1221,8 +1231,8 @@
   u32 r_next = wv, c_next = wv;
 #pragma unroll
   for (int k = 0; k < NS; k++) {
-    ro[k] = take(s_rdesc, s_rell, wv + (u32)k * NW, nrs, nR, nT, a_off);
-    co[k] = take(s_cdesc, s_cell, wv + (u32)k * NW, ncs, nT, nR, g_off);
+    ro[k] = take(std::integral_constant<bool, PAIRS>{}, s_rdesc, s_rell, wv + (u32)k * NW, nrs, nR, nT, a_off);
+    co[k] = take(std::false_type{}, s_cdesc, s_cell, wv + (u32)k * NW, ncs, nT, nR, g_off);
     if (ro[k].has && r_next == wv + (u32)k * NW) r_next += NW; else ro[k].has = false;
     if (co[k].has && c_next == wv + (u32)k * NW) c_next += NW; else co[k].has = false;
     r_cnt[k] = 0; r_wc[k] = 0; c_single[k] = 0.0; c_eff[k] = 1.0; c_at[k] = 0.0; c_cur[k] = 0.0;
@@ -1231,6 +1241,7 @@
   }
   double* const al = s_al0; double* const av = s_a0;
   const unsigned char* const lds0 = smem;
+  auto row_g = [](u32 cnt, u32 wc, double S) { return (cnt == 0 || (double)wc * S < 4.9406564584124654e-324) ? 0.0 : (double)cnt / S; };
   for (int r = 0; r < n_rounds; r++) {
     const bool tick = clk && r == EMS_CLK_ROUND && lane == 0;
     long long w0 = 0;
@@ -1240,6 +1251,22 @@
       if (ro[k].has) {
         const bool tk = tick && k == 0;
         if (tk) clk[12] = clock64();
+        if constexpr (PAIRS) {
+          if (ro[k].pair) {
+            u64 cw2 = 0;
+            if (ro[k].fin2) cw2 = s_cw[ro[k].seg + L::SELL_LANES];
+            double v[16], S0, S1;
+            auto tree4 = [](const double* x) { return (x[0] + x[1]) + (x[2] + x[3]); };
+            if (ro[k].nq0 == 1) { ems_reg_gather<2>(ro[k].w, lds0, v); S0 = tree4(v); S1 = tree4(v + 4); }
+            else if (ro[k].nq == 3) { ems_reg_gather<3>(ro[k].w, lds0, v); S0 = tree4(v) + tree4(v + 4); S1 = tree4(v + 8); }
+            else { ems_reg_gather<4>(ro[k].w, lds0, v); S0 = tree4(v) + tree4(v + 4); S1 = tree4(v + 8) + tree4(v + 12); }
+            if (tk) { clk[13] = clock64(); clk[14] = (long long)((ro[k].nq * 4u) | 0x20000u); }
+            if (ro[k].fin) s_g[ro[k].seg] = row_g(r_cnt[k], r_wc[k], S0);
+            if (ro[k].fin2) s_g[ro[k].seg + L::SELL_LANES] = row_g((u32)cw2, (u32)(cw2 >> 32), S1);
+            if (tk) clk[15] = clock64();
+            continue;
+          }
+        }
         double S = ems_reg_slice_sum<W, TREE>(ro[k].w, ro[k].nq, lds0);
         if (tk) { clk[13] = clock64(); clk[14] = (long long)((ro[k].nq * 4u) | (ro[k].meta ? 0x10000u : 0u)); }
         if (ro[k].meta) S = pm_scan_seg_masked(S, ro[k].reach, lane, ro[k].steps);
@@ -1250,7 +1277,18 @@
     for (u32 s = r_next; s < nrs; s += NW) {
       const u32 d0 = s_rdesc[2 * s], d1 = s_rdesc[2 * s + 1];
       const bool meta = (d0 & L::DESC_META) != 0;
-      const u32 off = d0 & ~L::DESC_META, width = d1 & 0xFFFFu;
+      const u32 off = d0 & L::DESC_OFF_MASK, width = d1 & 0xFFFFu;
+      if constexpr (PAIRS) {
+        if (d0 & L::DESC_PAIR) {
+          const u32 w0 = L::pair_w0(d1), w1 = L::pair_w1(d1);
+          const u64* e = reinterpret_cast<const u64*>(s_rell + off) + lane;
+          const double S0 = ems_slice_sum_narrow(e, w0, av), S1 = ems_slice_sum_narrow(e + (size_t)((w0 + 3u) >> 2) * 64, w1, av);
+          const u32 seg = (d1 >> 16) + (u32)lane;
+          if (seg < nR) { const u64 cwv = s_cw[seg]; s_g[seg] = row_g((u32)cwv, (u32)(cwv >> 32), S0); }
+          if (seg + L::SELL_LANES < nR) { const u64 cwv = s_cw[seg + L::SELL_LANES]; s_g[seg + L::SELL_LANES] = row_g((u32)cwv, (u32)(cwv >> 32), S1); }
+          continue;
+        }
+      }
       double S = ems_slice_sum_narrow(reinterpret_cast<const u64*>(s_rell + off + (meta ? 2 * L::SELL_META_WORDS : 0u)) + lane, width, av);
       u32 seg = (d1 >> 16) + (u32)lane; bool fin = seg < nR;
       if (meta) {
@@ -1294,7 +1332,7 @@
     for (u32 s = c_next; s < ncs; s += NW) {
       const u32 d0 = s_cdesc[2 * s], d1 = s_cdesc[2 * s + 1];
       const bool meta = (d0 & L::DESC_META) != 0;
-      const u32 off = d0 & ~L::DESC_META, width = d1 & 0xFFFFu;
+      const u32 off = d0 & L::DESC_OFF_MASK, width = d1 & 0xFFFFu;
       double acc = ems_slice_sum_narrow(reinterpret_cast<const u64*>(s_cell + off + (meta ? 2 * L::SELL_META_WORDS : 0u)) + lane, width, s_g);
       u32 seg = (d1 >> 16) + (u32)lane; bool fin = seg < nT;
       if (meta) {
@@ -1331,7 +1369,7 @@
   __syncthreads();
   return *s_flag != 0;
 }
-template <bool CLK, int EXP = 0, int W = 0, int NS = 1>
+template <bool CLK, int EXP = 0, int W = 0, int NS = 1, bool PAIRS = false>
 __global__ __launch_bounds__(EMS_MAX_BLOCK) __attribute__((amdgpu_waves_per_eu((W >= 8 || (W == 4 && NS == 2)) ? 4 : 8))) void k_em_sell(EmSellDev P, u32 g_first, const double* alpha, const double* a, double* alpha_out, double* a_out,
                                                            int n_rounds, int clamp, int* hist, EmsPrev prev, long long* clk) {
   extern __shared__ __attribute__((aligned(16))) unsigned char ems_smem[];
@@ -1341,7 +1379,7 @@
   if (threadIdx.x < EML_MAX_ROUNDS) s_hist[threadIdx.x] = 0;
   __syncthreads();
   long long* my_clk = CLK ? clk + ((size_t)blockIdx.x * (EMS_MAX_BLOCK / 64) + (threadIdx.x >> 6)) * EMS_CLK_WORDS : nullptr;
-  if constexpr (W > 0) ems_group_rounds_reg<W, NS>(P, g_first + blockIdx.x, ems_smem, threadIdx.x, blockDim.x, alpha, a, alpha_out, a_out, n_rounds, clamp, s_hist, my_clk);
+  if constexpr (W > 0) ems_group_rounds_reg<W, NS, PAIRS>(P, g_first + blockIdx.x, ems_smem, threadIdx.x, blockDim.x, alpha, a, alpha_out, a_out, n_rounds, clamp, s_hist, my_clk);
   else ems_group_rounds<false, EXP>(P, g_first + blockIdx.x, ems_smem, threadIdx.x, blockDim.x, alpha, a, alpha_out, a_out, n_rounds, clamp, s_hist, my_clk);
   __syncthreads();
   if (hist && (int)threadIdx.x < n_rounds && s_hist[threadIdx.x]) atomicAdd(&hist[threadIdx.x], s_hist[threadIdx.x]);
@@ -1364,6 +1402,7 @@
 struct SellBuild {
   const u32* row_base; const u32* tr_base; const u32* row_ptr; const u32* col_ptr; const uint16_t* row_tr; const uint16_t* col_row; const u64* nz_base;
   const u64* cw; const double* single; const double* eff; const u32* tr_id; u32 n_groups; u32 R; u32 M; u32 cap;
+  u32 pair_from;
   u32* rlen; u32* clen; u32* rnew; u32* cnew; u32* rlane; u32* clane; u32* rvl; u32* cvl; u32* gsz;
   const u32* rslice_base; const u32* cslice_base; const u64* rell_base; const u64* cell_base;
   u32* rdesc; u32* cdesc; uint16_t* rell; uint16_t* cell; u64* cw_new; double* single_new; double* eff_new; u32* tr_id_new;
@@ -1379,9 +1418,10 @@
   if (i < B.M) { const u32 g = sell_group_of(B.tr_base, B.n_groups, i); B.clen[i] = B.col_ptr[(u64)i + g + 1] - B.col_ptr[(u64)i + g]; }
 }
 constexpr int SELL_BUILD_WAVES = 4;
+constexpr u32 SELL_GSZ = 6;
 struct SellWaveScratch { u32 hist[kamd_em_sell::SELL_LANES + 1], start[kamd_em_sell::SELL_LANES + 1], cur[kamd_em_sell::SELL_LANES + 1]; };
 template <class Sink>
-__device__ kamd_em_sell::LayoutSize sell_layout_wave(const u32* __restrict__ len, u32 n, u32 cap, Sink& sink, SellWaveScratch& S) {
+__device__ kamd_em_sell::LayoutSize sell_layout_wave(const u32* __restrict__ len, u32 n, u32 cap, Sink& sink, SellWaveScratch& S, bool pair = false) {
   namespace L = kamd_em_sell;
   const int lane = lane_id();
   for (u32 b = lane; b <= L::SELL_LANES; b += 64) { S.hist[b] = 0; S.cur[b] = 0; }
@@ -1427,6 +1467,7 @@
   if (lane == 0) { u32 c = split_lanes; for (u32 b = L::SELL_LANES; b >= 1; b--) { S.start[b] = c; c += S.hist[b]; } S.start[0] = c; }
   __builtin_amdgcn_wave_barrier();
   const u32 total_lanes = S.start[0];
+  const u32 p0 = pair ? L::pair_tail_start(split_lanes, S.start[cap < L::PAIR_LEN ? cap : L::PAIR_LEN], total_lanes) : total_lanes;
   if (Sink::wants_segments) {
     for (u32 c0 = 0; c0 < n; c0 += 64) {
       const u32 i = c0 + lane;
@@ -1441,7 +1482,7 @@
       __builtin_amdgcn_wave_barrier();
       if (act) {
         const u32 p = S.start[l] + base + below;
-        sink.seg(i, n_split + (p - split_lanes), p, 1u, l);
+        sink.seg(i, n_split + (p - split_lanes), p < p0 ? p : L::pair_lane(p, p0), 1u, l);
         if (below + 1 == cls) S.cur[l] = base + cls;
       }
       __builtin_amdgcn_wave_barrier();
@@ -1452,7 +1493,9 @@
     while (b > 1 && !(p >= S.start[b] && p < S.start[b] + S.hist[b])) --b;
     return b;
   };
-  const u32 n_slices = (total_lanes + L::SELL_LANES - 1) / L::SELL_LANES;
+  const u32 n_head = (p0 + L::SELL_LANES - 1) / L::SELL_LANES;
+  const u32 n_slices = n_head + (total_lanes - p0 + 2 * L::SELL_LANES - 1) / (2 * L::SELL_LANES);
+  u32 n_paired = 0;
   if (split_lanes % L::SELL_LANES) {
     const u32 lo = closed * L::SELL_LANES, p = lo + (u32)lane;
     if (split_lanes < total_lanes) { const u32 b = len_at(split_lanes); width = b > width ? b : width; }
@@ -1463,14 +1506,18 @@
   }
   for (u32 s0 = closed; s0 < n_slices; s0 += 64) {
     const u32 si = s0 + (u32)lane;
-    u32 w = 0;
-    if (si < n_slices) w = len_at(si * L::SELL_LANES);
-    const u32 mine = L::quad_width(w) * L::SELL_LANES;
+    const u32 pb = si < n_head ? si * L::SELL_LANES : p0 + (si - n_head) * 2 * L::SELL_LANES;
+    const bool paired = si >= n_head && si < n_slices && total_lanes - pb > L::SELL_LANES;
+    u32 w = 0, w1 = 0;
+    if (si < n_slices) w = len_at(pb);
+    if (paired) w1 = len_at(pb + L::SELL_LANES);
+    const u32 mine = (L::quad_width(w) + L::quad_width(w1)) * L::SELL_LANES;
     const u32 incl = wave_incl_scan(mine);
-    if (si < n_slices) sink.slice(si, off + (incl - mine), w | ((n_split + (si * L::SELL_LANES - split_lanes)) << 16));
+    if (si < n_slices) sink.slice(si, (off + (incl - mine)) | (paired ? L::DESC_PAIR : 0u), w | (w1 << 8) | ((n_split + (pb - split_lanes)) << 16));
     off += (u32)__shfl((int)incl, 63, 64);
-  }
-  return L::LayoutSize{n_slices, off};
+    n_paired += (u32)__popcll(__ballot(paired));
+  }
+  return L::LayoutSize{n_slices, off, n_paired};
 }
 __global__ __launch_bounds__(64 * SELL_BUILD_WAVES) void k_sell_sizes(SellBuild B) {
   __shared__ SellWaveScratch scr[SELL_BUILD_WAVES];
@@ -1478,8 +1525,8 @@
   if (g >= B.n_groups) return;
   kamd_em_sell::NullSink ns;
   const kamd_em_sell::LayoutSize z = (w & 1) ? sell_layout_wave(B.clen + B.tr_base[g], B.tr_base[g + 1] - B.tr_base[g], B.cap, ns, scr[threadIdx.x / 64])
-                                             : sell_layout_wave(B.rlen + B.row_base[g], B.row_base[g + 1] - B.row_base[g], B.cap, ns, scr[threadIdx.x / 64]);
-  if (lane_id() == 0) { B.gsz[4 * g + 2 * (w & 1)] = z.n_slices; B.gsz[4 * g + 2 * (w & 1) + 1] = z.n_u16; }
+                                             : sell_layout_wave(B.rlen + B.row_base[g], B.row_base[g + 1] - B.row_base[g], B.cap, ns, scr[threadIdx.x / 64], g >= B.pair_from);
+  if (lane_id() == 0) { u32* o = B.gsz + SELL_GSZ * g + (SELL_GSZ / 2) * (w & 1); o[0] = z.n_slices; o[1] = z.n_u16; o[2] = z.n_paired; }
 }
 struct SellDevSink {
   static const bool wants_segments = true;
@@ -1497,7 +1544,7 @@
     sell_layout_wave(B.clen + B.tr_base[g], B.tr_base[g + 1] - B.tr_base[g], B.cap, sc, scr[threadIdx.x / 64]);
   } else {
     SellDevSink sr{B.rnew, B.rlane, B.rvl, B.rdesc, B.rell, B.row_base[g], B.rslice_base[g], B.rell_base[g]};
-    sell_layout_wave(B.rlen + B.row_base[g], B.row_base[g + 1] - B.row_base[g], B.cap, sr, scr[threadIdx.x / 64]);
+    sell_layout_wave(B.rlen + B.row_base[g], B.row_base[g + 1] - B.row_base[g], B.cap, sr, scr[threadIdx.x / 64], g >= B.pair_from);
   }
 }
 __global__ void k_sell_entries(SellBuild B) {
@@ -2581,11 +2628,16 @@
   return 0;
 }
 }
+inline bool ems_pair_rows(const kamd_tuning& t) {
+  const int cap = std::min(64, std::max(1, t.em_split_len));
+  return t.em_pair_rows == 1 && t.em_reg_slices == 1 && cap > 8 && cap <= 32;
+}
 namespace kamdi {
 struct SellCache {
   bool valid = false;
   const u64* d_ec_off = nullptr; const u32* d_ec_ids = nullptr; u64 n_ecs = 0, nnz = 0, T = 0, generation = 0;
   int split_len = 0, group_div = 0, small_nnz = 0;
+  bool pair_rows = false;
   bool host_maps = false;
   kamd_em_sell::Plan P;
   EmSellDev dev{};
@@ -2654,14 +2706,18 @@
     }
     if (n_big) {
 #define KAMD_EMS_LAUNCH(C, E) hipLaunchKernelGGL((k_em_sell<C, E>), dim3(n_big), dim3(block), lds, ss, dev, P.n_small, al_in, a_in, al_out, a_out, n, clamp, d_h, prev, clk)
-#define KAMD_EMS_LAUNCH_REG(C, W, NS) hipLaunchKernelGGL((k_em_sell<C, 0, W, NS>), dim3(n_big), dim3(block), lds, ss, dev, P.n_small, al_in, a_in, al_out, a_out, n, clamp, d_h, prev, clk)
-      if (reg_words == 2) { if (clk) KAMD_EMS_LAUNCH_REG(true, 2, 1); else KAMD_EMS_LAUNCH_REG(false, 2, 1); }
-      else if (reg_words == 4) { if (clk) KAMD_EMS_LAUNCH_REG(true, 4, 2); else KAMD_EMS_LAUNCH_REG(false, 4, 2); }
-      else if (reg_words == 8) { if (clk) KAMD_EMS_LAUNCH_REG(true, 8, 1); else KAMD_EMS_LAUNCH_REG(false, 8, 1); }
+#define KAMD_EMS_LAUNCH_REG(C, W, NS, PR) hipLaunchKernelGGL((k_em_sell<C, 0, W, NS, PR>), dim3(n_big), dim3(block), lds, ss, dev, P.n_small, al_in, a_in, al_out, a_out, n, clamp, d_h, prev, clk)
+#define KAMD_EMS_LAUNCH_PAIRS(W, NS) do { \
+        if (P.pair_rows) { if (clk) KAMD_EMS_LAUNCH_REG(true, W, NS, true); else KAMD_EMS_LAUNCH_REG(false, W, NS, true); } \
+        else { if (clk) KAMD_EMS_LAUNCH_REG(true, W, NS, false); else KAMD_EMS_LAUNCH_REG(false, W, NS, false); } } while (0)
+      if (reg_words == 2) { if (clk) KAMD_EMS_LAUNCH_REG(true, 2, 1, false); else KAMD_EMS_LAUNCH_REG(false, 2, 1, false); }
+      else if (reg_words == 4) KAMD_EMS_LAUNCH_PAIRS(4, 2);
+      else if (reg_words == 8) KAMD_EMS_LAUNCH_PAIRS(8, 1);
       else if (clk) KAMD_EMS_LAUNCH(true, 0);
       else KAMD_EMS_LAUNCH(false, 0);
 #undef KAMD_EMS_LAUNCH
 #undef KAMD_EMS_LAUNCH_REG
+#undef KAMD_EMS_LAUNCH_PAIRS
     }
     EmsPrev prev_w = prev;
     if (n_big) prev_w.host_hist = nullptr;
@@ -2720,10 +2776,11 @@
     HIPC(hipFuncSetAttribute((const void*)k_em_sell<true, 0>, hipFuncAttributeMaxDynamicSharedMemorySize, (int)lds));
     HIPC(hipFuncSetAttribute((const void*)k_em_sell<false, 0, 2>, hipFuncAttributeMaxDynamicSharedMemorySize, (int)lds));
     HIPC(hipFuncSetAttribute((const void*)k_em_sell<true, 0, 2>, hipFuncAttributeMaxDynamicSharedMemorySize, (int)lds));
-    HIPC(hipFuncSetAttribute((const void*)k_em_sell<false, 0, 4, 2>, hipFuncAttributeMaxDynamicSharedMemorySize, (int)lds));
-    HIPC(hipFuncSetAttribute((const void*)k_em_sell<true, 0, 4, 2>, hipFuncAttributeMaxDynamicSharedMemorySize, (int)lds));
-    HIPC(hipFuncSetAttribute((const void*)k_em_sell<false, 0, 8>, hipFuncAttributeMaxDynamicSharedMemorySize, (int)lds));
-    HIPC(hipFuncSetAttribute((const void*)k_em_sell<true, 0, 8>, hipFuncAttributeMaxDynamicSharedMemorySize, (int)lds));
+#define KAMD_EMS_ATTR(W, NS, PR) \
+    HIPC(hipFuncSetAttribute((const void*)k_em_sell<false, 0, W, NS, PR>, hipFuncAttributeMaxDynamicSharedMemorySize, (int)lds)); \
+    HIPC(hipFuncSetAttribute((const void*)k_em_sell<true, 0, W, NS, PR>, hipFuncAttributeMaxDynamicSharedMemorySize, (int)lds))
+    KAMD_EMS_ATTR(4, 2, false); KAMD_EMS_ATTR(4, 2, true); KAMD_EMS_ATTR(8, 1, false); KAMD_EMS_ATTR(8, 1, true);
+#undef KAMD_EMS_ATTR
   }
   if (gi && !c->em_ev_fork) {
     HIPC(hipEventCreateWithFlags(&c->em_ev_fork, hipEventDisableTiming));
@@ -2886,26 +2943,30 @@
     if (C.row_base[g + 1] - C.row_base[g] >= S::SELL_PAD || C.tr_base[g + 1] - C.tr_base[g] >= S::SELL_PAD) return 1;
   Carver tv;
   const size_t o_rlen = tv.take(R * 4 + 8), o_clen = tv.take(M * 4 + 8), o_rnew = tv.take(R * 4 + 8), o_cnew = tv.take(M * 4 + 8);
-  const size_t o_rlane = tv.take(R * 4 + 8), o_clane = tv.take(M * 4 + 8), o_rvl = tv.take(R * 4 + 8), o_cvl = tv.take(M * 4 + 8), o_gsz = tv.take((size_t)ng * 16 + 16);
+  const size_t o_rlane = tv.take(R * 4 + 8), o_clane = tv.take(M * 4 + 8), o_rvl = tv.take(R * 4 + 8), o_cvl = tv.take(M * 4 + 8), o_gsz = tv.take((size_t)ng * SELL_GSZ * 4 + 16);
   if (int rc = c->ems_tmp.ensure(tv.off, 0, c->stream)) return rc;
   char* tb = (char*)c->ems_tmp.p;
   SellBuild B{};
   B.row_base = cd.row_base; B.tr_base = cd.tr_base; B.row_ptr = cd.row_ptr; B.col_ptr = cd.col_ptr; B.row_tr = cd.row_tr; B.col_row = cd.col_row;
   B.nz_base = cd.nz_base; B.cw = cd.cw; B.single = cd.single; B.eff = cd.eff; B.tr_id = cd.tr_id; B.n_groups = ng; B.R = (u32)R; B.M = (u32)M;
   B.cap = (u32)std::min(64, std::max(1, c->tune.em_split_len));
+  P->pair_rows = ems_pair_rows(c->tune); P->n_pair_slices = 0;
+  B.pair_from = P->pair_rows ? C.n_small : ng;
   B.rlen = (u32*)(tb + o_rlen); B.clen = (u32*)(tb + o_clen); B.rnew = (u32*)(tb + o_rnew); B.cnew = (u32*)(tb + o_cnew);
   B.rlane = (u32*)(tb + o_rlane); B.clane = (u32*)(tb + o_clane); B.rvl = (u32*)(tb + o_rvl); B.cvl = (u32*)(tb + o_cvl); B.gsz = (u32*)(tb + o_gsz);
   const u64 nseg = std::max(R, M);
   hipLaunchKernelGGL(k_sell_lens, dim3(grid_for(nseg, BLOCK)), dim3(BLOCK), 0, c->stream, B);
   hipLaunchKernelGGL(k_sell_sizes, dim3(grid_for(2 * (u64)ng, SELL_BUILD_WAVES)), dim3(64 * SELL_BUILD_WAVES), 0, c->stream, B);
-  std::vector<u32> gsz((size_t)ng * 4);
-  HIPC(hipMemcpyAsync(gsz.data(), B.gsz, (size_t)ng * 16, hipMemcpyDeviceToHost, c->stream));
+  std::vector<u32> gsz((size_t)ng * SELL_GSZ);
+  HIPC(hipMemcpyAsync(gsz.data(), B.gsz, (size_t)ng * SELL_GSZ * 4, hipMemcpyDeviceToHost, c->stream));
   HIPC(hipStreamSynchronize(c->stream));
   P->n_groups = ng; P->n_small = C.n_small; P->T = T; P->row_base = C.row_base; P->tr_base = C.tr_base; P->single_all = C.single_all;
   P->rslice_base.assign(ng + 1, 0); P->cslice_base.assign(ng + 1, 0); P->rell_base.assign(ng + 1, 0); P->cell_base.assign(ng + 1, 0);
   P->max_group_bytes = 0; P->max_small_bytes = 0;
   for (u32 g = 0; g < ng; g++) {
-    const u64 gb = S::group_bytes(C.row_base[g + 1] - C.row_base[g], C.tr_base[g + 1] - C.tr_base[g], gsz[4 * g], gsz[4 * g + 2], gsz[4 * g + 1], gsz[4 * g + 3]);
+    const u32* gz = gsz.data() + (size_t)SELL_GSZ * g;
+    const u64 gb = S::group_bytes(C.row_base[g + 1] - C.row_base[g], C.tr_base[g + 1] - C.tr_base[g], gz[0], gz[3], gz[1], gz[4]);
+    P->n_pair_slices += gz[2];
     if (g < P->n_small) {
       if (gb > small_budget) return 2;
       P->max_small_bytes = std::max<uint64_t>(P->max_small_bytes, gb);
@@ -2913,8 +2974,8 @@
       if (gb > lds_budget) return 1;
       P->max_group_bytes = std::max<uint64_t>(P->max_group_bytes, gb);
     }
-    P->rslice_base[g + 1] = P->rslice_base[g] + gsz[4 * g]; P->rell_base[g + 1] = P->rell_base[g] + gsz[4 * g + 1];
-    P->cslice_base[g + 1] = P->cslice_base[g] + gsz[4 * g + 2]; P->cell_base[g + 1] = P->cell_base[g] + gsz[4 * g + 3];
+    P->rslice_base[g + 1] = P->rslice_base[g] + gz[0]; P->rell_base[g + 1] = P->rell_base[g] + gz[1];
+    P->cslice_base[g + 1] = P->cslice_base[g] + gz[3]; P->cell_base[g + 1] = P->cell_base[g] + gz[4];
   }
   const u64 nrs = P->rslice_base[ng], ncs = P->cslice_base[ng], nru = P->rell_base[ng], ncu = P->cell_base[ng];
   Carver pv;
@@ -3193,7 +3254,7 @@
   HIPC(hipEventRecord(c->ev0, c->stream));
   const bool own = c->finalized && d_ec_off == (const u64*)c->result.d_ec_off && d_ec_ids == c->result.d_ec_ids;
   const bool hit = own && K.valid && K.d_ec_off == d_ec_off && K.d_ec_ids == d_ec_ids && K.n_ecs == n_ecs && K.nnz == nnz && K.T == T &&
-                   K.generation == c->ec_generation && K.split_len == c->tune.em_split_len && K.group_div == c->tune.em_group_div &&
+                   K.generation == c->ec_generation && K.split_len == c->tune.em_split_len && K.pair_rows == ems_pair_rows(c->tune) && K.group_div == c->tune.em_group_div &&
                    K.small_nnz == c->tune.em_small_nnz && (K.host_maps || !multi) &&
                    (!K.hybrid || (!multi && K.giant_nnz_t == c->tune.em_giant_nnz && K.blocked_t == c->tune.em_blocked && K.hybrid_t == c->tune.em_hybrid));
   if (hit && K.hybrid) {
@@ -3258,7 +3319,7 @@
     if (own) {
       K.giant_nnz_t = c->tune.em_giant_nnz; K.blocked_t = c->tune.em_blocked; K.hybrid_t = c->tune.em_hybrid;
       K.valid = true; K.d_ec_off = d_ec_off; K.d_ec_ids = d_ec_ids; K.n_ecs = n_ecs; K.nnz = nnz; K.T = T; K.generation = c->ec_generation;
-      K.split_len = c->tune.em_split_len; K.group_div = c->tune.em_group_div; K.small_nnz = c->tune.em_small_nnz; K.host_maps = multi;
+      K.split_len = c->tune.em_split_len; K.pair_rows = ems_pair_rows(c->tune); K.group_div = c->tune.em_group_div; K.small_nnz = c->tune.em_small_nnz; K.host_maps = multi;
     }
   }
   const kamd_em_sell::Plan& P = K.P;
@@ -3292,6 +3353,7 @@
   c->last_em_iters = (uint64_t)r + (r < n_iter ? 1 : 0);
   c->last_em_nnz = nnz; c->last_em_k = -2; c->last_em_grid = P.n_groups; c->last_em_necs = n_ecs;
   c->last_em_lds = (uint32_t)P.max_group_bytes;
+  c->last_em_row_slices = P.n_groups ? P.rslice_base[P.n_groups] : 0; c->last_em_pair_slices = P.n_pair_slices;
   c->last_em_plan_cached = hit ? 1 : 0;
   c->last_em_graph_fallback = (K.hybrid && c->tune.em_graph != 2 && !K.G.use_graph) ? 1 : 0;
   if (rounds) *rounds = r;
diff --git a/kallisto_amd/csrc/kamd_em_sell.h b/kallisto_amd/csrc/kamd_em_sell.h
--- a/kallisto_amd/csrc/kamd_em_sell.h
+++ b/kallisto_amd/csrc/kamd_em_sell.h
@@ -15,9 +15,22 @@
 KAMD_HD uint32_t seg_lanes(uint32_t len, uint32_t cap) { const uint32_t nv = (len + cap - 1) / cap; return len <= cap ? 1u : (nv > SELL_LANES ? SELL_LANES : nv); }
 KAMD_HD uint32_t seg_vlen(uint32_t len, uint32_t cap) { const uint32_t nv = seg_lanes(len, cap); return (len + nv - 1) / nv; }
 
-static const uint32_t DESC_META = 1u << 31;
-
-struct LayoutSize { uint32_t n_slices; uint32_t n_u16; };
+static const uint32_t DESC_META = 1u << 31, DESC_PAIR = 1u << 30, DESC_OFF_MASK = ~(DESC_META | DESC_PAIR);
+static const uint32_t PAIR_LEN = 8;
+KAMD_HD uint32_t pair_w0(uint32_t d1) { return d1 & 0xFFu; }
+KAMD_HD uint32_t pair_w1(uint32_t d1) { return (d1 >> 8) & 0xFFu; }
+static const uint32_t LANE_HALF1 = 1u << 31;
+
+struct LayoutSize { uint32_t n_slices; uint32_t n_u16; uint32_t n_paired; };
+KAMD_HD uint32_t pair_tail_start(uint32_t split_lanes, uint32_t first_le, uint32_t total_lanes) {
+  const uint32_t m = (split_lanes + SELL_LANES - 1) / SELL_LANES * SELL_LANES, f = (first_le + SELL_LANES - 1) / SELL_LANES * SELL_LANES;
+  const uint32_t p0 = m > f ? m : f;
+  return p0 < total_lanes && total_lanes - p0 > SELL_LANES ? p0 : total_lanes;
+}
+KAMD_HD uint32_t pair_lane(uint32_t p, uint32_t p0) {
+  const uint32_t t = p - p0, k = t / (2 * SELL_LANES), r = t % (2 * SELL_LANES);
+  return (p0 / SELL_LANES + k) * SELL_LANES + (r % SELL_LANES) + (r >= SELL_LANES ? LANE_HALF1 : 0u);
+}
 
 struct NullSink {
   static const bool wants_segments = false;
@@ -28,7 +41,7 @@
 
 static const uint32_t LAYOUT_SCRATCH_WORDS = 3 * (SELL_LANES + 1);
 template <class Sink>
-KAMD_HD LayoutSize layout_group(const uint32_t* len, uint32_t n, uint32_t cap, Sink& sink, uint32_t* scratch, uint32_t ss) {
+KAMD_HD LayoutSize layout_group(const uint32_t* len, uint32_t n, uint32_t cap, Sink& sink, uint32_t* scratch, uint32_t ss, bool pair = false) {
 #define hist(b) scratch[(size_t)(b) * ss]
 #define start(b) scratch[(size_t)(SELL_LANES + 1 + (b)) * ss]
 #define cur(b) scratch[(size_t)(2 * (SELL_LANES + 1) + (b)) * ss]
@@ -48,6 +61,7 @@
   const uint32_t split_lanes = lane;
   { uint32_t c = split_lanes; for (uint32_t b = SELL_LANES; b >= 1; b--) { start(b) = c; c += hist(b); } start(0) = c; }
   const uint32_t total_lanes = start(0);
+  const uint32_t p0 = pair ? pair_tail_start(split_lanes, start(cap < PAIR_LEN ? cap : PAIR_LEN), total_lanes) : total_lanes;
   if (Sink::wants_segments) {
     for (uint32_t b = 0; b <= SELL_LANES; b++) cur(b) = 0;
     for (uint32_t i = 0; i < n; i++) {
@@ -55,10 +69,10 @@
       if (l > cap) continue;
       const uint32_t p = start(l) + cur(l);
       cur(l) = cur(l) + 1;
-      sink.seg(i, n_split + (p - split_lanes), p, 1u, l);
-    }
-  }
-  const uint32_t n_slices = (total_lanes + SELL_LANES - 1) / SELL_LANES;
+      sink.seg(i, n_split + (p - split_lanes), p < p0 ? p : pair_lane(p, p0), 1u, l);
+    }
+  }
+  const uint32_t n_slices = (p0 + SELL_LANES - 1) / SELL_LANES;
   const uint32_t meta_slices = (split_lanes + SELL_LANES - 1) / SELL_LANES;
   uint32_t off = 0;
   uint32_t si = 0;
@@ -99,10 +113,26 @@
     sink.slice(si, off | (has_meta ? DESC_META : 0u), width | (first_seg << 16));
     off += (has_meta ? 2 * SELL_META_WORDS : 0u) + quad_width(width) * SELL_LANES;
   }
+  uint32_t n_paired = 0;
+  for (uint32_t pb = p0; pb < total_lanes; pb += 2 * SELL_LANES, si++) {
+    uint32_t w0 = SELL_LANES, w1 = 0;
+    while (w0 > 1 && !(pb >= start(w0) && pb < start(w0) + hist(w0))) --w0;
+    const uint32_t first_seg = n_split + (pb - split_lanes);
+    if (total_lanes - pb > SELL_LANES) {
+      w1 = w0;
+      while (w1 > 1 && !(pb + SELL_LANES >= start(w1) && pb + SELL_LANES < start(w1) + hist(w1))) --w1;
+      sink.slice(si, off | DESC_PAIR, w0 | (w1 << 8) | (first_seg << 16));
+      off += (quad_width(w0) + quad_width(w1)) * SELL_LANES;
+      ++n_paired;
+    } else {
+      sink.slice(si, off, w0 | (first_seg << 16));
+      off += quad_width(w0) * SELL_LANES;
+    }
+  }
 #undef hist
 #undef start
 #undef cur
-  return LayoutSize{n_slices, off};
+  return LayoutSize{si, off, n_paired};
 }
 
 KAMD_HD uint64_t group_bytes(uint64_t rows, uint64_t tr, uint64_t row_slices, uint64_t col_slices, uint64_t row_u16, uint64_t col_u16) {
@@ -125,6 +155,8 @@
   std::vector<double> single_all;
   uint64_t max_group_bytes = 0;
   uint64_t max_small_bytes = 0;
+  bool pair_rows = false;
+  uint64_t n_pair_slices = 0;
 };
 
 struct VecSink {
@@ -137,15 +169,16 @@
 };
 KAMD_HD uint64_t entry_pos(const uint32_t* desc, uint32_t lane, uint32_t vlen, uint32_t q) {
   const uint32_t v = q / vlen, j = q % vlen;
-  const uint32_t ln = lane + v, s = ln / SELL_LANES;
+  const uint32_t ln = (lane & ~LANE_HALF1) + v, s = ln / SELL_LANES;
   const uint32_t d0 = desc[2 * s];
-  const uint64_t base = (uint64_t)(d0 & ~DESC_META) + ((d0 & DESC_META) ? 2 * SELL_META_WORDS : 0u);
-  return base + (uint64_t)(j / 4) * (4 * SELL_LANES) + (uint64_t)(ln % SELL_LANES) * 4 + (j % 4);
-}
-
-inline int from_csr_plan(const kamd_em_local::Plan& C, uint64_t budget_bytes, Plan* P, uint32_t cap = SELL_LANES) {
+  const uint64_t base = (uint64_t)(d0 & DESC_OFF_MASK) + ((d0 & DESC_META) ? 2 * SELL_META_WORDS : 0u);
+  const uint32_t q_first = (lane & LANE_HALF1) ? quad_width(pair_w0(desc[2 * s + 1])) / 4 : 0u;
+  return base + (uint64_t)(q_first + j / 4) * (4 * SELL_LANES) + (uint64_t)(ln % SELL_LANES) * 4 + (j % 4);
+}
+
+inline int from_csr_plan(const kamd_em_local::Plan& C, uint64_t budget_bytes, Plan* P, uint32_t cap = SELL_LANES, bool pair_rows = false) {
   const uint32_t ng = C.n_groups;
-  P->cap = cap;
+  P->cap = cap; P->pair_rows = pair_rows; P->n_pair_slices = 0;
   P->n_groups = ng; P->n_small = C.n_small; P->T = C.T; P->row_base = C.row_base; P->tr_base = C.tr_base; P->single_all = C.single_all;
   const uint64_t R = C.row_base[ng], M = C.tr_base[ng];
   std::vector<uint32_t> rlen(R), clen(M), rnew(R), cnew(M), rlane(R), clane(M), rnv(R), cnv(M), rvl(R), cvl(M);
@@ -158,7 +191,8 @@
     if (G.n_rows >= SELL_PAD || G.n_tr >= SELL_PAD) return 1;
     NullSink ns;
     uint32_t scratch[LAYOUT_SCRATCH_WORDS];
-    const LayoutSize lr = layout_group(rlen.data() + C.row_base[g], G.n_rows, cap, ns, scratch, 1);
+    const LayoutSize lr = layout_group(rlen.data() + C.row_base[g], G.n_rows, cap, ns, scratch, 1, pair_rows && g >= C.n_small);
+    P->n_pair_slices += lr.n_paired;
     const LayoutSize lc = layout_group(clen.data() + C.tr_base[g], G.n_tr, cap, ns, scratch, 1);
     const uint64_t gb = group_bytes(G.n_rows, G.n_tr, lr.n_slices, lc.n_slices, lr.n_u16, lc.n_u16);
     if (gb > budget_bytes) return 1;
@@ -174,7 +208,7 @@
     VecSink sr{&rnew, &rlane, &rnv, &rvl, &P->rdesc, &P->rell, P->rell_base[g], P->rslice_base[g], C.row_base[g]};
     VecSink sc{&cnew, &clane, &cnv, &cvl, &P->cdesc, &P->cell, P->cell_base[g], P->cslice_base[g], C.tr_base[g]};
     uint32_t scratch[LAYOUT_SCRATCH_WORDS];
-    layout_group(rlen.data() + C.row_base[g], G.n_rows, cap, sr, scratch, 1);
+    layout_group(rlen.data() + C.row_base[g], G.n_rows, cap, sr, scratch, 1, pair_rows && g >= C.n_small);
     layout_group(clen.data() + C.tr_base[g], G.n_tr, cap, sc, scratch, 1);
   }
   P->cw.assign(R, 0); P->single.assign(M, 0.0); P->eff.assign(M, 0.0); P->tr_id.assign(M, 0);
@@ -203,8 +237,20 @@
   for (uint32_t s = 0; s < n_slices; s++) {
     const uint32_t d0 = desc[2 * s], d1 = desc[2 * s + 1];
     const bool has_meta = (d0 & DESC_META) != 0;
-    const uint32_t off = d0 & ~DESC_META, width = d1 & 0xFFFFu, first_seg = d1 >> 16;
+    const uint32_t off = d0 & DESC_OFF_MASK, width = d1 & 0xFFFFu, first_seg = d1 >> 16;
     const uint16_t* e = ell + off + (has_meta ? 2 * SELL_META_WORDS : 0);
+    if (d0 & DESC_PAIR) {
+      for (uint32_t h = 0; h < 2; h++) {
+        const uint32_t w = h ? pair_w1(d1) : pair_w0(d1);
+        const uint16_t* eh = e + (h ? quad_width(pair_w0(d1)) * SELL_LANES : 0u);
+        for (uint32_t l = 0; l < SELL_LANES; l++) {
+          double S = 0.0;
+          for (uint32_t j = 0; j < w; j++) { const uint32_t ix = eh[(j / 4) * (4 * SELL_LANES) + l * 4 + (j % 4)]; S += src[ix == SELL_PAD ? zero : ix]; }
+          if (first_seg + h * SELL_LANES + l < n_segs) out[first_seg + h * SELL_LANES + l] = S;
+        }
+      }
+      continue;
+    }
     double lane_sum[SELL_LANES];
     for (uint32_t l = 0; l < SELL_LANES; l++) {
       double S = 0.0;
diff --git a/scratch/em_clk_report.py b/scratch/em_clk_report.py
--- a/scratch/em_clk_report.py
+++ b/scratch/em_clk_report.py
@@ -35,7 +35,8 @@
         has = st != 0
         width = (wd & 0xFFFF)[has]; meta = ((wd >> 16) & 1)[has]
         t_sum = (sm - st)[has]; t_fin = (fn - sm)[has]
-        print(f"{name}: first slices {has.sum()}, with split lanes {meta.mean():.2f}")
+        pair = ((wd >> 17) & 1)[has]
+        print(f"{name}: first slices {has.sum()}, with split lanes {meta.mean():.2f}" + (f", paired {pair.mean():.2f}" if pair.any() else ""))
         for lo, hi in ((1, 4), (5, 8), (9, 16), (17, 24), (25, 32), (33, 64)):
             sel = (width >= lo) & (width <= hi)
             if sel.any():
```

Measured after the change: 1127. About the same (-0.8%).
